# meituan/YOLOv6

Measured on NVIDIA B200. Metric: images/sec YOLOv6-S 640 bs32, higher is better.
Workload: dtype bf16

## Files before the change

### include/yv6.h

```cpp
#ifndef YV6_H_
#define YV6_H_

#include <stdint.h>

#ifdef __cplusplus
extern "C" {
#endif

#define YV6_ABI_VERSION 4

enum {
  YV6_OK = 0,
  YV6_ERR_ARG = -1,
  YV6_ERR_CUDA = -2,
  YV6_ERR_STATE = -3
};

enum { YV6_ACT_NONE = 0, YV6_ACT_RELU = 1, YV6_ACT_SILU = 2, YV6_ACT_SIGMOID = 3 };
enum { YV6_DT_BF16 = 0, YV6_DT_F32 = 1, YV6_DT_U8 = 2 };
#define YV6_PAD_SAME (-1000000)

typedef struct yv6_handle yv6_handle;

int yv6_create(int device, yv6_handle** out);
int yv6_destroy(yv6_handle* h);
const char* yv6_last_error(void);
int yv6_abi_version(void);

typedef struct yv6_conv_desc {
  const void* x;
  int32_t N, H, W, Cin;
  int32_t x_c_total;
  int64_t x_plane_stride;
  const void* w;
  int64_t w_plane_stride;
  const float* bias;
  int32_t Cout, kh, kw, stride, pad;
  int32_t act;
  void* y;
  int32_t y_dtype;
  int64_t y_img_stride, y_h_stride, y_w_stride;
  int64_t y_plane_stride;
  const void* res;
  float alpha;
  int64_t res_img_stride, res_h_stride, res_w_stride, res_plane_stride;
  int32_t nsplit;
  int32_t force_bw, force_bh, force_bi, force_bn, force_stages, force_grid;
  int32_t force_direct;
  int32_t force_halo;
  int32_t pad_w, out_h, out_w;
  int32_t force_groups;
  void* trace;
  int32_t stride_w;
  int32_t force_pair;
  int32_t pair_view;
  int32_t reserved0;
} yv6_conv_desc;

int yv6_conv_fwd(yv6_handle* h, const yv6_conv_desc* d, void* stream);
int yv6_conv_plan(yv6_handle* h, const yv6_conv_desc* d, int32_t* out10);
int yv6_conv_plan_host(int num_sms, int max_smem_optin, int max_clusters, const yv6_conv_desc* d, int32_t* out12);

typedef struct yv6_stem_desc {
  const void* x;
  int32_t x_dtype;
  float in_scale;
  int32_t N, H, W;
  const float* w;
  const float* bias;
  int32_t Cout, act;
  void* y;
  int64_t y_plane_stride;
  int32_t nsplit;
  int32_t fp32_math;
  int32_t force_sync_loads;
} yv6_stem_desc;
int yv6_stem_fwd(yv6_handle* h, const yv6_stem_desc* d, void* stream);

int yv6_sppf_pool(yv6_handle* h, void* buf, int32_t N, int32_t H, int32_t W, int32_t C, int32_t c_total,
                  int32_t nsplit, int64_t plane_stride, void* stream);

int yv6_head_decode(yv6_handle* h, const float* cls, const float* reg, float* out, int32_t B, int32_t nc,
                    int32_t reg_ch, int32_t nl, const int32_t* lvl_h, const int32_t* lvl_w,
                    const float* lvl_stride, void* stream);

int64_t yv6_nms_workspace_bytes(int32_t B, int32_t A, int32_t nc, int32_t multi_label);
int yv6_nms_batched(yv6_handle* h, const float* pred, int32_t B, int32_t A, int32_t nc, float conf_thres,
                    double iou_thres, int32_t agnostic, int32_t multi_label, const uint8_t* class_mask,
                    int32_t max_det, float* out, int32_t* out_count, int32_t* out_src, int32_t* overflow,
                    void* workspace, int64_t workspace_bytes, void* stream);

int yv6_nms_batched_head(yv6_handle* h, const float* cls, const float* reg, int32_t B, int32_t nc, int32_t reg_ch, int32_t nl,
                         const int32_t* lvl_h, const int32_t* lvl_w, const float* lvl_stride, float conf_thres, double iou_thres,
                         int32_t agnostic, int32_t multi_label, const uint8_t* class_mask, int32_t max_det, float* out,
                         int32_t* out_count, int32_t* out_src, int32_t* overflow, void* workspace, int64_t workspace_bytes,
                         void* stream);

int yv6_eval_boxes(yv6_handle* h, const float* det, const int32_t* count, const float* meta, int32_t B, int32_t max_det,
                   float* out, void* stream);


int yv6_targets_pad(yv6_handle* h, const float* targets, int32_t n, int32_t B, int32_t G, float scale_w,
                    float scale_h, double* gt, int32_t* gt_count, void* stream);

int64_t yv6_assign_workspace_bytes(int32_t B, int32_t A, int32_t G);

int yv6_tal_assign(yv6_handle* h, const float* pd_scores, const float* pd_bboxes, const float* anc_points,
                   const double* gt, const uint8_t* mask_gt, int32_t B, int32_t A, int32_t G, int32_t nc,
                   int32_t topk, double alpha, double beta, double eps, int32_t* gt_idx, uint8_t* fg,
                   double* norm, void* workspace, int64_t workspace_bytes, void* stream);

int yv6_atss_assign(yv6_handle* h, const float* anc_bboxes, const int32_t* n_level_bboxes, int32_t nl,
                    const double* gt, const uint8_t* mask_gt, const float* pd_bboxes, int32_t B, int32_t A,
                    int32_t G, int32_t nc, int32_t topk, int32_t* gt_idx, uint8_t* fg, double* norm,
                    void* workspace, int64_t workspace_bytes, void* stream);

int yv6_assign_expand(yv6_handle* h, const double* gt, const int32_t* gt_idx, const uint8_t* fg,
                      const double* norm, int32_t B, int32_t A, int32_t G, int32_t nc, int32_t bg_label,
                      int64_t* labels, double* bboxes, double* scores, uint8_t* fg_out, void* stream);

int yv6_box_decode(yv6_handle* h, const float* pred_distri, const float* anc_points, const float* strides,
                   int32_t B, int32_t A, int32_t reg_ch, int32_t scale_to_pixels, float* boxes, void* stream);

typedef struct yv6_loss_desc {
  const float* pred_scores;
  const float* pred_distri;
  const float* anc_points;
  const float* strides;
  const double* gt;
  const int32_t* gt_idx;
  const uint8_t* fg;
  const double* norm;
  int32_t B, A, G, nc, reg_ch;
  int32_t iou_type;
  double w_cls, w_iou, w_dfl;
  double grad_scale;
  float* grad_scores;
  float* grad_distri;
  double* out;
  void* workspace;
  int64_t workspace_bytes;
  int32_t norm_gt_zero;
} yv6_loss_desc;
int64_t yv6_det_loss_workspace_bytes(int32_t B, int32_t A);
int yv6_det_loss(yv6_handle* h, const yv6_loss_desc* d, void* stream);

int yv6_head_ab_pack(yv6_handle* h, const float* raw_cls, const float* raw_reg, int32_t B, int32_t hw, int32_t na, int32_t nc,
                     const float* anchors_wh, int32_t row_off, int32_t rows_total, float* cls_ab, float* reg_ab, void* stream);
int yv6_head_ab_grad(yv6_handle* h, const float* grad_cls_ab, const float* cls_ab, const float* grad_reg_ab, const float* raw_reg,
                     int32_t B, int32_t hw, int32_t na, int32_t nc, const float* anchors_wh, int32_t row_off, int32_t rows_total,
                     int32_t cls_pad, int32_t reg_pad, void* dl_cls, void* dl_reg, void* stream);
int yv6_ab_boxes(yv6_handle* h, const float* reg_ab, const float* anc_points, const float* strides, int32_t B, int32_t A,
                 float* ltrb, float* boxes_px, void* stream);
int yv6_ab_boxes_bwd(yv6_handle* h, const float* grad_ltrb, int64_t rows, float* grad_reg_ab, void* stream);

int yv6_kl_rows(yv6_handle* h, const float* student, const float* teacher, int64_t rows, int32_t C, float temperature,
                const uint8_t* row_mask, int32_t rows_per_mask, double scale, const double* count_ptr, const double* gate_ptr,
                double* acc, float* grad, void* stream);


typedef struct yv6_wgrad_desc {
  const void* x;  int32_t N, H, W, Cin, x_c_total;
  const void* dy; int32_t Cout, dy_c_total;
  int32_t kh, kw, stride, pad;
  float* dw;
  int32_t force_ksplit;
  int32_t force_taps;
} yv6_wgrad_desc;
int yv6_conv_wgrad(yv6_handle* h, const yv6_wgrad_desc* d, void* stream);

int yv6_bn_stats(yv6_handle* h, const void* x, int64_t pixels, int32_t C, int64_t pitch, double* sum, double* sumsq,
                 void* stream);
int yv6_bn_finalize(yv6_handle* h, const double* sum, const double* sumsq, double count, const float* gamma,
                    const float* beta, float eps, float momentum, float* running_mean, float* running_var,
                    float* mean_out, float* invstd_out, float* scale, float* shift, int32_t C, void* stream);

typedef struct yv6_bn_desc {
  int32_t nb, act, C;
  int64_t pixels;
  const void* x[3];  int64_t x_pitch[3];
  const float* mean[3]; const float* invstd[3]; const float* scale[3]; const float* shift[3];
  void* y; int64_t y_pitch;
  const void* dy; int64_t dy_pitch;
  double* s1; double* s2[3];
  void* dx[3]; int64_t dx_pitch[3]; int32_t accumulate[3];
  const void* res; int64_t res_pitch; float res_alpha;
  void* dres; int64_t dres_pitch; double* dalpha;
  const float* res_alpha_dev;
  double* work; uint32_t* counter; float* coef; int32_t zeroed;
  int32_t dres_assign;
} yv6_bn_desc;
int yv6_bn_apply_fwd(yv6_handle* h, const yv6_bn_desc* d, void* stream);

typedef struct yv6_bn_stats_desc {
  int32_t nb, C;
  int64_t pixels;
  const void* x[3]; int64_t x_pitch[3];
  double* sums;
  uint32_t* counter;
  int32_t zeroed;
  const float* gamma[3]; const float* beta[3];
  float* running_mean[3]; float* running_var[3];
  float* stats[3];
  float eps, momentum;
} yv6_bn_stats_desc;
int yv6_bn_stats_finalize(yv6_handle* h, const yv6_bn_stats_desc* d, void* stream);
int yv6_bn_bwd(yv6_handle* h, const yv6_bn_desc* d, void* stream);

int yv6_head_grad_prep(yv6_handle* h, const float* grad, const float* scores_or_null, int32_t B, int32_t A, int32_t ch,
                       int32_t level_off, int32_t level_hw, int32_t ch_pad, void* out_bf16, void* stream);
int yv6_maxpool5_bwd(yv6_handle* h, const void* x, int64_t x_pitch, const void* dy, int64_t dy_pitch, int32_t N,
                     int32_t H, int32_t W, int32_t C, float* dx_scratch, void* dx, int64_t dx_pitch, int32_t accumulate,
                     void* stream);
int yv6_stem_wgrad(yv6_handle* h, const void* x, int32_t x_dtype, float in_scale, const void* dy, int64_t dy_pitch,
                   int32_t N, int32_t H, int32_t W, int32_t Cout, float* dw, void* stream);

int yv6_stem_wgrad2(yv6_handle* h, const void* x, int32_t x_dtype, float in_scale, const void* dy3, int64_t dy3_pitch,
                    const void* dy1, int64_t dy1_pitch, int32_t N, int32_t H, int32_t W, int32_t Cout, float* dw3, float* dw1,
                    int32_t zeroed, void* stream);

int yv6_stem_im2col(yv6_handle* h, const void* x, int32_t x_dtype, float in_scale, int32_t N, int32_t H, int32_t W,
                    void* patches_bf16, void* patches_lo_bf16, void* stream);

#define YV6_XFORM_CHUNK 4096
enum { YV6_XF_F32 = 0, YV6_XF_F64 = 1, YV6_XF_BF16 = 2 };
typedef struct yv6_xform_seg {
  void* dst; const void* src;
  int32_t n[4], ds[4], ss[4];
  int32_t dst_dtype, src_dtype;
} yv6_xform_seg;
int yv6_xform(yv6_handle* h, const yv6_xform_seg* segs_dev, const int32_t* chunk_seg_dev, const int32_t* chunk_first_dev,
              int32_t n_chunks, int32_t accumulate, void* stream);

int yv6_sgd_ema_step(yv6_handle* h, float* param, const float* grad, float* momentum_buf, float* ema_or_null,
                     const uint8_t* group_per4, int64_t n, const float* hyper_dev, void* stream);

#ifdef __cplusplus
}
#endif
#endif
```

### yolov6_b200/_lib.py

```python
import ctypes as C
import os
import threading

_HERE = os.path.dirname(os.path.abspath(__file__))
LIB_PATH = os.path.join(_HERE, "libyolov6_b200.so")

ACT_NONE, ACT_RELU, ACT_SILU, ACT_SIGMOID = 0, 1, 2, 3
DT_BF16, DT_F32, DT_U8 = 0, 1, 2
PAD_SAME = -1000000
ACT_CODES = {None: ACT_NONE, "none": ACT_NONE, "relu": ACT_RELU, "silu": ACT_SILU, "sigmoid": ACT_SIGMOID}


class ConvDesc(C.Structure):
    _fields_ = [
        ("x", C.c_void_p), ("N", C.c_int32), ("H", C.c_int32), ("W", C.c_int32), ("Cin", C.c_int32),
        ("x_c_total", C.c_int32), ("x_plane_stride", C.c_int64),
        ("w", C.c_void_p), ("w_plane_stride", C.c_int64), ("bias", C.c_void_p),
        ("Cout", C.c_int32), ("kh", C.c_int32), ("kw", C.c_int32), ("stride", C.c_int32), ("pad", C.c_int32),
        ("act", C.c_int32),
        ("y", C.c_void_p), ("y_dtype", C.c_int32),
        ("y_img_stride", C.c_int64), ("y_h_stride", C.c_int64), ("y_w_stride", C.c_int64),
        ("y_plane_stride", C.c_int64),
        ("res", C.c_void_p), ("alpha", C.c_float),
        ("res_img_stride", C.c_int64), ("res_h_stride", C.c_int64), ("res_w_stride", C.c_int64),
        ("res_plane_stride", C.c_int64),
        ("nsplit", C.c_int32),
        ("force_bw", C.c_int32), ("force_bh", C.c_int32), ("force_bi", C.c_int32), ("force_bn", C.c_int32),
        ("force_stages", C.c_int32), ("force_grid", C.c_int32), ("force_direct", C.c_int32), ("force_halo", C.c_int32),
        ("pad_w", C.c_int32), ("out_h", C.c_int32), ("out_w", C.c_int32), ("force_groups", C.c_int32),
        ("trace", C.c_void_p), ("stride_w", C.c_int32), ("force_pair", C.c_int32), ("pair_view", C.c_int32), ("reserved0", C.c_int32),
    ]


class StemDesc(C.Structure):
    _fields_ = [
        ("x", C.c_void_p), ("x_dtype", C.c_int32), ("in_scale", C.c_float),
        ("N", C.c_int32), ("H", C.c_int32), ("W", C.c_int32),
        ("w", C.c_void_p), ("bias", C.c_void_p),
        ("Cout", C.c_int32), ("act", C.c_int32),
        ("y", C.c_void_p), ("y_plane_stride", C.c_int64), ("nsplit", C.c_int32), ("fp32_math", C.c_int32),
        ("force_sync_loads", C.c_int32),
    ]


class LossDesc(C.Structure):
    _fields_ = [
        ("pred_scores", C.c_void_p), ("pred_distri", C.c_void_p), ("anc_points", C.c_void_p), ("strides", C.c_void_p),
        ("gt", C.c_void_p), ("gt_idx", C.c_void_p), ("fg", C.c_void_p), ("norm", C.c_void_p),
        ("B", C.c_int32), ("A", C.c_int32), ("G", C.c_int32), ("nc", C.c_int32), ("reg_ch", C.c_int32),
        ("iou_type", C.c_int32),
        ("w_cls", C.c_double), ("w_iou", C.c_double), ("w_dfl", C.c_double), ("grad_scale", C.c_double),
        ("grad_scores", C.c_void_p), ("grad_distri", C.c_void_p), ("out", C.c_void_p),
        ("workspace", C.c_void_p), ("workspace_bytes", C.c_int64), ("norm_gt_zero", C.c_int32),
    ]


class WgradDesc(C.Structure):
    _fields_ = [
        ("x", C.c_void_p), ("N", C.c_int32), ("H", C.c_int32), ("W", C.c_int32), ("Cin", C.c_int32), ("x_c_total", C.c_int32),
        ("dy", C.c_void_p), ("Cout", C.c_int32), ("dy_c_total", C.c_int32),
        ("kh", C.c_int32), ("kw", C.c_int32), ("stride", C.c_int32), ("pad", C.c_int32),
        ("dw", C.c_void_p), ("force_ksplit", C.c_int32), ("force_taps", C.c_int32),
    ]


class BnDesc(C.Structure):
    _fields_ = [
        ("nb", C.c_int32), ("act", C.c_int32), ("C", C.c_int32), ("pixels", C.c_int64),
        ("x", C.c_void_p * 3), ("x_pitch", C.c_int64 * 3),
        ("mean", C.c_void_p * 3), ("invstd", C.c_void_p * 3), ("scale", C.c_void_p * 3), ("shift", C.c_void_p * 3),
        ("y", C.c_void_p), ("y_pitch", C.c_int64),
        ("dy", C.c_void_p), ("dy_pitch", C.c_int64),
        ("s1", C.c_void_p), ("s2", C.c_void_p * 3),
        ("dx", C.c_void_p * 3), ("dx_pitch", C.c_int64 * 3), ("accumulate", C.c_int32 * 3),
        ("res", C.c_void_p), ("res_pitch", C.c_int64), ("res_alpha", C.c_float),
        ("dres", C.c_void_p), ("dres_pitch", C.c_int64), ("dalpha", C.c_void_p),
        ("res_alpha_dev", C.c_void_p),
        ("work", C.c_void_p), ("counter", C.c_void_p), ("coef", C.c_void_p), ("zeroed", C.c_int32), ("dres_assign", C.c_int32),
    ]


class BnStatsDesc(C.Structure):
    _fields_ = [
        ("nb", C.c_int32), ("C", C.c_int32), ("pixels", C.c_int64),
        ("x", C.c_void_p * 3), ("x_pitch", C.c_int64 * 3),
        ("sums", C.c_void_p), ("counter", C.c_void_p), ("zeroed", C.c_int32),
        ("gamma", C.c_void_p * 3), ("beta", C.c_void_p * 3),
        ("running_mean", C.c_void_p * 3), ("running_var", C.c_void_p * 3),
        ("stats", C.c_void_p * 3),
        ("eps", C.c_float), ("momentum", C.c_float),
    ]


class XformSeg(C.Structure):
    _fields_ = [
        ("dst", C.c_void_p), ("src", C.c_void_p),
        ("n", C.c_int32 * 4), ("ds", C.c_int32 * 4), ("ss", C.c_int32 * 4),
        ("dst_dtype", C.c_int32), ("src_dtype", C.c_int32),
    ]


XF_F32, XF_F64, XF_BF16 = 0, 1, 2
XFORM_CHUNK = 4096


_lib = None
_lock = threading.Lock()
_handles = {}

_SIGNATURES = {
    "yv6_create": (C.c_int, [C.c_int, C.POINTER(C.c_void_p)]),
    "yv6_destroy": (C.c_int, [C.c_void_p]),
    "yv6_last_error": (C.c_char_p, []),
    "yv6_abi_version": (C.c_int, []),
    "yv6_conv_fwd": (C.c_int, [C.c_void_p, C.POINTER(ConvDesc), C.c_void_p]),
    "yv6_conv_plan": (C.c_int, [C.c_void_p, C.POINTER(ConvDesc), C.POINTER(C.c_int32)]),
    "yv6_conv_plan_host": (C.c_int, [C.c_int, C.c_int, C.c_int, C.POINTER(ConvDesc), C.POINTER(C.c_int32)]),
    "yv6_stem_fwd": (C.c_int, [C.c_void_p, C.POINTER(StemDesc), C.c_void_p]),
    "yv6_sppf_pool": (C.c_int, [C.c_void_p, C.c_void_p, C.c_int32, C.c_int32, C.c_int32, C.c_int32, C.c_int32,
                                C.c_int32, C.c_int64, C.c_void_p]),
    "yv6_head_decode": (C.c_int, [C.c_void_p, C.c_void_p, C.c_void_p, C.c_void_p, C.c_int32, C.c_int32, C.c_int32,
                                  C.c_int32, C.POINTER(C.c_int32), C.POINTER(C.c_int32), C.POINTER(C.c_float),
                                  C.c_void_p]),
    "yv6_targets_pad": (C.c_int, [C.c_void_p, C.c_void_p, C.c_int32, C.c_int32, C.c_int32, C.c_float, C.c_float,
                                  C.c_void_p, C.c_void_p, C.c_void_p]),
    "yv6_assign_workspace_bytes": (C.c_int64, [C.c_int32, C.c_int32, C.c_int32]),
    "yv6_tal_assign": (C.c_int, [C.c_void_p, C.c_void_p, C.c_void_p, C.c_void_p, C.c_void_p, C.c_void_p, C.c_int32,
                                 C.c_int32, C.c_int32, C.c_int32, C.c_int32, C.c_double, C.c_double, C.c_double,
                                 C.c_void_p, C.c_void_p, C.c_void_p, C.c_void_p, C.c_int64, C.c_void_p]),
    "yv6_atss_assign": (C.c_int, [C.c_void_p, C.c_void_p, C.POINTER(C.c_int32), C.c_int32, C.c_void_p, C.c_void_p,
                                  C.c_void_p, C.c_int32, C.c_int32, C.c_int32, C.c_int32, C.c_int32, C.c_void_p,
                                  C.c_void_p, C.c_void_p, C.c_void_p, C.c_int64, C.c_void_p]),
    "yv6_assign_expand": (C.c_int, [C.c_void_p, C.c_void_p, C.c_void_p, C.c_void_p, C.c_void_p, C.c_int32, C.c_int32,
                                    C.c_int32, C.c_int32, C.c_int32, C.c_void_p, C.c_void_p, C.c_void_p, C.c_void_p,
                                    C.c_void_p]),
    "yv6_head_ab_pack": (C.c_int, [C.c_void_p, C.c_void_p, C.c_void_p, C.c_int32, C.c_int32, C.c_int32, C.c_int32, C.POINTER(C.c_float),
                                   C.c_int32, C.c_int32, C.c_void_p, C.c_void_p, C.c_void_p]),
    "yv6_head_ab_grad": (C.c_int, [C.c_void_p, C.c_void_p, C.c_void_p, C.c_void_p, C.c_void_p, C.c_int32, C.c_int32, C.c_int32, C.c_int32,
                                   C.POINTER(C.c_float), C.c_int32, C.c_int32, C.c_int32, C.c_int32, C.c_void_p, C.c_void_p, C.c_void_p]),
    "yv6_ab_boxes": (C.c_int, [C.c_void_p, C.c_void_p, C.c_void_p, C.c_void_p, C.c_int32, C.c_int32, C.c_void_p, C.c_void_p, C.c_void_p]),
    "yv6_ab_boxes_bwd": (C.c_int, [C.c_void_p, C.c_void_p, C.c_int64, C.c_void_p, C.c_void_p]),
    "yv6_kl_rows": (C.c_int, [C.c_void_p, C.c_void_p, C.c_void_p, C.c_int64, C.c_int32, C.c_float, C.c_void_p, C.c_int32, C.c_double,
                              C.c_void_p, C.c_void_p, C.c_void_p, C.c_void_p, C.c_void_p]),
    "yv6_box_decode": (C.c_int, [C.c_void_p, C.c_void_p, C.c_void_p, C.c_void_p, C.c_int32, C.c_int32, C.c_int32,
                                 C.c_int32, C.c_void_p, C.c_void_p]),
    "yv6_det_loss_workspace_bytes": (C.c_int64, [C.c_int32, C.c_int32]),
    "yv6_det_loss": (C.c_int, [C.c_void_p, C.POINTER(LossDesc), C.c_void_p]),
    "yv6_conv_wgrad": (C.c_int, [C.c_void_p, C.POINTER(WgradDesc), C.c_void_p]),
    "yv6_bn_stats": (C.c_int, [C.c_void_p, C.c_void_p, C.c_int64, C.c_int32, C.c_int64, C.c_void_p, C.c_void_p, C.c_void_p]),
    "yv6_bn_finalize": (C.c_int, [C.c_void_p, C.c_void_p, C.c_void_p, C.c_double, C.c_void_p, C.c_void_p, C.c_float, C.c_float,
                                  C.c_void_p, C.c_void_p, C.c_void_p, C.c_void_p, C.c_void_p, C.c_void_p, C.c_int32, C.c_void_p]),
    "yv6_bn_apply_fwd": (C.c_int, [C.c_void_p, C.POINTER(BnDesc), C.c_void_p]),
    "yv6_bn_bwd": (C.c_int, [C.c_void_p, C.POINTER(BnDesc), C.c_void_p]),
    "yv6_head_grad_prep": (C.c_int, [C.c_void_p, C.c_void_p, C.c_void_p, C.c_int32, C.c_int32, C.c_int32, C.c_int32, C.c_int32,
                                     C.c_int32, C.c_void_p, C.c_void_p]),
    "yv6_maxpool5_bwd": (C.c_int, [C.c_void_p, C.c_void_p, C.c_int64, C.c_void_p, C.c_int64, C.c_int32, C.c_int32, C.c_int32,
                                   C.c_int32, C.c_void_p, C.c_void_p, C.c_int64, C.c_int32, C.c_void_p]),
    "yv6_stem_wgrad": (C.c_int, [C.c_void_p, C.c_void_p, C.c_int32, C.c_float, C.c_void_p, C.c_int64, C.c_int32, C.c_int32,
                                 C.c_int32, C.c_int32, C.c_void_p, C.c_void_p]),
    "yv6_nms_batched_head": (C.c_int, [C.c_void_p, C.c_void_p, C.c_void_p, C.c_int32, C.c_int32, C.c_int32, C.c_int32,
                                       C.POINTER(C.c_int32), C.POINTER(C.c_int32), C.POINTER(C.c_float), C.c_float, C.c_double,
                                       C.c_int32, C.c_int32, C.c_void_p, C.c_int32, C.c_void_p, C.c_void_p, C.c_void_p,
                                       C.c_void_p, C.c_void_p, C.c_int64, C.c_void_p]),
    "yv6_eval_boxes": (C.c_int, [C.c_void_p, C.c_void_p, C.c_void_p, C.c_void_p, C.c_int32, C.c_int32, C.c_void_p, C.c_void_p]),
    "yv6_bn_stats_finalize": (C.c_int, [C.c_void_p, C.POINTER(BnStatsDesc), C.c_void_p]),
    "yv6_stem_wgrad2": (C.c_int, [C.c_void_p, C.c_void_p, C.c_int32, C.c_float, C.c_void_p, C.c_int64, C.c_void_p, C.c_int64,
                                  C.c_int32, C.c_int32, C.c_int32, C.c_int32, C.c_void_p, C.c_void_p, C.c_int32, C.c_void_p]),
    "yv6_stem_im2col": (C.c_int, [C.c_void_p, C.c_void_p, C.c_int32, C.c_float, C.c_int32, C.c_int32, C.c_int32, C.c_void_p, C.c_void_p, C.c_void_p]),
    "yv6_xform": (C.c_int, [C.c_void_p, C.c_void_p, C.c_void_p, C.c_void_p, C.c_int32, C.c_int32, C.c_void_p]),
    "yv6_sgd_ema_step": (C.c_int, [C.c_void_p, C.c_void_p, C.c_void_p, C.c_void_p, C.c_void_p, C.c_void_p, C.c_int64,
                                   C.c_void_p, C.c_void_p]),
    "yv6_nms_workspace_bytes": (C.c_int64, [C.c_int32, C.c_int32, C.c_int32, C.c_int32]),
    "yv6_nms_batched": (C.c_int, [C.c_void_p, C.c_void_p, C.c_int32, C.c_int32, C.c_int32, C.c_float, C.c_double,
                                  C.c_int32, C.c_int32, C.c_void_p, C.c_int32, C.c_void_p, C.c_void_p, C.c_void_p,
                                  C.c_void_p, C.c_void_p, C.c_int64, C.c_void_p]),
}


def exported_symbols():
    return sorted(_SIGNATURES)


def lib():
    global _lib
    if _lib is not None:
        return _lib
    with _lock:
        if _lib is None:
            if not os.path.exists(LIB_PATH):
                raise RuntimeError(
                    f"{LIB_PATH} is missing: build it with `python -c 'import __graft_entry__ as g; g.build()'` "
                    "(yolov6_b200 has no CPU/PyTorch fallback for its CUDA path)")
            l = C.CDLL(LIB_PATH)
            for name, (res, args) in _SIGNATURES.items():
                try:
                    fn = getattr(l, name)
                except AttributeError as e:
                    raise RuntimeError(f"{LIB_PATH} does not export {name}; rebuild the library") from e
                fn.restype = res
                fn.argtypes = args
            _lib = l
    return _lib


def check(rc):
    if rc != 0:
        raise RuntimeError(f"yolov6_b200 kernel call failed ({rc}): {lib().yv6_last_error().decode()}")


def handle(device_index=0):
    h = _handles.get(device_index)
    if h is None:
        p = C.c_void_p()
        check(lib().yv6_create(int(device_index), C.byref(p)))
        h = _handles[device_index] = p
    return h


def stream_ptr(stream=None):
    import torch
    s = stream if stream is not None else torch.cuda.current_stream()
    return C.c_void_p(s.cuda_stream)
```

### yolov6_b200/csrc/yv6_aux.cu

```cuda
#include "yv6_common.cuh"
#include "yv6_handle.h"

namespace yv6 {

constexpr int kStemMaxCout = 64;
struct StemParams {
  const float* w;
  const float* b;
  const void* x;
  __nv_bfloat16* y;
  int64_t y_plane_stride;
  int32_t N, H, W, Ho, Wo;
  int32_t x_u8, act, planes;
  float in_scale;
};

template <int COUT>
__global__ void __launch_bounds__(256) stem_kernel(const StemParams p) {
  __shared__ __align__(16) float sw[27 * COUT];
  __shared__ __align__(16) __nv_bfloat16 tile[256 * COUT];
  for (int i = threadIdx.x; i < 27 * COUT; i += 256) sw[i] = p.w[i];
  __syncthreads();
  const int64_t total = (int64_t)p.N * p.Ho * p.Wo;
  const int64_t pix0 = (int64_t)blockIdx.x * 256;
  const int64_t pix = pix0 + threadIdx.x;
  float acc[COUT];
#pragma unroll
  for (int c = 0; c < COUT; ++c) acc[c] = p.b ? p.b[c] : 0.f;
  if (pix < total) {
    const int wo = (int)(pix % p.Wo);
    const int ho = (int)((pix / p.Wo) % p.Ho);
    const int n = (int)(pix / ((int64_t)p.Wo * p.Ho));
#pragma unroll
    for (int r = 0; r < 3; ++r) {
      const int hi = 2 * ho - 1 + r;
#pragma unroll
      for (int s = 0; s < 3; ++s) {
        const int wi = 2 * wo - 1 + s;
        const bool ok = (hi >= 0) && (hi < p.H) && (wi >= 0) && (wi < p.W);
#pragma unroll
        for (int c = 0; c < 3; ++c) {
          float v = 0.f;
          if (ok) {
            const int64_t idx = (((int64_t)n * 3 + c) * p.H + hi) * p.W + wi;
            v = p.x_u8 ? (float)__ldg(reinterpret_cast<const uint8_t*>(p.x) + idx) * p.in_scale
                       : __ldg(reinterpret_cast<const float*>(p.x) + idx);
          }
          const float4* wk = reinterpret_cast<const float4*>(&sw[((r * 3 + s) * 3 + c) * COUT]);
#pragma unroll
          for (int c4 = 0; c4 < COUT / 4; ++c4) {
            const float4 w4 = wk[c4];
            acc[4 * c4 + 0] = fmaf(v, w4.x, acc[4 * c4 + 0]);
            acc[4 * c4 + 1] = fmaf(v, w4.y, acc[4 * c4 + 1]);
            acc[4 * c4 + 2] = fmaf(v, w4.z, acc[4 * c4 + 2]);
            acc[4 * c4 + 3] = fmaf(v, w4.w, acc[4 * c4 + 3]);
          }
        }
      }
    }
#pragma unroll
    for (int c = 0; c < COUT; ++c) acc[c] = act_apply(acc[c], p.act);
  }
  const int nvec = 256 * COUT / 8;
  const int64_t left = total - pix0;
  const int64_t valid_elems = (left < 256 ? left : (int64_t)256) * COUT;
  for (int pl = 0; pl < p.planes; ++pl) {
    if (pl) __syncthreads();
#pragma unroll
    for (int c = 0; c < COUT; c += 2) {
      __nv_bfloat162 v = __floats2bfloat162_rn(acc[c], acc[c + 1]);
      *reinterpret_cast<__nv_bfloat162*>(&tile[threadIdx.x * COUT + c]) = v;
      if (pl + 1 < p.planes) {
        acc[c] -= __low2float(v);
        acc[c + 1] -= __high2float(v);
      }
    }
    __syncthreads();
    uint4* dst = reinterpret_cast<uint4*>(p.y + pl * p.y_plane_stride + pix0 * COUT);
    const uint4* src = reinterpret_cast<const uint4*>(tile);
    for (int i = threadIdx.x; i < nvec; i += 256)
      if ((int64_t)i * 8 < valid_elems) dst[i] = src[i];
  }
}

template <int COUT>
__global__ void __launch_bounds__(256, 2) stem_mma_kernel(const StemParams p) {
  constexpr int TH = 8, TW = 32, PH = 2 * TH + 1, PW = 2 * TW + 1, NT = COUT / 8;
  constexpr int PWP = 68;
  static_assert(PW + 1 <= PWP, "patch pitch");
  constexpr int PITCH = COUT * 2 + 16;
  __shared__ __align__(16) __nv_bfloat16 patch[3 * PH * PWP];
  __shared__ __align__(16) uint8_t stage[8 * 32 * PITCH];
  const int tiles_w = (p.Wo + TW - 1) / TW, tiles_h = (p.Ho + TH - 1) / TH;
  const int num_tiles = tiles_w * tiles_h * p.N;
  const int warp = threadIdx.x >> 5, lane = threadIdx.x & 31, g = lane >> 2, t = lane & 3;

  uint32_t bfrag[NT][2][2];
#pragma unroll
  for (int nt = 0; nt < NT; ++nt)
#pragma unroll
    for (int ks = 0; ks < 2; ++ks)
#pragma unroll
      for (int h2 = 0; h2 < 2; ++h2) {
        const int k = ks * 16 + h2 * 8 + 2 * t, nn = nt * 8 + g;
        const float w0 = (k < 27) ? __ldg(p.w + k * COUT + nn) : 0.f;
        const float w1 = (k + 1 < 27) ? __ldg(p.w + (k + 1) * COUT + nn) : 0.f;
        __nv_bfloat162 v = __floats2bfloat162_rn(w0, w1);
        bfrag[nt][ks][h2] = *reinterpret_cast<uint32_t*>(&v);
      }
  float bias[NT][2];
#pragma unroll
  for (int nt = 0; nt < NT; ++nt) {
    bias[nt][0] = p.b ? __ldg(p.b + nt * 8 + 2 * t) : 0.f;
    bias[nt][1] = p.b ? __ldg(p.b + nt * 8 + 2 * t + 1) : 0.f;
  }
  int koff[2][2][2];
#pragma unroll
  for (int ks = 0; ks < 2; ++ks)
#pragma unroll
    for (int h2 = 0; h2 < 2; ++h2)
#pragma unroll
      for (int e = 0; e < 2; ++e) {
        const int k = ks * 16 + h2 * 8 + 2 * t + e;
        const int tap = k / 3, c = k - 3 * tap, r = tap / 3, sx = tap - 3 * r;
        koff[ks][h2][e] = (k < 27) ? (c * PH + r) * PWP + sx + 1 : -1;
      }
  const bool vec_ok = (p.W % 4 == 0);
  const unsigned short* P = reinterpret_cast<const unsigned short*>(patch);
  uint8_t* wstage = stage + warp * 32 * PITCH;

  constexpr int NITEM = (3 * PH * 17 + 255) / 256;
  float4 pre[NITEM];
  auto fetch = [&](int tile) {
    const int tw = tile % tiles_w, th = (tile / tiles_w) % tiles_h, n = tile / (tiles_w * tiles_h);
    const int hi0 = 2 * th * TH - 1, wi0 = 2 * tw * TW - 1;
#pragma unroll
    for (int it = 0; it < NITEM; ++it) {
      const int item = threadIdx.x + it * 256;
      float4 v = make_float4(0.f, 0.f, 0.f, 0.f);
      if (item < 3 * PH * 17) {
        const int rc = item / 17, q = item - rc * 17;
        const int row = rc % PH, c = rc / PH;
        const int hi = hi0 + row;
        if (hi >= 0 && hi < p.H) {
          const int64_t rbase = (((int64_t)n * 3 + c) * p.H + hi) * p.W;
          if (q == 0) {
            if (wi0 >= 0)
              v.x = p.x_u8 ? (float)__ldg(reinterpret_cast<const uint8_t*>(p.x) + rbase + wi0) * p.in_scale
                           : __ldg(reinterpret_cast<const float*>(p.x) + rbase + wi0);
          } else {
            const int wi = wi0 + 1 + 4 * (q - 1);
            if (vec_ok && wi + 3 < p.W) {
              if (p.x_u8) {
                const uchar4 u = __ldg(reinterpret_cast<const uchar4*>(reinterpret_cast<const uint8_t*>(p.x) + rbase + wi));
                v = make_float4(u.x * p.in_scale, u.y * p.in_scale, u.z * p.in_scale, u.w * p.in_scale);
              } else {
                v = __ldg(reinterpret_cast<const float4*>(reinterpret_cast<const float*>(p.x) + rbase + wi));
              }
            } else {
              float e[4] = {0.f, 0.f, 0.f, 0.f};
#pragma unroll
              for (int j = 0; j < 4; ++j)
                if (wi + j < p.W)
                  e[j] = p.x_u8 ? (float)__ldg(reinterpret_cast<const uint8_t*>(p.x) + rbase + wi + j) * p.in_scale
                                : __ldg(reinterpret_cast<const float*>(p.x) + rbase + wi + j);
              v = make_float4(e[0], e[1], e[2], e[3]);
            }
          }
        }
      }
      pre[it] = v;
    }
  };
  if ((int)blockIdx.x < num_tiles) fetch(blockIdx.x);

  for (int tile = blockIdx.x; tile < num_tiles; tile += gridDim.x) {
    const int tw = tile % tiles_w, th = (tile / tiles_w) % tiles_h, n = tile / (tiles_w * tiles_h);
    const int px0 = tw * TW, py0 = th * TH;
    __syncthreads();
#pragma unroll
    for (int it = 0; it < NITEM; ++it) {
      const int item = threadIdx.x + it * 256;
      if (item < 3 * PH * 17) {
        const int rc = item / 17, q = item - rc * 17;
        __nv_bfloat16* dst = patch + rc * PWP;
        if (q == 0) {
          dst[1] = __float2bfloat16_rn(pre[it].x);
        } else {
          __nv_bfloat162* d2 = reinterpret_cast<__nv_bfloat162*>(dst + 2 + 4 * (q - 1));
          d2[0] = __floats2bfloat162_rn(pre[it].x, pre[it].y);
          d2[1] = __floats2bfloat162_rn(pre[it].z, pre[it].w);
        }
      }
    }
    __syncthreads();
    if (tile + (int)gridDim.x < num_tiles) fetch(tile + gridDim.x);
    float acc[2][NT][4];
#pragma unroll
    for (int mt = 0; mt < 2; ++mt)
#pragma unroll
      for (int nt = 0; nt < NT; ++nt)
#pragma unroll
        for (int j = 0; j < 4; ++j) acc[mt][nt][j] = 0.f;
#pragma unroll
    for (int mt = 0; mt < 2; ++mt) {
      const int base0 = (2 * warp) * PWP + 2 * (mt * 16 + g), base1 = base0 + 16;
#pragma unroll
      for (int ks = 0; ks < 2; ++ks) {
        uint32_t a[4];
#pragma unroll
        for (int h2 = 0; h2 < 2; ++h2) {
          const int o0 = koff[ks][h2][0], o1 = koff[ks][h2][1];
          const uint32_t lo0 = o0 >= 0 ? P[base0 + o0] : 0u, hi0v = o1 >= 0 ? P[base0 + o1] : 0u;
          const uint32_t lo1 = o0 >= 0 ? P[base1 + o0] : 0u, hi1v = o1 >= 0 ? P[base1 + o1] : 0u;
          a[2 * h2 + 0] = lo0 | (hi0v << 16);
          a[2 * h2 + 1] = lo1 | (hi1v << 16);
        }
#pragma unroll
        for (int nt = 0; nt < NT; ++nt) {
          asm volatile(
              "mma.sync.aligned.m16n8k16.row.col.f32.bf16.bf16.f32 {%0,%1,%2,%3}, {%4,%5,%6,%7}, {%8,%9}, {%0,%1,%2,%3};"
              : "+f"(acc[mt][nt][0]), "+f"(acc[mt][nt][1]), "+f"(acc[mt][nt][2]), "+f"(acc[mt][nt][3])
              : "r"(a[0]), "r"(a[1]), "r"(a[2]), "r"(a[3]), "r"(bfrag[nt][ks][0]), "r"(bfrag[nt][ks][1]));
        }
      }
    }
#pragma unroll
    for (int mt = 0; mt < 2; ++mt)
#pragma unroll
      for (int nt = 0; nt < NT; ++nt) {
        const float v0 = act_apply(acc[mt][nt][0] + bias[nt][0], p.act), v1 = act_apply(acc[mt][nt][1] + bias[nt][1], p.act);
        const float v2 = act_apply(acc[mt][nt][2] + bias[nt][0], p.act), v3 = act_apply(acc[mt][nt][3] + bias[nt][1], p.act);
        *reinterpret_cast<__nv_bfloat162*>(wstage + (mt * 16 + g) * PITCH + (nt * 8 + 2 * t) * 2) = __floats2bfloat162_rn(v0, v1);
        *reinterpret_cast<__nv_bfloat162*>(wstage + (mt * 16 + g + 8) * PITCH + (nt * 8 + 2 * t) * 2) = __floats2bfloat162_rn(v2, v3);
      }
    __syncwarp();
    const int py = py0 + warp;
    if (py < p.Ho) {
      const int valid = min(TW, p.Wo - px0);
      __nv_bfloat16* dst = p.y + (((int64_t)n * p.Ho + py) * p.Wo + px0) * COUT;
      constexpr int CPP = COUT / 8;
      for (int i = lane; i < valid * CPP; i += 32) {
        const int px = i / CPP, part = i - px * CPP;
        reinterpret_cast<uint4*>(dst)[i] = *reinterpret_cast<const uint4*>(wstage + px * PITCH + part * 16);
      }
    }
    __syncwarp();
  }
}

__device__ __forceinline__ void cp_async16(void* dst, const void* src, int src_bytes) {
  asm volatile("cp.async.cg.shared.global [%0], [%1], 16, %2;" ::"r"(smem_u32(dst)), "l"(src), "r"(src_bytes) : "memory");
}
__device__ __forceinline__ void cp_async4(void* dst, const void* src, int src_bytes) {
  asm volatile("cp.async.ca.shared.global [%0], [%1], 4, %2;" ::"r"(smem_u32(dst)), "l"(src), "r"(src_bytes) : "memory");
}
__device__ __forceinline__ void cp_async_commit() { asm volatile("cp.async.commit_group;" ::: "memory"); }
template <int N>
__device__ __forceinline__ void cp_async_wait() { asm volatile("cp.async.wait_group %0;" ::"n"(N) : "memory"); }

template <int COUT>
__global__ void __launch_bounds__(256, 2) stem_mma_async_kernel(const StemParams p) {
  constexpr int TH = 8, TW = 32, PH = 2 * TH + 1, NT = COUT / 8;
  constexpr int PWP = 72;
  constexpr int PATCH = 3 * PH * PWP;
  constexpr int STAGES = 3;
  constexpr int PITCH = COUT * 2 + 16;
  extern __shared__ __align__(16) uint8_t stem_smem[];
  float* ring = reinterpret_cast<float*>(stem_smem);
  uint8_t* stage = stem_smem + (size_t)STAGES * PATCH * sizeof(float);
  const int tiles_w = (p.Wo + TW - 1) / TW, tiles_h = (p.Ho + TH - 1) / TH;
  const int num_tiles = tiles_w * tiles_h * p.N;
  const int warp = threadIdx.x >> 5, lane = threadIdx.x & 31, g = lane >> 2, t = lane & 3;

  uint32_t bfrag[NT][2][2];
#pragma unroll
  for (int nt = 0; nt < NT; ++nt)
#pragma unroll
    for (int ks = 0; ks < 2; ++ks)
#pragma unroll
      for (int h2 = 0; h2 < 2; ++h2) {
        const int k = ks * 16 + h2 * 8 + 2 * t, nn = nt * 8 + g;
        const float w0 = (k < 27) ? __ldg(p.w + k * COUT + nn) : 0.f;
        const float w1 = (k + 1 < 27) ? __ldg(p.w + (k + 1) * COUT + nn) : 0.f;
        __nv_bfloat162 v = __floats2bfloat162_rn(w0, w1);
        bfrag[nt][ks][h2] = *reinterpret_cast<uint32_t*>(&v);
      }
  float bias[NT][2];
#pragma unroll
  for (int nt = 0; nt < NT; ++nt) {
    bias[nt][0] = p.b ? __ldg(p.b + nt * 8 + 2 * t) : 0.f;
    bias[nt][1] = p.b ? __ldg(p.b + nt * 8 + 2 * t + 1) : 0.f;
  }
  int koff[2][2][2];
#pragma unroll
  for (int ks = 0; ks < 2; ++ks)
#pragma unroll
    for (int h2 = 0; h2 < 2; ++h2)
#pragma unroll
      for (int e = 0; e < 2; ++e) {
        const int k = ks * 16 + h2 * 8 + 2 * t + e;
        const int tap = k / 3, c = k - 3 * tap, r = tap / 3, sx = tap - 3 * r;
        koff[ks][h2][e] = (k < 27) ? (c * PH + r) * PWP + sx + 3 : -1;
      }
  uint8_t* wstage = stage + warp * 32 * PITCH;
  const float* X = reinterpret_cast<const float*>(p.x);

  auto issue = [&](int tile, int slot) {
    if (tile < num_tiles) {
      const int tw = tile % tiles_w, th = (tile / tiles_w) % tiles_h, n = tile / (tiles_w * tiles_h);
      const int hi0 = 2 * th * TH - 1, wc0 = 64 * tw;
      float* dst0 = ring + (size_t)slot * PATCH;
      for (int item = threadIdx.x; item < 3 * PH * 17; item += 256) {
        const int rc = item / 17, q = item - rc * 17;
        const int row = rc % PH, c = rc / PH;
        const int hi = hi0 + row;
        const bool row_ok = (hi >= 0 && hi < p.H);
        const float* src_row = X + (((int64_t)n * 3 + c) * p.H + (row_ok ? hi : 0)) * p.W;
        float* d = dst0 + rc * PWP;
        if (q == 0) {
          const int col = wc0 - 1;
          const bool ok = row_ok && col >= 0;
          cp_async4(d + 3, src_row + (ok ? col : 0), ok ? 4 : 0);
        } else {
          const int col = wc0 + 4 * (q - 1);
          const int nb = row_ok ? max(0, min(16, (p.W - col) * 4)) : 0;
          cp_async16(d + 4 + 4 * (q - 1), src_row + (nb > 0 ? col : 0), nb);
        }
      }
    }
    cp_async_commit();
  };
  issue(blockIdx.x, 0);
  issue(blockIdx.x + gridDim.x, 1);
  int slot = 0;
  for (int tile = blockIdx.x; tile < num_tiles; tile += gridDim.x) {
    const int tw = tile % tiles_w, th = (tile / tiles_w) % tiles_h, n = tile / (tiles_w * tiles_h);
    const int px0 = tw * TW, py0 = th * TH;
    cp_async_wait<1>();
    __syncthreads();
    issue(tile + 2 * gridDim.x, (slot + 2) % STAGES);
    const float* P = ring + (size_t)slot * PATCH;
    float acc[2][NT][4];
#pragma unroll
    for (int mt = 0; mt < 2; ++mt)
#pragma unroll
      for (int nt = 0; nt < NT; ++nt)
#pragma unroll
        for (int j = 0; j < 4; ++j) acc[mt][nt][j] = 0.f;
#pragma unroll
    for (int mt = 0; mt < 2; ++mt) {
      const int base0 = (2 * warp) * PWP + 2 * (mt * 16 + g), base1 = base0 + 16;
#pragma unroll
      for (int ks = 0; ks < 2; ++ks) {
        uint32_t a[4];
#pragma unroll
        for (int h2 = 0; h2 < 2; ++h2) {
          const int o0 = koff[ks][h2][0], o1 = koff[ks][h2][1];
          const float l0 = o0 >= 0 ? P[base0 + o0] : 0.f, h0 = o1 >= 0 ? P[base0 + o1] : 0.f;
          const float l1 = o0 >= 0 ? P[base1 + o0] : 0.f, h1 = o1 >= 0 ? P[base1 + o1] : 0.f;
          __nv_bfloat162 q0 = __floats2bfloat162_rn(l0, h0), q1 = __floats2bfloat162_rn(l1, h1);
          a[2 * h2 + 0] = *reinterpret_cast<uint32_t*>(&q0);
          a[2 * h2 + 1] = *reinterpret_cast<uint32_t*>(&q1);
        }
#pragma unroll
        for (int nt = 0; nt < NT; ++nt) {
          asm volatile(
              "mma.sync.aligned.m16n8k16.row.col.f32.bf16.bf16.f32 {%0,%1,%2,%3}, {%4,%5,%6,%7}, {%8,%9}, {%0,%1,%2,%3};"
              : "+f"(acc[mt][nt][0]), "+f"(acc[mt][nt][1]), "+f"(acc[mt][nt][2]), "+f"(acc[mt][nt][3])
              : "r"(a[0]), "r"(a[1]), "r"(a[2]), "r"(a[3]), "r"(bfrag[nt][ks][0]), "r"(bfrag[nt][ks][1]));
        }
      }
    }
#pragma unroll
    for (int mt = 0; mt < 2; ++mt)
#pragma unroll
      for (int nt = 0; nt < NT; ++nt) {
        const float v0 = act_apply(acc[mt][nt][0] + bias[nt][0], p.act), v1 = act_apply(acc[mt][nt][1] + bias[nt][1], p.act);
        const float v2 = act_apply(acc[mt][nt][2] + bias[nt][0], p.act), v3 = act_apply(acc[mt][nt][3] + bias[nt][1], p.act);
        *reinterpret_cast<__nv_bfloat162*>(wstage + (mt * 16 + g) * PITCH + (nt * 8 + 2 * t) * 2) = __floats2bfloat162_rn(v0, v1);
        *reinterpret_cast<__nv_bfloat162*>(wstage + (mt * 16 + g + 8) * PITCH + (nt * 8 + 2 * t) * 2) = __floats2bfloat162_rn(v2, v3);
      }
    __syncwarp();
    const int py = py0 + warp;
    if (py < p.Ho) {
      const int valid = min(TW, p.Wo - px0);
      __nv_bfloat16* dst = p.y + (((int64_t)n * p.Ho + py) * p.Wo + px0) * COUT;
      constexpr int CPP = COUT / 8;
      for (int i = lane; i < valid * CPP; i += 32) {
        const int px = i / CPP, part = i - px * CPP;
        reinterpret_cast<uint4*>(dst)[i] = *reinterpret_cast<const uint4*>(wstage + px * PITCH + part * 16);
      }
    }
    __syncwarp();
    slot = (slot + 1) % STAGES;
  }
  cp_async_wait<0>();
}

struct PoolParams {
  __nv_bfloat16* buf;
  int64_t plane_stride;
  int32_t N, H, W, C, c_total, planes;
};

__device__ __forceinline__ void load8(const __nv_bfloat16* p, float (&v)[8]) {
  const uint4 q = __ldg(reinterpret_cast<const uint4*>(p));
  const uint32_t w[4] = {q.x, q.y, q.z, q.w};
#pragma unroll
  for (int j = 0; j < 4; ++j) {
    const __nv_bfloat162 b2 = *reinterpret_cast<const __nv_bfloat162*>(&w[j]);
    v[2 * j] = __low2float(b2);
    v[2 * j + 1] = __high2float(b2);
  }
}

__global__ void __launch_bounds__(256) sppf_pool_kernel(const PoolParams p) {
  extern __shared__ float sp[];
  const int cgs = p.C / 8;
  const int n = blockIdx.x / cgs, cg = blockIdx.x % cgs;
  const int HW = p.H * p.W;
  float* sx = sp;
  float* r5 = sp + (size_t)HW * 8;
  float* r9 = r5 + (size_t)HW * 8;
  float* r13 = r9 + (size_t)HW * 8;
  for (int i = threadIdx.x; i < HW; i += blockDim.x) {
    const int64_t off = ((int64_t)n * HW + i) * p.c_total + cg * 8;
    float v[8];
    load8(p.buf + off, v);
    for (int pl = 1; pl < p.planes; ++pl) {
      float t[8];
      load8(p.buf + pl * p.plane_stride + off, t);
#pragma unroll
      for (int j = 0; j < 8; ++j) v[j] += t[j];
    }
#pragma unroll
    for (int j = 0; j < 8; ++j) sx[i * 8 + j] = v[j];
  }
  __syncthreads();
  for (int i = threadIdx.x; i < HW; i += blockDim.x) {
    const int h = i / p.W, w = i % p.W;
    float m5[8], m9[8], m13[8];
#pragma unroll
    for (int j = 0; j < 8; ++j) m5[j] = m9[j] = m13[j] = -INFINITY;
    for (int dx = -6; dx <= 6; ++dx) {
      const int ww = w + dx;
      if (ww < 0 || ww >= p.W) continue;
      const float* v = &sx[(h * p.W + ww) * 8];
      const int ad = abs(dx);
#pragma unroll
      for (int j = 0; j < 8; ++j) {
        m13[j] = fmaxf(m13[j], v[j]);
        if (ad <= 4) m9[j] = fmaxf(m9[j], v[j]);
        if (ad <= 2) m5[j] = fmaxf(m5[j], v[j]);
      }
    }
#pragma unroll
    for (int j = 0; j < 8; ++j) { r5[i * 8 + j] = m5[j]; r9[i * 8 + j] = m9[j]; r13[i * 8 + j] = m13[j]; }
  }
  __syncthreads();
  for (int i = threadIdx.x; i < HW; i += blockDim.x) {
    const int h = i / p.W, w = i % p.W;
    float m[3][8];
#pragma unroll
    for (int j = 0; j < 8; ++j) m[0][j] = m[1][j] = m[2][j] = -INFINITY;
    for (int dy = -6; dy <= 6; ++dy) {
      const int hh = h + dy;
      if (hh < 0 || hh >= p.H) continue;
      const int o = (hh * p.W + w) * 8;
      const int ad = abs(dy);
#pragma unroll
      for (int j = 0; j < 8; ++j) {
        m[2][j] = fmaxf(m[2][j], r13[o + j]);
        if (ad <= 4) m[1][j] = fmaxf(m[1][j], r9[o + j]);
        if (ad <= 2) m[0][j] = fmaxf(m[0][j], r5[o + j]);
      }
    }
    const int64_t o = ((int64_t)n * HW + i) * p.c_total + cg * 8;
#pragma unroll
    for (int k = 0; k < 3; ++k) {
      for (int pl = 0; pl < p.planes; ++pl) {
        uint32_t wds[4];
#pragma unroll
        for (int j = 0; j < 4; ++j) {
          __nv_bfloat162 b2 = __floats2bfloat162_rn(m[k][2 * j], m[k][2 * j + 1]);
          wds[j] = *reinterpret_cast<uint32_t*>(&b2);
          m[k][2 * j] -= __low2float(b2);
          m[k][2 * j + 1] -= __high2float(b2);
        }
        *reinterpret_cast<uint4*>(p.buf + pl * p.plane_stride + o + (int64_t)(k + 1) * p.C) =
            make_uint4(wds[0], wds[1], wds[2], wds[3]);
      }
    }
  }
}

__device__ __forceinline__ uint4 hmax8(uint4 a, uint4 b) {
  uint4 r;
  *reinterpret_cast<__nv_bfloat162*>(&r.x) = __hmax2(*reinterpret_cast<__nv_bfloat162*>(&a.x), *reinterpret_cast<__nv_bfloat162*>(&b.x));
  *reinterpret_cast<__nv_bfloat162*>(&r.y) = __hmax2(*reinterpret_cast<__nv_bfloat162*>(&a.y), *reinterpret_cast<__nv_bfloat162*>(&b.y));
  *reinterpret_cast<__nv_bfloat162*>(&r.z) = __hmax2(*reinterpret_cast<__nv_bfloat162*>(&a.z), *reinterpret_cast<__nv_bfloat162*>(&b.z));
  *reinterpret_cast<__nv_bfloat162*>(&r.w) = __hmax2(*reinterpret_cast<__nv_bfloat162*>(&a.w), *reinterpret_cast<__nv_bfloat162*>(&b.w));
  return r;
}

__global__ void __launch_bounds__(256) sppf_pool_bf16_kernel(const PoolParams p) {
  extern __shared__ uint4 sq[];
  const int cgs = p.C / 16;
  const int n = blockIdx.x / cgs, cg = blockIdx.x % cgs;
  const int HW = p.H * p.W, U = HW * 2;
  uint4* sx = sq;
  uint4* r5 = sq + U;
  uint4* r9 = r5 + U;
  uint4* r13 = r9 + U;
  const __nv_bfloat16* src = p.buf + (int64_t)n * HW * p.c_total + cg * 16;
  for (int u = threadIdx.x; u < U; u += blockDim.x)
    sx[u] = __ldg(reinterpret_cast<const uint4*>(src + (int64_t)(u >> 1) * p.c_total + (u & 1) * 8));
  __syncthreads();
  for (int u = threadIdx.x; u < U; u += blockDim.x) {
    const int i = u >> 1, half = u & 1;
    const int h = i / p.W, w = i - h * p.W;
    uint4 m5 = sx[u], m9, m13;
#pragma unroll
    for (int dx = 1; dx <= 2; ++dx) {
      if (w - dx >= 0) m5 = hmax8(m5, sx[u - 2 * dx]);
      if (w + dx < p.W) m5 = hmax8(m5, sx[u + 2 * dx]);
    }
    m9 = m5;
#pragma unroll
    for (int dx = 3; dx <= 4; ++dx) {
      if (w - dx >= 0) m9 = hmax8(m9, sx[u - 2 * dx]);
      if (w + dx < p.W) m9 = hmax8(m9, sx[u + 2 * dx]);
    }
    m13 = m9;
#pragma unroll
    for (int dx = 5; dx <= 6; ++dx) {
      if (w - dx >= 0) m13 = hmax8(m13, sx[u - 2 * dx]);
      if (w + dx < p.W) m13 = hmax8(m13, sx[u + 2 * dx]);
    }
    (void)half;
    r5[u] = m5;
    r9[u] = m9;
    r13[u] = m13;
  }
  __syncthreads();
  __nv_bfloat16* dst = p.buf + (int64_t)n * HW * p.c_total + cg * 16;
  const int rs = 2 * p.W;
  for (int u = threadIdx.x; u < U; u += blockDim.x) {
    const int i = u >> 1;
    const int h = i / p.W;
    uint4 m5 = r5[u], m9 = r9[u], m13 = r13[u];
#pragma unroll
    for (int dy = 1; dy <= 6; ++dy) {
      if (h - dy >= 0) {
        if (dy <= 2) m5 = hmax8(m5, r5[u - dy * rs]);
        if (dy <= 4) m9 = hmax8(m9, r9[u - dy * rs]);
        m13 = hmax8(m13, r13[u - dy * rs]);
      }
      if (h + dy < p.H) {
        if (dy <= 2) m5 = hmax8(m5, r5[u + dy * rs]);
        if (dy <= 4) m9 = hmax8(m9, r9[u + dy * rs]);
        m13 = hmax8(m13, r13[u + dy * rs]);
      }
    }
    __nv_bfloat16* o = dst + (int64_t)i * p.c_total + (u & 1) * 8;
    *reinterpret_cast<uint4*>(o + (int64_t)p.C) = m5;
    *reinterpret_cast<uint4*>(o + (int64_t)2 * p.C) = m9;
    *reinterpret_cast<uint4*>(o + (int64_t)3 * p.C) = m13;
  }
}

constexpr int kMaxLevels = 6;
struct DecodeParams {
  const float* cls;
  const float* reg;
  float* out;
  int32_t B, A, nc, R, reg_max, nl;
  int32_t lvl_off[kMaxLevels + 1];
  int32_t lvl_w[kMaxLevels];
  float lvl_stride[kMaxLevels];
};

__global__ void __launch_bounds__(256) head_decode_kernel(const __grid_constant__ DecodeParams p) {
  const int lane = threadIdx.x & 31;
  const int64_t row = (int64_t)blockIdx.x * (blockDim.x >> 5) + (threadIdx.x >> 5);
  if (row >= (int64_t)p.B * p.A) return;
  const int a = (int)(row % p.A);
  const float* cls = p.cls + row * p.nc;
  float* out = p.out + row * (5 + p.nc);
  for (int c = lane; c < p.nc; c += 32) out[5 + c] = __ldg(cls + c);
  float dist = 0.f;
  if (lane < 4) {
    const float* reg = p.reg + row * p.R;
    if (p.R == 4) {
      dist = __ldg(reg + lane);
    } else {
      const int nb = p.reg_max + 1;
      const float* l = reg + lane * nb;
      float mx = -INFINITY;
      for (int i = 0; i < nb; ++i) mx = fmaxf(mx, __ldg(l + i));
      float den = 0.f;
      for (int i = 0; i < nb; ++i) den += expf(__ldg(l + i) - mx);
      float e = 0.f;
      for (int i = 0; i < nb; ++i) e = __fadd_rn(e, __fmul_rn(expf(__ldg(l + i) - mx) / den, (float)i));
      dist = e;
    }
  }
  const float dl = __shfl_sync(0xffffffffu, dist, 0), dt = __shfl_sync(0xffffffffu, dist, 1);
  const float dr = __shfl_sync(0xffffffffu, dist, 2), db = __shfl_sync(0xffffffffu, dist, 3);
  if (lane == 0) {
    int lvl = 0;
    while (lvl + 1 < p.nl && a >= p.lvl_off[lvl + 1]) ++lvl;
    const int local = a - p.lvl_off[lvl];
    const float ax = (float)(local % p.lvl_w[lvl]) + 0.5f;
    const float ay = (float)(local / p.lvl_w[lvl]) + 0.5f;
    const float s = p.lvl_stride[lvl];
    const float x1 = __fsub_rn(ax, dl), y1 = __fsub_rn(ay, dt);
    const float x2 = __fadd_rn(ax, dr), y2 = __fadd_rn(ay, db);
    out[0] = __fmul_rn(__fdiv_rn(__fadd_rn(x1, x2), 2.f), s);
    out[1] = __fmul_rn(__fdiv_rn(__fadd_rn(y1, y2), 2.f), s);
    out[2] = __fmul_rn(__fsub_rn(x2, x1), s);
    out[3] = __fmul_rn(__fsub_rn(y2, y1), s);
    out[4] = 1.0f;
  }
}

}

using namespace yv6;

extern "C" int yv6_stem_fwd(yv6_handle* h, const yv6_stem_desc* d, void* stream) {
  yv6_device_guard _dev(h);
  YV6_REQUIRE(h && d && d->x && d->w && d->y, "stem: null argument");
  YV6_REQUIRE(d->Cout > 0 && d->Cout <= kStemMaxCout && d->Cout % 16 == 0, "stem: Cout=%d must be 16/32/48/64", d->Cout);
  YV6_REQUIRE(d->nsplit == 1 || d->nsplit == 3, "stem: nsplit must be 1 or 3");
  YV6_REQUIRE(d->x_dtype == YV6_DT_F32 || d->x_dtype == YV6_DT_U8, "stem: image must be fp32 or uint8");
  StemParams p;
  p.w = d->w;
  p.b = d->bias;
  p.x = d->x;
  p.y = reinterpret_cast<__nv_bfloat16*>(d->y);
  p.y_plane_stride = d->y_plane_stride;
  p.N = d->N;
  p.H = d->H;
  p.W = d->W;
  p.Ho = (d->H + 2 - 3) / 2 + 1;
  p.Wo = (d->W + 2 - 3) / 2 + 1;
  p.x_u8 = (d->x_dtype == YV6_DT_U8);
  p.in_scale = d->in_scale;
  p.act = d->act;
  p.planes = d->nsplit;
  const int64_t total = (int64_t)p.N * p.Ho * p.Wo;
  const unsigned grid = (unsigned)((total + 255) / 256);
  cudaStream_t s = (cudaStream_t)stream;
  if (d->nsplit == 1 && !d->fp32_math) {
    const unsigned ntile = (unsigned)(((p.Wo + 31) / 32) * ((p.Ho + 7) / 8) * p.N);
    const unsigned tiles = std::min<unsigned>(ntile, (unsigned)h->num_sms * 2);
    if (!p.x_u8 && p.W % 4 == 0 && (reinterpret_cast<uintptr_t>(p.x) & 15) == 0 && (d->Cout == 16 || d->Cout == 32 || d->Cout == 48 || d->Cout == 64) &&
        d->force_sync_loads == 0) {
      const size_t smem = (size_t)3 * 3 * 17 * 72 * 4 + (size_t)8 * 32 * (d->Cout * 2 + 16);
      if (!(h->configured & YV6_CFG_STEM)) {
        YV6_CHECK_CUDA(cudaFuncSetAttribute(stem_mma_async_kernel<16>, cudaFuncAttributeMaxDynamicSharedMemorySize, 96 * 1024));
        YV6_CHECK_CUDA(cudaFuncSetAttribute(stem_mma_async_kernel<32>, cudaFuncAttributeMaxDynamicSharedMemorySize, 96 * 1024));
        YV6_CHECK_CUDA(cudaFuncSetAttribute(stem_mma_async_kernel<48>, cudaFuncAttributeMaxDynamicSharedMemorySize, 96 * 1024));
        YV6_CHECK_CUDA(cudaFuncSetAttribute(stem_mma_async_kernel<64>, cudaFuncAttributeMaxDynamicSharedMemorySize, 96 * 1024));
        h->configured |= YV6_CFG_STEM;
      }
      switch (d->Cout) {
        case 16: stem_mma_async_kernel<16><<<tiles, 256, smem, s>>>(p); break;
        case 32: stem_mma_async_kernel<32><<<tiles, 256, smem, s>>>(p); break;
        case 48: stem_mma_async_kernel<48><<<tiles, 256, smem, s>>>(p); break;
        default: stem_mma_async_kernel<64><<<tiles, 256, smem, s>>>(p); break;
      }
      YV6_CHECK_CUDA(cudaGetLastError());
      return YV6_OK;
    }
    switch (d->Cout) {
      case 16: stem_mma_kernel<16><<<tiles, 256, 0, s>>>(p); break;
      case 32: stem_mma_kernel<32><<<tiles, 256, 0, s>>>(p); break;
      case 48: stem_mma_kernel<48><<<tiles, 256, 0, s>>>(p); break;
      default: stem_mma_kernel<64><<<tiles, 256, 0, s>>>(p); break;
    }
    YV6_CHECK_CUDA(cudaGetLastError());
    return YV6_OK;
  }
  switch (d->Cout) {
    case 16: stem_kernel<16><<<grid, 256, 0, s>>>(p); break;
    case 32: stem_kernel<32><<<grid, 256, 0, s>>>(p); break;
    case 48: stem_kernel<48><<<grid, 256, 0, s>>>(p); break;
    default: stem_kernel<64><<<grid, 256, 0, s>>>(p); break;
  }
  YV6_CHECK_CUDA(cudaGetLastError());
  return YV6_OK;
}

extern "C" int yv6_sppf_pool(yv6_handle* h, void* buf, int32_t N, int32_t H, int32_t W, int32_t C, int32_t c_total,
                             int32_t nsplit, int64_t plane_stride, void* stream) {
  yv6_device_guard _dev(h);
  YV6_REQUIRE(h && buf, "sppf_pool: null argument");
  YV6_REQUIRE(C % 8 == 0 && c_total >= 4 * C && c_total % 8 == 0, "sppf_pool: bad channels C=%d c_total=%d", C, c_total);
  const size_t smem = (size_t)4 * H * W * 8 * sizeof(float);
  YV6_REQUIRE(smem <= (size_t)h->max_smem_optin, "sppf_pool: %dx%d plane does not fit in shared memory", H, W);
  PoolParams p{reinterpret_cast<__nv_bfloat16*>(buf), plane_stride, N, H, W, C, c_total, nsplit == 3 ? 3 : 1};
  if (!(h->configured & YV6_CFG_POOL)) {
    YV6_CHECK_CUDA(cudaFuncSetAttribute(sppf_pool_kernel, cudaFuncAttributeMaxDynamicSharedMemorySize, (int)h->max_smem_optin));
    h->configured |= YV6_CFG_POOL;
  }
  const size_t smem16 = (size_t)4 * H * W * 32;
  if (nsplit != 3 && C % 16 == 0 && smem16 <= (size_t)h->max_smem_optin) {
    if (!(h->configured & YV6_CFG_POOL16)) {
      YV6_CHECK_CUDA(cudaFuncSetAttribute(sppf_pool_bf16_kernel, cudaFuncAttributeMaxDynamicSharedMemorySize, (int)h->max_smem_optin));
      h->configured |= YV6_CFG_POOL16;
    }
    sppf_pool_bf16_kernel<<<(unsigned)(N * (C / 16)), 256, smem16, (cudaStream_t)stream>>>(p);
    YV6_CHECK_CUDA(cudaGetLastError());
    return YV6_OK;
  }
  sppf_pool_kernel<<<(unsigned)(N * (C / 8)), 256, smem, (cudaStream_t)stream>>>(p);
  YV6_CHECK_CUDA(cudaGetLastError());
  return YV6_OK;
}

extern "C" int yv6_head_decode(yv6_handle* h, const float* cls, const float* reg, float* out, int32_t B, int32_t nc,
                               int32_t reg_ch, int32_t nl, const int32_t* lvl_h, const int32_t* lvl_w,
                               const float* lvl_stride, void* stream) {
  yv6_device_guard _dev(h);
  YV6_REQUIRE(h && cls && reg && out && lvl_h && lvl_w && lvl_stride, "head_decode: null argument");
  YV6_REQUIRE(nl >= 1 && nl <= kMaxLevels, "head_decode: nl=%d out of range", nl);
  YV6_REQUIRE(reg_ch == 4 || reg_ch % 4 == 0, "head_decode: reg_ch=%d", reg_ch);
  DecodeParams p;
  p.cls = cls;
  p.reg = reg;
  p.out = out;
  p.B = B;
  p.nc = nc;
  p.R = reg_ch;
  p.reg_max = reg_ch / 4 - 1;
  p.nl = nl;
  int off = 0;
  for (int l = 0; l < nl; ++l) {
    p.lvl_off[l] = off;
    p.lvl_w[l] = lvl_w[l];
    p.lvl_stride[l] = lvl_stride[l];
    off += lvl_h[l] * lvl_w[l];
  }
  p.lvl_off[nl] = off;
  p.A = off;
  const int64_t rows = (int64_t)B * p.A;
  head_decode_kernel<<<(unsigned)((rows + 7) / 8), 256, 0, (cudaStream_t)stream>>>(p);
  YV6_CHECK_CUDA(cudaGetLastError());
  return YV6_OK;
}
```

### yolov6_b200/csrc/yv6_common.cuh

```cuda
#pragma once
#include <cuda.h>
#include <cuda_bf16.h>
#include <cuda_runtime.h>
#include <stdint.h>
#include <stdio.h>
#include <string.h>

#include "../../include/yv6.h"

void yv6_set_error(const char* fmt, ...);

#define YV6_CHECK_CUDA(expr)                                                          \
  do {                                                                                \
    cudaError_t _e = (expr);                                                          \
    if (_e != cudaSuccess) {                                                          \
      yv6_set_error("%s:%d CUDA error %d (%s) in `%s`", __FILE__, __LINE__, (int)_e,  \
                    cudaGetErrorString(_e), #expr);                                   \
      (void)cudaGetLastError();  \
      return YV6_ERR_CUDA;                                                            \
    }                                                                                 \
  } while (0)

#define YV6_REQUIRE(cond, ...)                                                        \
  do {                                                                                \
    if (!(cond)) {                                                                    \
      yv6_set_error(__VA_ARGS__);                                                     \
      return YV6_ERR_ARG;                                                             \
    }                                                                                 \
  } while (0)

namespace yv6 {

__device__ __forceinline__ uint32_t smem_u32(const void* p) {
  return static_cast<uint32_t>(__cvta_generic_to_shared(p));
}

__device__ __forceinline__ uint32_t lane_id() { return threadIdx.x & 31; }

__device__ __forceinline__ bool elect_one() {
  uint32_t pred;
  asm volatile(
      "{\n"
      ".reg .pred p;\n"
      "elect.sync _|p, 0xffffffff;\n"
      "selp.b32 %0, 1, 0, p;\n"
      "}\n"
      : "=r"(pred));
  return pred != 0;
}

__device__ __forceinline__ void mbar_init(uint64_t* bar, uint32_t count) {
  asm volatile("mbarrier.init.shared::cta.b64 [%0], %1;" ::"r"(smem_u32(bar)), "r"(count));
}
__device__ __forceinline__ void fence_mbar_init() {
  asm volatile("fence.mbarrier_init.release.cluster;" ::: "memory");
}
__device__ __forceinline__ void fence_proxy_async_smem() {
  asm volatile("fence.proxy.async.shared::cta;" ::: "memory");
}
__device__ __forceinline__ void mbar_expect_tx(uint64_t* bar, uint32_t bytes) {
  asm volatile("mbarrier.arrive.expect_tx.shared::cta.b64 _, [%0], %1;" ::"r"(smem_u32(bar)),
               "r"(bytes)
               : "memory");
}
__device__ __forceinline__ void mbar_arrive(uint64_t* bar) {
  asm volatile("mbarrier.arrive.shared::cta.b64 _, [%0];" ::"r"(smem_u32(bar)) : "memory");
}
__device__ __forceinline__ bool mbar_try_wait(uint64_t* bar, uint32_t parity) {
  uint32_t ok;
  asm volatile(
      "{\n"
      ".reg .pred p;\n"
      "mbarrier.try_wait.parity.shared::cta.b64 p, [%1], %2;\n"
      "selp.b32 %0, 1, 0, p;\n"
      "}\n"
      : "=r"(ok)
      : "r"(smem_u32(bar)), "r"(parity)
      : "memory");
  return ok != 0;
}
static __device__ __noinline__ void mbar_wait_slow(uint64_t* bar, uint32_t parity) {
  uint64_t t0 = 0;
  uint32_t spins = 0;
  while (!mbar_try_wait(bar, parity)) {
    if ((++spins & 0x3fff) == 0) {
      uint64_t now;
      asm volatile("mov.u64 %0, %%globaltimer;" : "=l"(now));
      if (t0 == 0) t0 = now;
      else if (now - t0 > 4000000000ull) {
        if ((threadIdx.x & 31) == 0) printf("yv6: mbarrier wait timeout block %d warp %d\n", blockIdx.x, threadIdx.x >> 5);
        __trap();
      }
    }
  }
}
__device__ __forceinline__ void mbar_wait(uint64_t* bar, uint32_t parity) {
  if (!mbar_try_wait(bar, parity)) mbar_wait_slow(bar, parity);
}

__device__ __forceinline__ void tma_prefetch_desc(const CUtensorMap* m) {
  asm volatile("prefetch.tensormap [%0];" ::"l"(reinterpret_cast<uint64_t>(m)) : "memory");
}
__device__ __forceinline__ void tma_load_2d(void* dst, const CUtensorMap* m, uint64_t* bar, int c0,
                                            int c1) {
  asm volatile(
      "cp.async.bulk.tensor.2d.shared::cluster.global.tile.mbarrier::complete_tx::bytes"
      " [%0], [%1, {%3, %4}], [%2];" ::"r"(smem_u32(dst)),
      "l"(reinterpret_cast<uint64_t>(m)), "r"(smem_u32(bar)), "r"(c0), "r"(c1)
      : "memory");
}
__device__ __forceinline__ void tma_load_5d(void* dst, const CUtensorMap* m, uint64_t* bar, int c0,
                                            int c1, int c2, int c3, int c4) {
  asm volatile(
      "cp.async.bulk.tensor.5d.shared::cluster.global.tile.mbarrier::complete_tx::bytes"
      " [%0], [%1, {%3, %4, %5, %6, %7}], [%2];" ::"r"(smem_u32(dst)),
      "l"(reinterpret_cast<uint64_t>(m)), "r"(smem_u32(bar)), "r"(c0), "r"(c1), "r"(c2), "r"(c3),
      "r"(c4)
      : "memory");
}

__device__ __forceinline__ void tc_fence_before() {
  asm volatile("tcgen05.fence::before_thread_sync;" ::: "memory");
}
__device__ __forceinline__ void tc_fence_after() {
  asm volatile("tcgen05.fence::after_thread_sync;" ::: "memory");
}
__device__ __forceinline__ void tmem_alloc(uint32_t* dst_smem, uint32_t ncols) {
  asm volatile("tcgen05.alloc.cta_group::1.sync.aligned.shared::cta.b32 [%0], %1;" ::"r"(
                   smem_u32(dst_smem)),
               "r"(ncols)
               : "memory");
  asm volatile("tcgen05.relinquish_alloc_permit.cta_group::1.sync.aligned;" ::: "memory");
}
__device__ __forceinline__ void tmem_dealloc(uint32_t taddr, uint32_t ncols) {
  asm volatile("tcgen05.dealloc.cta_group::1.sync.aligned.b32 %0, %1;" ::"r"(taddr), "r"(ncols)
               : "memory");
}
__device__ __forceinline__ void umma_bf16(uint32_t tmem_d, uint64_t adesc, uint64_t bdesc,
                                          uint32_t idesc, uint32_t accumulate) {
  asm volatile(
      "{\n"
      ".reg .pred p;\n"
      "setp.ne.b32 p, %4, 0;\n"
      "tcgen05.mma.cta_group::1.kind::f16 [%0], %1, %2, %3, p;\n"
      "}\n" ::"r"(tmem_d),
      "l"(adesc), "l"(bdesc), "r"(idesc), "r"(accumulate)
      : "memory");
}
__device__ __forceinline__ void umma_commit(uint64_t* bar) {
  asm volatile("tcgen05.commit.cta_group::1.mbarrier::arrive::one.shared::cluster.b64 [%0];" ::"r"(
                   smem_u32(bar))
               : "memory");
}
__device__ __forceinline__ uint32_t cluster_ctarank() {
  uint32_t r;
  asm volatile("mov.u32 %0, %%cluster_ctarank;" : "=r"(r));
  return r;
}
__device__ __forceinline__ void cluster_sync_all() {
  asm volatile("barrier.cluster.arrive.release.aligned;" ::: "memory");
  asm volatile("barrier.cluster.wait.acquire.aligned;" ::: "memory");
}
constexpr uint32_t kPeerBitMask = 0xFEFFFFFFu;
__device__ __forceinline__ void tmem_alloc_pair(uint32_t* dst_smem, uint32_t ncols) {
  asm volatile("tcgen05.alloc.cta_group::2.sync.aligned.shared::cta.b32 [%0], %1;" ::"r"(smem_u32(dst_smem)), "r"(ncols)
               : "memory");
  asm volatile("tcgen05.relinquish_alloc_permit.cta_group::2.sync.aligned;" ::: "memory");
}
__device__ __forceinline__ void tmem_dealloc_pair(uint32_t taddr, uint32_t ncols) {
  asm volatile("tcgen05.dealloc.cta_group::2.sync.aligned.b32 %0, %1;" ::"r"(taddr), "r"(ncols) : "memory");
}
__device__ __forceinline__ void umma_bf16_pair(uint32_t tmem_d, uint64_t adesc, uint64_t bdesc, uint32_t idesc,
                                               uint32_t accumulate) {
  asm volatile(
      "{\n"
      ".reg .pred p;\n"
      "setp.ne.b32 p, %4, 0;\n"
      "tcgen05.mma.cta_group::2.kind::f16 [%0], %1, %2, %3, p;\n"
      "}\n" ::"r"(tmem_d),
      "l"(adesc), "l"(bdesc), "r"(idesc), "r"(accumulate)
      : "memory");
}
__device__ __forceinline__ void umma_commit_pair(uint64_t* bar) {
  asm volatile("tcgen05.commit.cta_group::2.mbarrier::arrive::one.shared::cluster.multicast::cluster.b64 [%0], %1;" ::"r"(
                   smem_u32(bar)),
               "h"((uint16_t)3)
               : "memory");
}
__device__ __forceinline__ void tma_load_5d_pair(void* dst, const CUtensorMap* m, uint64_t* bar, int c0, int c1, int c2,
                                                 int c3, int c4) {
  asm volatile(
      "cp.async.bulk.tensor.5d.cta_group::2.shared::cluster.global.mbarrier::complete_tx::bytes"
      " [%0], [%1, {%3, %4, %5, %6, %7}], [%2];" ::"r"(smem_u32(dst)),
      "l"(reinterpret_cast<uint64_t>(m)), "r"(smem_u32(bar) & kPeerBitMask), "r"(c0), "r"(c1), "r"(c2), "r"(c3), "r"(c4)
      : "memory");
}
__device__ __forceinline__ void tma_load_3d_pair(void* dst, const CUtensorMap* m, uint64_t* bar, int c0, int c1, int c2) {
  asm volatile(
      "cp.async.bulk.tensor.3d.cta_group::2.shared::cluster.global.mbarrier::complete_tx::bytes"
      " [%0], [%1, {%3, %4, %5}], [%2];" ::"r"(smem_u32(dst)),
      "l"(reinterpret_cast<uint64_t>(m)), "r"(smem_u32(bar) & kPeerBitMask), "r"(c0), "r"(c1), "r"(c2)
      : "memory");
}
__device__ __forceinline__ void mbar_arrive_leader(uint64_t* bar) {
  asm volatile("mbarrier.arrive.release.cluster.shared::cluster.b64 _, [%0];" ::"r"(smem_u32(bar) & kPeerBitMask) : "memory");
}

__device__ __forceinline__ void tmem_ld16(uint32_t taddr, uint32_t (&r)[16]) {
  asm volatile(
      "tcgen05.ld.sync.aligned.32x32b.x16.b32 "
      "{%0, %1, %2, %3, %4, %5, %6, %7, %8, %9, %10, %11, %12, %13, %14, %15}, [%16];"
      : "=r"(r[0]), "=r"(r[1]), "=r"(r[2]), "=r"(r[3]), "=r"(r[4]), "=r"(r[5]), "=r"(r[6]),
        "=r"(r[7]), "=r"(r[8]), "=r"(r[9]), "=r"(r[10]), "=r"(r[11]), "=r"(r[12]), "=r"(r[13]),
        "=r"(r[14]), "=r"(r[15])
      : "r"(taddr)
      : "memory");
}
__device__ __forceinline__ void tmem_ld32(uint32_t taddr, uint32_t (&r)[32]) {
  asm volatile(
      "tcgen05.ld.sync.aligned.32x32b.x32.b32 "
      "{%0, %1, %2, %3, %4, %5, %6, %7, %8, %9, %10, %11, %12, %13, %14, %15, "
      "%16, %17, %18, %19, %20, %21, %22, %23, %24, %25, %26, %27, %28, %29, %30, %31}, [%32];"
      : "=r"(r[0]), "=r"(r[1]), "=r"(r[2]), "=r"(r[3]), "=r"(r[4]), "=r"(r[5]), "=r"(r[6]), "=r"(r[7]),
        "=r"(r[8]), "=r"(r[9]), "=r"(r[10]), "=r"(r[11]), "=r"(r[12]), "=r"(r[13]), "=r"(r[14]), "=r"(r[15]),
        "=r"(r[16]), "=r"(r[17]), "=r"(r[18]), "=r"(r[19]), "=r"(r[20]), "=r"(r[21]), "=r"(r[22]), "=r"(r[23]),
        "=r"(r[24]), "=r"(r[25]), "=r"(r[26]), "=r"(r[27]), "=r"(r[28]), "=r"(r[29]), "=r"(r[30]), "=r"(r[31])
      : "r"(taddr)
      : "memory");
}
__device__ __forceinline__ void tmem_ld_wait() {
  asm volatile("tcgen05.wait::ld.sync.aligned;" ::: "memory");
}

__device__ __forceinline__ uint64_t umma_smem_desc(uint32_t saddr, uint32_t sbo_bytes,
                                                   uint32_t layout_type) {
  uint64_t d = 0;
  d |= (uint64_t)((saddr >> 4) & 0x3fff);
  d |= (uint64_t)1 << 16;
  d |= (uint64_t)((sbo_bytes >> 4) & 0x3fff) << 32;
  d |= (uint64_t)1 << 46;
  d |= (uint64_t)(layout_type & 7) << 61;
  return d;
}

__host__ __device__ inline uint32_t umma_idesc_bf16(uint32_t M, uint32_t N) {
  uint32_t d = 0;
  d |= 1u << 4;
  d |= 1u << 7;
  d |= 1u << 10;
  d |= (N >> 3) << 17;
  d |= (M >> 4) << 24;
  return d;
}

__device__ __forceinline__ float act_apply(float v, int act) {
  switch (act) {
    case YV6_ACT_RELU: return fmaxf(v, 0.f);
    case YV6_ACT_SILU: return v / (1.f + expf(-v));
    case YV6_ACT_SIGMOID: return 1.f / (1.f + expf(-v));
    default: return v;
  }
}

}
```

### yolov6_b200/csrc/yv6_conv_igemm.cu

```cuda
#include <algorithm>
#include <cstdarg>

#include "yv6_common.cuh"
#include "yv6_handle.h"

namespace yv6 {

constexpr int kMaxGroups = 4;
constexpr int kMaxStages = 12;
constexpr int kTileRows = 128;

struct ConvKParams {
  int32_t BW, BH, BI, rows;
  int32_t tiles_w, tiles_h, tiles_i, tiles_n, num_tiles;
  int32_t N, Ho, Wo, Cout, BN;
  int32_t taps, kw, stride, stride_w, pad, pad_w, Cin;
  int32_t cin_blocks, kb_elems, kb_bytes, ksteps;
  int32_t sbo_bytes, layout_type;
  int32_t npairs;
  int32_t stages, a_stage_bytes, b_stage_bytes;
  int32_t tmem_cols, groups;
  int32_t act, y_dtype, out_planes, res_planes;
  void* y;
  int64_t y_img_stride, y_h_stride, y_w_stride, y_plane_stride;
  const __nv_bfloat16* res;
  float alpha;
  int64_t res_img_stride, res_h_stride, res_w_stride, res_plane_stride;
  const float* bias;
  int32_t tma_store;
  int32_t c_chunk;
  int32_t halo, a_stages, b_stages, b_resident;
  int32_t skip_cb;
  int32_t a_region_bytes, b_region_bytes;
  int32_t cpair, m_tiles, b_rows;
  int32_t bias_smem;
  int32_t res_aligned;
  int32_t fast_act;
  unsigned long long* trace;
};
#define YV6_TRACE(slot) do { if (p.trace != nullptr && blockIdx.x == 0) p.trace[slot] = (unsigned long long)clock64(); } while (0)

constexpr int kHaloW = 10, kHaloH = 18;
constexpr int kHaloBytes = kHaloW * kHaloH * 128;
constexpr int kHaloStageBytes = 24 * 1024;
template <bool S2>
struct HaloGeom {
  static constexpr int W = S2 ? 9 : kHaloW, H = S2 ? 33 : kHaloH, KW = S2 ? 2 : 3, TAPS = S2 ? 6 : 9, SH = S2 ? 2 : 1;
  static constexpr int kBytes = W * H * 128;
  static constexpr int kStageBytes = ((kBytes + 1023) / 1024) * 1024;
};
constexpr int kMaxAStages = 6, kMaxBStages = 40;

__device__ __forceinline__ void tma_load_3d(void* dst, const CUtensorMap* m, uint64_t* bar, int c0,
                                            int c1, int c2) {
  asm volatile(
      "cp.async.bulk.tensor.3d.shared::cluster.global.tile.mbarrier::complete_tx::bytes"
      " [%0], [%1, {%3, %4, %5}], [%2];" ::"r"(smem_u32(dst)),
      "l"(reinterpret_cast<uint64_t>(m)), "r"(smem_u32(bar)), "r"(c0), "r"(c1), "r"(c2)
      : "memory");
}

__device__ __forceinline__ void tma_store_5d(const CUtensorMap* m, const void* src, int c0, int c1, int c2,
                                             int c3, int c4) {
  asm volatile(
      "cp.async.bulk.tensor.5d.global.shared::cta.tile.bulk_group [%0, {%2, %3, %4, %5, %6}], [%1];" ::"l"(
          reinterpret_cast<uint64_t>(m)),
      "r"(smem_u32(src)), "r"(c0), "r"(c1), "r"(c2), "r"(c3), "r"(c4)
      : "memory");
}
__device__ __forceinline__ void tma_store_commit() { asm volatile("cp.async.bulk.commit_group;" ::: "memory"); }
template <int N>
__device__ __forceinline__ void tma_store_wait_read() {
  asm volatile("cp.async.bulk.wait_group.read %0;" ::"n"(N) : "memory");
}
__device__ __forceinline__ void epi_bar_sync(int group) {
  asm volatile("bar.sync %0, 128;" ::"r"(group + 1) : "memory");
}

struct TileCoord {
  int w0, h0, i0, n0;
};
__device__ __forceinline__ TileCoord decode_tile(const ConvKParams& p, int tile) {
  TileCoord t;
  int nt = tile % p.tiles_n;
  int m = tile / p.tiles_n;
  int tw = m % p.tiles_w;
  m /= p.tiles_w;
  int th = m % p.tiles_h;
  int ti = m / p.tiles_h;
  t.w0 = tw * p.BW;
  t.h0 = th * p.BH;
  t.i0 = ti * p.BI;
  t.n0 = nt * p.BN;
  return t;
}

__device__ __forceinline__ TileCoord decode_unit(const ConvKParams& p, int unit, int rank) {
  TileCoord t;
  const int nt = unit % p.tiles_n;
  int m = (unit / p.tiles_n) * 2 + rank;
  t.n0 = nt * p.BN;
  if (m >= p.m_tiles) {
    t.w0 = 0;
    t.h0 = 0;
    t.i0 = p.N;
    return t;
  }
  const int tw = m % p.tiles_w;
  m /= p.tiles_w;
  const int th = m % p.tiles_h;
  const int ti = m / p.tiles_h;
  t.w0 = tw * p.BW;
  t.h0 = th * p.BH;
  t.i0 = ti * p.BI;
  return t;
}

__constant__ int kPairA[6] = {0, 1, 2, 0, 1, 0};
__constant__ int kPairB[6] = {2, 1, 0, 1, 0, 0};

__device__ __forceinline__ uint32_t pack_bf16x2(float a, float b) {
  __nv_bfloat162 v = __floats2bfloat162_rn(a, b);
  return *reinterpret_cast<uint32_t*>(&v);
}

__device__ __forceinline__ void store_chunk(const ConvKParams& p, int64_t off, int n, int ncol,
                                            const float (&v)[16]) {
  if (p.y_dtype == YV6_DT_F32) {
    float* y = reinterpret_cast<float*>(p.y) + off + n;
    if (ncol == 16 && ((reinterpret_cast<uintptr_t>(y) & 15) == 0)) {
      float4* y4 = reinterpret_cast<float4*>(y);
#pragma unroll
      for (int j = 0; j < 4; ++j) y4[j] = make_float4(v[4 * j], v[4 * j + 1], v[4 * j + 2], v[4 * j + 3]);
    } else {
      for (int j = 0; j < ncol; ++j) y[j] = v[j];
    }
    return;
  }
  float rem[16];
#pragma unroll
  for (int j = 0; j < 16; ++j) rem[j] = v[j];
  for (int pl = 0; pl < p.out_planes; ++pl) {
    __nv_bfloat16* y = reinterpret_cast<__nv_bfloat16*>(p.y) + pl * p.y_plane_stride + off + n;
    if (ncol == 16 && ((reinterpret_cast<uintptr_t>(y) & 15) == 0)) {
      uint4 q0, q1;
      q0.x = pack_bf16x2(rem[0], rem[1]);
      q0.y = pack_bf16x2(rem[2], rem[3]);
      q0.z = pack_bf16x2(rem[4], rem[5]);
      q0.w = pack_bf16x2(rem[6], rem[7]);
      q1.x = pack_bf16x2(rem[8], rem[9]);
      q1.y = pack_bf16x2(rem[10], rem[11]);
      q1.z = pack_bf16x2(rem[12], rem[13]);
      q1.w = pack_bf16x2(rem[14], rem[15]);
      reinterpret_cast<uint4*>(y)[0] = q0;
      reinterpret_cast<uint4*>(y)[1] = q1;
    } else {
      for (int j = 0; j < ncol; ++j) y[j] = __float2bfloat16_rn(rem[j]);
    }
    if (pl + 1 < p.out_planes) {
#pragma unroll
      for (int j = 0; j < 16; ++j) rem[j] -= __bfloat162float(__float2bfloat16_rn(rem[j]));
    }
  }
}

constexpr int kCBufBytes = kTileRows * 128;
constexpr int kCBufCount = 4;

constexpr int kBiasSmemFloats = 1024;

__device__ __forceinline__ float ex2_ftz(float x) {
  float y;
  asm("ex2.approx.ftz.f32 %0, %1;" : "=f"(y) : "f"(x));
  return y;
}
__device__ __forceinline__ float rcp_ftz(float x) {
  float y;
  asm("rcp.approx.ftz.f32 %0, %1;" : "=f"(y) : "f"(x));
  return y;
}
__device__ __forceinline__ float tanh_fast(float x) {
  float y;
  asm("tanh.approx.f32 %0, %1;" : "=f"(y) : "f"(x));
  return y;
}

__device__ __forceinline__ void epilogue_math(const ConvKParams& p, const float* sbias, const uint32_t (&r)[16], int n, int ncol,
                                              bool valid, int64_t roff, float (&v)[16]) {
  if (p.bias != nullptr) {
#pragma unroll
    for (int j = 0; j < 4; ++j) {
      const float4 b = sbias ? *reinterpret_cast<const float4*>(sbias + n + 4 * j)
                             : __ldg(reinterpret_cast<const float4*>(p.bias + n) + j);
      v[4 * j + 0] = __uint_as_float(r[4 * j + 0]) + b.x;
      v[4 * j + 1] = __uint_as_float(r[4 * j + 1]) + b.y;
      v[4 * j + 2] = __uint_as_float(r[4 * j + 2]) + b.z;
      v[4 * j + 3] = __uint_as_float(r[4 * j + 3]) + b.w;
    }
  } else {
#pragma unroll
    for (int j = 0; j < 16; ++j) v[j] = __uint_as_float(r[j]);
  }
  if (p.act == YV6_ACT_RELU) {
#pragma unroll
    for (int j = 0; j < 16; ++j) v[j] = fmaxf(v[j], 0.f);
  } else if (p.act == YV6_ACT_SILU) {
    if (p.fast_act) {
#pragma unroll
      for (int j = 0; j < 16; ++j) {
        const float h = 0.5f * v[j];
        v[j] = fmaf(h, tanh_fast(h), h);
      }
    } else {
#pragma unroll
      for (int j = 0; j < 16; ++j) v[j] = v[j] * rcp_ftz(1.f + ex2_ftz(-1.4426950408889634f * v[j]));
    }
  } else if (p.act == YV6_ACT_SIGMOID) {
#pragma unroll
    for (int j = 0; j < 16; ++j) v[j] = rcp_ftz(1.f + ex2_ftz(-1.4426950408889634f * v[j]));
  }
  if (p.res != nullptr && valid && ncol > 0) {
    for (int pl = 0; pl < p.res_planes; ++pl) {
      const __nv_bfloat16* rp = p.res + pl * p.res_plane_stride + roff + n;
      if (ncol == 16 && ((reinterpret_cast<uintptr_t>(rp) & 15) == 0)) {
        const uint4 q0 = __ldg(reinterpret_cast<const uint4*>(rp));
        const uint4 q1 = __ldg(reinterpret_cast<const uint4*>(rp) + 1);
        const uint32_t w[8] = {q0.x, q0.y, q0.z, q0.w, q1.x, q1.y, q1.z, q1.w};
#pragma unroll
        for (int j = 0; j < 8; ++j) {
          const __nv_bfloat162 b2 = *reinterpret_cast<const __nv_bfloat162*>(&w[j]);
          v[2 * j] += p.alpha * __low2float(b2);
          v[2 * j + 1] += p.alpha * __high2float(b2);
        }
      } else {
#pragma unroll
        for (int j = 0; j < 16; ++j)
          if (j < ncol) v[j] += p.alpha * __bfloat162float(rp[j]);
      }
    }
  }
}

template <bool F32>
__device__ __forceinline__ void epi_cols32(const ConvKParams& p, const float* sbias, uint32_t taddr, int n,
                                           const __nv_bfloat16* res_row, uint32_t base, uint32_t rxor, int unit0) {
  uint32_t r[32];
  tmem_ld32(taddr, r);
  uint4 rq[4];
  if (res_row != nullptr) {
#pragma unroll
    for (int j = 0; j < 4; ++j) rq[j] = __ldg(reinterpret_cast<const uint4*>(res_row + n) + j);
  }
  tmem_ld_wait();
  float v[32];
  if (p.bias != nullptr) {
#pragma unroll
    for (int j = 0; j < 8; ++j) {
      const float4 b = sbias ? *reinterpret_cast<const float4*>(sbias + n + 4 * j)
                             : __ldg(reinterpret_cast<const float4*>(p.bias + n) + j);
      v[4 * j + 0] = __uint_as_float(r[4 * j + 0]) + b.x;
      v[4 * j + 1] = __uint_as_float(r[4 * j + 1]) + b.y;
      v[4 * j + 2] = __uint_as_float(r[4 * j + 2]) + b.z;
      v[4 * j + 3] = __uint_as_float(r[4 * j + 3]) + b.w;
    }
  } else {
#pragma unroll
    for (int j = 0; j < 32; ++j) v[j] = __uint_as_float(r[j]);
  }
  if (p.act == YV6_ACT_RELU) {
#pragma unroll
    for (int j = 0; j < 32; ++j) v[j] = fmaxf(v[j], 0.f);
  } else if (p.act == YV6_ACT_SILU) {
    if (p.fast_act) {
#pragma unroll
      for (int j = 0; j < 32; ++j) {
        const float h = 0.5f * v[j];
        v[j] = fmaf(h, tanh_fast(h), h);
      }
    } else {
#pragma unroll
      for (int j = 0; j < 32; ++j) v[j] = v[j] * rcp_ftz(1.f + ex2_ftz(-1.4426950408889634f * v[j]));
    }
  } else if (p.act == YV6_ACT_SIGMOID) {
#pragma unroll
    for (int j = 0; j < 32; ++j) v[j] = rcp_ftz(1.f + ex2_ftz(-1.4426950408889634f * v[j]));
  }
  if (res_row != nullptr) {
#pragma unroll
    for (int j = 0; j < 4; ++j) {
      const uint32_t w[4] = {rq[j].x, rq[j].y, rq[j].z, rq[j].w};
#pragma unroll
      for (int k = 0; k < 4; ++k) {
        const __nv_bfloat162 b2 = *reinterpret_cast<const __nv_bfloat162*>(&w[k]);
        v[8 * j + 2 * k] = fmaf(p.alpha, __low2float(b2), v[8 * j + 2 * k]);
        v[8 * j + 2 * k + 1] = fmaf(p.alpha, __high2float(b2), v[8 * j + 2 * k + 1]);
      }
    }
  }
  if (F32) {
#pragma unroll
    for (int j = 0; j < 8; ++j) {
      const uint32_t a = base + ((((uint32_t)(unit0 + j)) ^ rxor) << 4);
      asm volatile("st.shared.v4.f32 [%0], {%1, %2, %3, %4};" ::"r"(a), "f"(v[4 * j]), "f"(v[4 * j + 1]), "f"(v[4 * j + 2]),
                   "f"(v[4 * j + 3])
                   : "memory");
    }
  } else {
#pragma unroll
    for (int j = 0; j < 4; ++j) {
      const uint32_t a = base + ((((uint32_t)(unit0 + j)) ^ rxor) << 4);
      asm volatile("st.shared.v4.b32 [%0], {%1, %2, %3, %4};" ::"r"(a), "r"(pack_bf16x2(v[8 * j + 0], v[8 * j + 1])),
                   "r"(pack_bf16x2(v[8 * j + 2], v[8 * j + 3])), "r"(pack_bf16x2(v[8 * j + 4], v[8 * j + 5])),
                   "r"(pack_bf16x2(v[8 * j + 6], v[8 * j + 7]))
                   : "memory");
    }
  }
}

template <int G, int MODE, bool CP>
__global__ void __launch_bounds__(64 + 128 * G, 1)
conv_igemm_kernel(const __grid_constant__ CUtensorMap tmA, const __grid_constant__ CUtensorMap tmB,
                  const __grid_constant__ CUtensorMap tmC, const ConvKParams p) {
  extern __shared__ uint8_t smem_raw[];
  const uint32_t raw_addr = smem_u32(smem_raw);
  uint8_t* smem = smem_raw + ((1024u - (raw_addr & 1023u)) & 1023u);
  uint8_t* sA = smem;
  uint8_t* sB = smem + (size_t)p.a_region_bytes;
  uint8_t* sC = sB + (size_t)p.b_region_bytes;
  float* sBiasBuf = reinterpret_cast<float*>(sC + kCBufCount * kCBufBytes);
  uint64_t* bars = reinterpret_cast<uint64_t*>(sC + kCBufCount * kCBufBytes + kBiasSmemFloats * sizeof(float));
  uint64_t* full = bars;
  uint64_t* empty = bars + kMaxStages;
  uint64_t* tfull = bars + 2 * kMaxStages;
  uint64_t* tempty = tfull + kMaxGroups;
  uint32_t* tmem_ptr = reinterpret_cast<uint32_t*>(tempty + kMaxGroups);
  uint64_t* a_full = tempty + kMaxGroups + 2;
  uint64_t* a_empty = a_full + kMaxAStages;
  uint64_t* b_full = a_empty + kMaxAStages;
  uint64_t* b_empty = b_full + kMaxBStages;

  const int warp = threadIdx.x >> 5;
  const int lane = threadIdx.x & 31;
  constexpr bool HALO = (MODE != 0);
  constexpr bool BRES = (MODE == 2 || MODE == 4);
  using HG = HaloGeom<(MODE >= 3)>;
  const int rank = CP ? (int)cluster_ctarank() : 0;
  const int unit0 = CP ? (int)(blockIdx.x >> 1) : (int)blockIdx.x;
  const int ustep = CP ? (int)(gridDim.x >> 1) : (int)gridDim.x;
  const bool leader = (rank == 0);
  if (threadIdx.x == 0) YV6_TRACE(0);

  if (warp == 0) {
    if (lane == 0) {
      tma_prefetch_desc(&tmA);
      tma_prefetch_desc(&tmB);
      if (p.tma_store) tma_prefetch_desc(&tmC);
    }
    constexpr int kBarSlots = 2 * kMaxStages + 2 * kMaxGroups + 2 + 2 * kMaxAStages + 2 * kMaxBStages;
    constexpr int kTemptyFirst = 2 * kMaxStages + kMaxGroups, kTmemSlot = 2 * kMaxStages + 2 * kMaxGroups;
    for (int i = lane; i < kBarSlots; i += 32) {
      if (i == kTmemSlot || i == kTmemSlot + 1) continue;
      const bool is_tempty = (i >= kTemptyFirst && i < kTemptyFirst + kMaxGroups);
      mbar_init(&bars[i], is_tempty ? (CP ? 8u : 128u) : 1u);
    }
    fence_mbar_init();
  }
  if (warp == 1) {
    if (CP) tmem_alloc_pair(tmem_ptr, (uint32_t)p.tmem_cols);
    else tmem_alloc(tmem_ptr, (uint32_t)p.tmem_cols);
  }
  tc_fence_before();
  if (CP) cluster_sync_all();
  else __syncthreads();
  tc_fence_after();
  const uint32_t tmem_base = *tmem_ptr;
  if (threadIdx.x == 0) YV6_TRACE(1);

  const int kblocks = p.npairs * p.taps * p.cin_blocks;

  if (warp == 0) {
    if constexpr (HALO) {
      int sa = 0, sb = 0;
      uint32_t pha = 0, phb = 0;
      bool first = true;
      const uint32_t a_tx = (uint32_t)HG::kBytes * (CP ? 2u : 1u), b_tx = (uint32_t)(p.b_rows * 128) * (CP ? 2u : 1u);
      const int nrow0 = rank * p.b_rows;
      for (int tile = unit0; tile < p.num_tiles; tile += ustep) {
        const TileCoord t = CP ? decode_unit(p, tile, rank) : decode_tile(p, tile);
        int slot = 0;
        for (int pi = 0; pi < p.npairs; ++pi) {
          const int pa = kPairA[6 - p.npairs + pi], pb = kPairB[6 - p.npairs + pi];
          for (int cb = 0; cb < p.cin_blocks; ++cb) {
            mbar_wait(&a_empty[sa], pha ^ 1);
            if (pi == 0 && cb == 0 && lane == 0) {
              if (tile == unit0 + 4 * ustep) YV6_TRACE(12);
              if (tile == unit0 + 8 * ustep) YV6_TRACE(13);
            }
            if (elect_one()) {
              if (leader) mbar_expect_tx(&a_full[sa], a_tx);
              if (CP) tma_load_5d_pair(sA + (size_t)sa * HG::kStageBytes, &tmA, &a_full[sa], cb * 64, t.w0 - 1, t.h0 * HG::SH - 1, t.i0, pa);
              else tma_load_5d(sA + (size_t)sa * HG::kStageBytes, &tmA, &a_full[sa], cb * 64, t.w0 - 1, t.h0 * HG::SH - 1, t.i0, pa);
            }
            __syncwarp();
            if (++sa == p.a_stages) { sa = 0; pha ^= 1; }
            for (int tap = 0; tap < HG::TAPS; ++tap) {
              if (HG::SH == 2 && (tap % HG::KW) == 0 && cb < p.skip_cb) continue;
              if constexpr (BRES) {
                if (first && elect_one()) {
                  if (leader) mbar_expect_tx(&b_full[slot], b_tx);
                  if (CP) tma_load_3d_pair(sB + (size_t)slot * p.b_stage_bytes, &tmB, &b_full[slot], tap * p.Cin + cb * 64, t.n0 + nrow0, pb);
                  else tma_load_3d(sB + (size_t)slot * p.b_stage_bytes, &tmB, &b_full[slot], tap * p.Cin + cb * 64, t.n0, pb);
                }
                __syncwarp();
              } else {
                mbar_wait(&b_empty[sb], phb ^ 1);
                if (elect_one()) {
                  if (leader) mbar_expect_tx(&b_full[sb], b_tx);
                  if (CP) tma_load_3d_pair(sB + (size_t)sb * p.b_stage_bytes, &tmB, &b_full[sb], tap * p.Cin + cb * 64, t.n0 + nrow0, pb);
                  else tma_load_3d(sB + (size_t)sb * p.b_stage_bytes, &tmB, &b_full[sb], tap * p.Cin + cb * 64, t.n0, pb);
                }
                __syncwarp();
                if (++sb == p.b_stages) { sb = 0; phb ^= 1; }
              }
              ++slot;
            }
          }
        }
        first = false;
      }
    } else {
    int stage = 0;
    uint32_t phase = 0;
    const uint32_t tx = (uint32_t)(p.rows * p.kb_bytes + p.b_rows * p.kb_bytes) * (CP ? 2u : 1u);
    const int nrow0 = rank * p.b_rows;
    for (int tile = unit0; tile < p.num_tiles; tile += ustep) {
      const TileCoord t = CP ? decode_unit(p, tile, rank) : decode_tile(p, tile);
      for (int pi = 0; pi < p.npairs; ++pi) {
        const int pa = kPairA[6 - p.npairs + pi], pb = kPairB[6 - p.npairs + pi];
        for (int tap = 0; tap < p.taps; ++tap) {
          const int r = tap / p.kw, s = tap - r * p.kw;
          const int cx = t.w0 * p.stride_w + s - p.pad_w;
          const int cy = t.h0 * p.stride + r - p.pad;
          for (int cb = 0; cb < p.cin_blocks; ++cb) {
            mbar_wait(&empty[stage], phase ^ 1);
            if (elect_one()) {
              if (leader) mbar_expect_tx(&full[stage], tx);
              if (CP) {
                tma_load_5d_pair(sA + (size_t)stage * p.a_stage_bytes, &tmA, &full[stage], cb * p.kb_elems, cx, cy, t.i0, pa);
                tma_load_3d_pair(sB + (size_t)stage * p.b_stage_bytes, &tmB, &full[stage], tap * p.Cin + cb * p.kb_elems,
                                 t.n0 + nrow0, pb);
              } else {
                tma_load_5d(sA + (size_t)stage * p.a_stage_bytes, &tmA, &full[stage], cb * p.kb_elems, cx, cy,
                            t.i0, pa);
                tma_load_3d(sB + (size_t)stage * p.b_stage_bytes, &tmB, &full[stage],
                            tap * p.Cin + cb * p.kb_elems, t.n0, pb);
              }
              if (tile == unit0 && pi == 0 && tap == 0 && cb == 0) YV6_TRACE(2);
            }
            __syncwarp();
            if (++stage == p.stages) {
              stage = 0;
              phase ^= 1;
            }
          }
        }
      }
    }
    }
  } else if (warp == 1 && leader) {
    const uint32_t idesc = umma_idesc_bf16(CP ? 256u : 128u, (uint32_t)p.BN);
    const uint64_t desc_const = umma_smem_desc(0, (uint32_t)p.sbo_bytes, (uint32_t)p.layout_type);
    const uint32_t a_base = (smem_u32(sA) & 0x3ffffu) >> 4, b_base = (smem_u32(sB) & 0x3ffffu) >> 4;
    auto mma = [&](uint32_t d, uint64_t ad, uint64_t bd, uint32_t accumulate) {
      if (CP) umma_bf16_pair(d, ad, bd, idesc, accumulate);
      else umma_bf16(d, ad, bd, idesc, accumulate);
    };
    auto commit = [&](uint64_t* bar) {
      if (CP) umma_commit_pair(bar);
      else umma_commit(bar);
    };
    const uint32_t a_step = (uint32_t)p.a_stage_bytes >> 4, b_step = (uint32_t)p.b_stage_bytes >> 4;
    int stage = 0;
    uint32_t phase = 0;
    int acc = 0;
    uint32_t acc_phase = 0;
    const int num_tiles = p.num_tiles, BN = p.BN, ksteps = p.ksteps, nstages = p.stages;
    const int a_stages = p.a_stages, b_stages = p.b_stages;
    constexpr bool b_resident = BRES;
    const int pcs = p.npairs * p.cin_blocks;
    if constexpr (HALO) {
      const uint64_t desc_a = umma_smem_desc(0, (uint32_t)(HG::W * 128 * HG::SH), 2u);
      const uint64_t desc_b = umma_smem_desc(0, 1024u, 2u);
      const uint32_t halo_step = (uint32_t)HG::kStageBytes >> 4;
      const int skip_cb = p.skip_cb, cin_blocks = p.cin_blocks;
      int sa = 0, sb = 0;
      uint32_t pha = 0, phb = 0;
      bool first = true;
      for (int tile = unit0; tile < num_tiles; tile += ustep) {
        mbar_wait(&tempty[acc], acc_phase ^ 1);
        tc_fence_after();
        const uint32_t d_tmem = tmem_base + (uint32_t)(acc * BN);
        int slot = 0;
        uint32_t started = 0;
        for (int pc = 0; pc < pcs; ++pc) {
          mbar_wait(&a_full[sa], pha);
          tc_fence_after();
          const uint32_t a0 = a_base + (uint32_t)sa * halo_step;
          const bool skip_s0 = (HG::SH == 2) && (pc % cin_blocks) < skip_cb;
#pragma unroll
          for (int tap = 0; tap < HG::TAPS; ++tap) {
            if (HG::SH == 2 && (tap % HG::KW) == 0 && skip_s0) continue;
            const int bs = b_resident ? slot : sb;
            if (!b_resident || first) {
              mbar_wait(&b_full[bs], b_resident ? 0u : phb);
              tc_fence_after();
            }
            const uint64_t ad = desc_a | (uint64_t)(a0 + (uint32_t)((tap / HG::KW) * HG::W + (tap % HG::KW)) * 8u);
            const uint64_t bd = desc_b | (uint64_t)(b_base + (uint32_t)bs * b_step);
            if (elect_one()) {
              mma(d_tmem, ad, bd, started);
              mma(d_tmem, ad + 2, bd + 2, 1u);
              mma(d_tmem, ad + 4, bd + 4, 1u);
              mma(d_tmem, ad + 6, bd + 6, 1u);
              if (!b_resident) commit(&b_empty[sb]);
            }
            __syncwarp();
            started = 1u;
            if (!b_resident && ++sb == b_stages) { sb = 0; phb ^= 1; }
            ++slot;
          }
          if (elect_one()) commit(&a_empty[sa]);
          __syncwarp();
          if (++sa == a_stages) { sa = 0; pha ^= 1; }
        }
        if (elect_one()) commit(&tfull[acc]);
        __syncwarp();
        if (lane == 0) {
          if (tile == unit0) YV6_TRACE(4);
          if (tile == unit0 + 4 * ustep) YV6_TRACE(14);
          if (tile == unit0 + 8 * ustep) YV6_TRACE(15);
        }
        first = false;
        if (++acc == G) { acc = 0; acc_phase ^= 1; }
      }
    } else
    for (int tile = unit0; tile < num_tiles; tile += ustep) {
      mbar_wait(&tempty[acc], acc_phase ^ 1);
      tc_fence_after();
      const uint32_t d_tmem = tmem_base + (uint32_t)(acc * BN);
      for (int kb = 0; kb < kblocks; ++kb) {
        mbar_wait(&full[stage], phase);
        tc_fence_after();
        if (kb == 0 && tile == unit0 && lane == 0) YV6_TRACE(3);
        const uint64_t ad = desc_const | (uint64_t)(a_base + (uint32_t)stage * a_step);
        const uint64_t bd = desc_const | (uint64_t)(b_base + (uint32_t)stage * b_step);
        if (elect_one()) {
          mma(d_tmem, ad, bd, (uint32_t)(kb != 0));
          if (ksteps > 1) mma(d_tmem, ad + 2, bd + 2, 1u);
          if (ksteps > 2) {
            mma(d_tmem, ad + 4, bd + 4, 1u);
            mma(d_tmem, ad + 6, bd + 6, 1u);
          }
          commit(&empty[stage]);
        }
        __syncwarp();
        if (++stage == nstages) {
          stage = 0;
          phase ^= 1;
        }
      }
      if (elect_one()) commit(&tfull[acc]);
      __syncwarp();
      if (tile == unit0 && lane == 0) YV6_TRACE(4);
      if (++acc == G) { acc = 0; acc_phase ^= 1; }
    }
  } else if (warp >= 2) {
    const int group = (warp - 2) >> 2;
    const int q = warp & 3;
    const int row = q * 32 + lane;
    const int bw = row % p.BW;
    const int tq = row / p.BW;
    const int bh = tq % p.BH;
    const int bi = tq / p.BH;
    constexpr int NBUF = kCBufCount / G;
    uint8_t* gC = sC + group * NBUF * kCBufBytes;
    const bool f32 = (p.y_dtype == YV6_DT_F32);
    const float* sbias = nullptr;
    if (p.bias_smem) {
      for (int i = (int)threadIdx.x - 64; i < p.tiles_n * p.BN; i += 128 * G) sBiasBuf[i] = __ldg(p.bias + i);
      asm volatile("bar.sync 7, %0;" ::"r"(128 * G) : "memory");
      sbias = sBiasBuf;
    }
    uint32_t acc_phase = 0;
    int cbuf = 0;
    for (int tile = unit0 + group * ustep; tile < p.num_tiles; tile += G * ustep) {
      const TileCoord t = CP ? decode_unit(p, tile, rank) : decode_tile(p, tile);
      const int img = t.i0 + bi, ho = t.h0 + bh, wo = t.w0 + bw;
      const bool valid = (row < p.rows) && (img < p.N) && (ho < p.Ho) && (wo < p.Wo);
      const int64_t off = (int64_t)img * p.y_img_stride + (int64_t)ho * p.y_h_stride +
                          (int64_t)wo * p.y_w_stride;
      const int64_t roff = (int64_t)img * p.res_img_stride + (int64_t)ho * p.res_h_stride +
                           (int64_t)wo * p.res_w_stride;
      const __nv_bfloat16* res_row = (p.res != nullptr && valid) ? p.res + roff : nullptr;
      const bool fast_tile = (p.out_planes == 1) && (p.res == nullptr || (p.res_planes == 1 && p.res_aligned));
      mbar_wait(&tfull[group], acc_phase);
      tc_fence_after();
      if (tile == unit0 && q == 0 && lane == 0) YV6_TRACE(5);
      const uint32_t taddr = tmem_base + ((uint32_t)(q * 32) << 16) + (uint32_t)(group * p.BN);
      if (p.tma_store == 2) {
        const int wrow0 = q * 32;
        const int sw0 = t.w0 + wrow0 % p.BW, sh0 = t.h0 + wrow0 / p.BW;
        const uint32_t lrow = (uint32_t)lane * 128u, lxor = (uint32_t)(lane & 7);
        for (int c0 = 0; c0 < p.BN; c0 += p.c_chunk) {
          const int nsub = min(p.c_chunk, p.BN - c0) >> 4;
          for (int pl = 0; pl < p.out_planes; ++pl) {
            uint8_t* buf = gC + cbuf * kCBufBytes + q * 4096;
            if (lane == 0) tma_store_wait_read<NBUF - 1>();
            __syncwarp();
            const uint32_t base = smem_u32(buf) + lrow;
            if (fast_tile && nsub * 16 == p.c_chunk) {
              if (f32) {
                epi_cols32<true>(p, sbias, taddr + (uint32_t)c0, t.n0 + c0, res_row, base, lxor, 0);
              } else {
                epi_cols32<false>(p, sbias, taddr + (uint32_t)c0, t.n0 + c0, res_row, base, lxor, 0);
                epi_cols32<false>(p, sbias, taddr + (uint32_t)(c0 + 32), t.n0 + c0 + 32, res_row, base, lxor, 4);
              }
            } else {
            uint32_t r[2][16];
            tmem_ld16(taddr + (uint32_t)c0, r[0]);
#pragma unroll 1
            for (int sb = 0; sb < 4; ++sb) {
              if (sb < nsub) {
                tmem_ld_wait();
                if (sb + 1 < nsub) tmem_ld16(taddr + (uint32_t)(c0 + 16 * (sb + 1)), r[(sb + 1) & 1]);
                const int n = t.n0 + c0 + 16 * sb;
                float v[16];
                epilogue_math(p, sbias, r[sb & 1], n, min(16, p.Cout - n), valid, roff, v);
                for (int k = 0; k < pl; ++k) {
#pragma unroll
                  for (int j = 0; j < 16; ++j) v[j] -= __bfloat162float(__float2bfloat16_rn(v[j]));
                }
                if (f32) {
#pragma unroll
                  for (int j = 0; j < 4; ++j) {
                    const uint32_t a = base + ((((uint32_t)(4 * sb + j)) ^ lxor) << 4);
                    asm volatile("st.shared.v4.f32 [%0], {%1, %2, %3, %4};" ::"r"(a), "f"(v[4 * j]), "f"(v[4 * j + 1]),
                                 "f"(v[4 * j + 2]), "f"(v[4 * j + 3])
                                 : "memory");
                  }
                } else {
#pragma unroll
                  for (int j = 0; j < 2; ++j) {
                    const uint32_t a = base + ((((uint32_t)(2 * sb + j)) ^ lxor) << 4);
                    asm volatile("st.shared.v4.b32 [%0], {%1, %2, %3, %4};" ::"r"(a),
                                 "r"(pack_bf16x2(v[8 * j + 0], v[8 * j + 1])), "r"(pack_bf16x2(v[8 * j + 2], v[8 * j + 3])),
                                 "r"(pack_bf16x2(v[8 * j + 4], v[8 * j + 5])), "r"(pack_bf16x2(v[8 * j + 6], v[8 * j + 7]))
                                 : "memory");
                  }
                }
              }
            }
            }
            fence_proxy_async_smem();
            __syncwarp();
            if (lane == 0) {
              tma_store_5d(&tmC, buf, t.n0 + c0, sw0, sh0, t.i0, pl);
              tma_store_commit();
            }
            if (++cbuf == NBUF) cbuf = 0;
          }
        }
      } else if (p.tma_store == 1) {
        const bool issuer = (((warp - 2) & 3) == 0 && lane == 0);
        const uint32_t row_smem = (uint32_t)row * 128u, row_xor = (uint32_t)(row & 7);
        for (int c0 = 0; c0 < p.BN; c0 += p.c_chunk) {
          const int nsub = min(p.c_chunk, p.BN - c0) >> 4;
          for (int pl = 0; pl < p.out_planes; ++pl) {
            uint8_t* buf = gC + cbuf * kCBufBytes;
            if (issuer) tma_store_wait_read<NBUF - 1>();
            epi_bar_sync(group);
            const uint32_t base = smem_u32(buf) + row_smem;
            if (fast_tile && nsub * 16 == p.c_chunk) {
              if (f32) {
                epi_cols32<true>(p, sbias, taddr + (uint32_t)c0, t.n0 + c0, res_row, base, row_xor, 0);
              } else {
                epi_cols32<false>(p, sbias, taddr + (uint32_t)c0, t.n0 + c0, res_row, base, row_xor, 0);
                epi_cols32<false>(p, sbias, taddr + (uint32_t)(c0 + 32), t.n0 + c0 + 32, res_row, base, row_xor, 4);
              }
            } else {
            uint32_t r[2][16];
            tmem_ld16(taddr + (uint32_t)c0, r[0]);
#pragma unroll 1
            for (int sb = 0; sb < 4; ++sb) {
              if (sb < nsub) {
                tmem_ld_wait();
                if (sb + 1 < nsub) tmem_ld16(taddr + (uint32_t)(c0 + 16 * (sb + 1)), r[(sb + 1) & 1]);
                const int n = t.n0 + c0 + 16 * sb;
                float v[16];
                epilogue_math(p, sbias, r[sb & 1], n, min(16, p.Cout - n), valid, roff, v);
                for (int k = 0; k < pl; ++k) {
#pragma unroll
                  for (int j = 0; j < 16; ++j) v[j] -= __bfloat162float(__float2bfloat16_rn(v[j]));
                }
                if (row < p.rows) {
                  if (f32) {
#pragma unroll
                    for (int j = 0; j < 4; ++j) {
                      const uint32_t a = base + ((((uint32_t)(4 * sb + j)) ^ row_xor) << 4);
                      asm volatile("st.shared.v4.f32 [%0], {%1, %2, %3, %4};" ::"r"(a), "f"(v[4 * j]), "f"(v[4 * j + 1]),
                                   "f"(v[4 * j + 2]), "f"(v[4 * j + 3])
                                   : "memory");
                    }
                  } else {
#pragma unroll
                    for (int j = 0; j < 2; ++j) {
                      const uint32_t a = base + ((((uint32_t)(2 * sb + j)) ^ row_xor) << 4);
                      asm volatile("st.shared.v4.b32 [%0], {%1, %2, %3, %4};" ::"r"(a),
                                   "r"(pack_bf16x2(v[8 * j + 0], v[8 * j + 1])), "r"(pack_bf16x2(v[8 * j + 2], v[8 * j + 3])),
                                   "r"(pack_bf16x2(v[8 * j + 4], v[8 * j + 5])), "r"(pack_bf16x2(v[8 * j + 6], v[8 * j + 7]))
                                   : "memory");
                    }
                  }
                }
              }
            }
            }
            fence_proxy_async_smem();
            epi_bar_sync(group);
            if (issuer) {
              tma_store_5d(&tmC, buf, t.n0 + c0, t.w0, t.h0, t.i0, pl);
              tma_store_commit();
            }
            if (++cbuf == NBUF) cbuf = 0;
          }
        }
      } else {
        for (int c0 = 0; c0 < p.BN; c0 += 16) {
          uint32_t r[16];
          tmem_ld16(taddr + (uint32_t)c0, r);
          tmem_ld_wait();
          const int n = t.n0 + c0;
          const int ncol = min(16, p.Cout - n);
          float v[16];
          epilogue_math(p, sbias, r, n, ncol, valid, roff, v);
          if (valid && ncol > 0) store_chunk(p, off, n, ncol, v);
        }
      }
      tc_fence_before();
      if (CP) {
        __syncwarp();
        if (lane == 0) mbar_arrive_leader(&tempty[group]);
      } else {
        mbar_arrive(&tempty[group]);
      }
      if (q == 0 && lane == 0) {
        if (tile == unit0) YV6_TRACE(6);
        if (tile == unit0 + 4 * ustep) YV6_TRACE(9);
        if (tile == unit0 + 8 * ustep) YV6_TRACE(10);
      }
      acc_phase ^= 1;
    }
    if (p.tma_store && lane == 0) asm volatile("cp.async.bulk.wait_group.read 0;" ::: "memory");
    if (group == 0 && q == 0 && lane == 0) YV6_TRACE(7);
  }

  tc_fence_before();
  if (CP) cluster_sync_all();
  else __syncthreads();
  if (warp == 1) {
    tc_fence_after();
    if (CP) tmem_dealloc_pair(tmem_base, (uint32_t)p.tmem_cols);
    else tmem_dealloc(tmem_base, (uint32_t)p.tmem_cols);
    if (lane == 0) YV6_TRACE(8);
  }
}

struct ConvPlan {
  ConvKParams k;
  int grid;
  size_t smem_bytes;
  CUtensorMapSwizzle swz;
};

static inline int ceil_div(int a, int b) { return (a + b - 1) / b; }

static int plan_conv(const yv6_handle* h, const yv6_conv_desc* d, ConvPlan* plan) {
  YV6_REQUIRE(d != nullptr, "conv: null descriptor");
  YV6_REQUIRE(d->x && d->w && d->y, "conv: null tensor pointer");
  YV6_REQUIRE(d->N > 0 && d->H > 0 && d->W > 0, "conv: bad input shape %dx%dx%d", d->N, d->H, d->W);
  YV6_REQUIRE(d->Cin > 0 && d->Cin % 16 == 0, "conv: Cin=%d must be a positive multiple of 16", d->Cin);
  YV6_REQUIRE(d->x_c_total >= d->Cin && d->x_c_total % 8 == 0, "conv: bad x_c_total=%d", d->x_c_total);
  YV6_REQUIRE(d->Cout > 0, "conv: Cout=%d", d->Cout);
  YV6_REQUIRE(d->kh >= 1 && d->kh <= 3 && d->kw >= 1 && d->kw <= 3, "conv: kernel %dx%d unsupported", d->kh, d->kw);
  YV6_REQUIRE(d->stride == 1 || d->stride == 2, "conv: stride %d unsupported", d->stride);
  YV6_REQUIRE(d->stride_w >= 0 && d->stride_w <= 2, "conv: stride_w %d unsupported", d->stride_w);
  const int stride_w = d->stride_w > 0 ? d->stride_w : d->stride;
  YV6_REQUIRE(d->nsplit == 1 || d->nsplit == 3, "conv: nsplit must be 1 or 3");
  YV6_REQUIRE((reinterpret_cast<uintptr_t>(d->x) & 15) == 0 && (reinterpret_cast<uintptr_t>(d->w) & 15) == 0,
              "conv: x / w must be 16-byte aligned");
  YV6_REQUIRE(d->y_dtype == YV6_DT_BF16 || d->y_dtype == YV6_DT_F32, "conv: bad y_dtype");

  ConvKParams& k = plan->k;
  memset(&k, 0, sizeof(k));
  k.N = d->N;
  const int pad_w = (d->pad_w == YV6_PAD_SAME) ? d->pad : d->pad_w;
  k.Ho = d->out_h > 0 ? d->out_h : (d->H + 2 * d->pad - d->kh) / d->stride + 1;
  k.Wo = d->out_w > 0 ? d->out_w : (d->W + 2 * pad_w - d->kw) / stride_w + 1;
  YV6_REQUIRE(k.Ho > 0 && k.Wo > 0, "conv: empty output");
  k.Cout = d->Cout;
  k.Cin = d->Cin;
  k.taps = d->kh * d->kw;
  k.kw = d->kw;
  k.stride = d->stride;
  k.stride_w = stride_w;
  k.pad = d->pad;
  k.pad_w = pad_w;

  k.kb_elems = (d->Cin % 64 == 0) ? 64 : (d->Cin % 32 == 0) ? 32 : 16;
  k.kb_bytes = k.kb_elems * 2;
  k.ksteps = k.kb_elems / 16;
  k.cin_blocks = d->Cin / k.kb_elems;
  k.sbo_bytes = 8 * k.kb_bytes;
  k.layout_type = (k.kb_bytes == 128) ? 2 : (k.kb_bytes == 64) ? 4 : 6;
  plan->swz = (k.kb_bytes == 128) ? CU_TENSOR_MAP_SWIZZLE_128B
              : (k.kb_bytes == 64) ? CU_TENSOR_MAP_SWIZZLE_64B
                                   : CU_TENSOR_MAP_SWIZZLE_32B;
  k.npairs = (d->nsplit == 3) ? 6 : 1;

  const int esz = (d->y_dtype == YV6_DT_F32) ? 4 : 2;
  k.c_chunk = 128 / esz;
  k.tma_store = (d->force_direct != 1) && ((d->y_w_stride * esz) % 16 == 0) && ((d->y_h_stride * esz) % 16 == 0) &&
                ((d->y_img_stride * esz) % 16 == 0) && ((d->y_plane_stride * esz) % 16 == 0) &&
                ((reinterpret_cast<uintptr_t>(d->y) & 15) == 0);
  const int bn_align = k.c_chunk;
  if (d->force_bw > 0) {
    k.BW = d->force_bw;
    k.BH = std::max(1, d->force_bh);
    k.BI = std::max(1, d->force_bi);
    YV6_REQUIRE(k.BW * k.BH * k.BI <= kTileRows && k.BW * stride_w <= 256 && k.BH * d->stride <= 256,
                "conv: forced tile %dx%dx%d invalid", k.BW, k.BH, k.BI);
  } else {
    long best_tiles = -1, best_box_tiles = -1;
    int bestw = 1, besth = 1, besti = 1, boxw = 0, boxh = 0;
    const int maxbw = std::min(std::min(k.Wo, kTileRows), 256 / stride_w);
    for (int bw = 1; bw <= maxbw; ++bw) {
      const int maxbh = std::min(std::min(k.Ho, kTileRows / bw), 256 / d->stride);
      for (int bh = 1; bh <= maxbh; ++bh) {
        int bi = 1;
        if (bw >= k.Wo && bh >= k.Ho) bi = std::max(1, std::min(d->N, kTileRows / (bw * bh)));
        long tiles = (long)ceil_div(k.Wo, bw) * ceil_div(k.Ho, bh) * ceil_div(d->N, bi);
        if (best_tiles < 0 || tiles < best_tiles || (tiles == best_tiles && bw > bestw)) {
          best_tiles = tiles;
          bestw = bw;
          besth = bh;
          besti = bi;
        }
      }
    }
    for (int bw = 1; bw <= std::min(kTileRows, 256 / stride_w); bw <<= 1) {
      const int bh = kTileRows / bw;
      if (bh * d->stride > 256) continue;
      long tiles = (long)ceil_div(k.Wo, bw) * ceil_div(k.Ho, bh) * d->N;
      if (best_box_tiles < 0 || tiles < best_box_tiles || (tiles == best_box_tiles && bw > boxw)) {
        best_box_tiles = tiles;
        boxw = bw;
        boxh = bh;
      }
    }
    if (best_box_tiles > 0 && best_box_tiles * 100 <= best_tiles * 108 && d->force_bi == 0) {
      bestw = boxw;
      besth = boxh;
      besti = 1;
    }
    k.BW = bestw;
    k.BH = besth;
    k.BI = besti;
  }
  k.halo = 0;
  if (d->kh == 3 && d->kw == 3 && d->stride == 1 && stride_w == 1 && d->pad == 1 && pad_w == 1 && d->out_h == 0 && d->out_w == 0 &&
      d->Cin % 64 == 0 && d->force_bw == 0 && d->force_halo >= 0) {
    const long generic = (long)ceil_div(k.Wo, k.BW) * ceil_div(k.Ho, k.BH) * ceil_div(d->N, k.BI);
    const long halo_tiles = (long)ceil_div(k.Wo, 8) * ceil_div(k.Ho, 16) * d->N;
    if (d->force_halo > 0 || halo_tiles * 4 <= generic * 5) {
      k.halo = 1;
      k.BW = 8;
      k.BH = 16;
      k.BI = 1;
    }
  }
  k.skip_cb = 0;
  if (d->kh == 3 && d->kw == 2 && d->stride == 2 && stride_w == 1 && d->pad == 1 && pad_w == 1 && d->out_w == d->W && d->out_h == 0 &&
      d->Cin % 64 == 0 && d->force_bw == 0 && d->force_halo >= 0 && d->H % 2 == 0) {
    const long generic = (long)ceil_div(k.Wo, k.BW) * ceil_div(k.Ho, k.BH) * ceil_div(d->N, k.BI);
    const long halo_tiles = (long)ceil_div(k.Wo, 8) * ceil_div(k.Ho, 16) * d->N;
    if (d->force_halo > 0 || (halo_tiles * 4 <= generic * 5 && d->Cin <= 256)) {
      k.halo = 2;
      k.BW = 8;
      k.BH = 16;
      k.BI = 1;
      if (d->pair_view && (d->Cin / 2) % 64 == 0) k.skip_cb = d->Cin / 128;
    }
  }
  const long m_tiles = (long)ceil_div(k.Wo, k.BW) * ceil_div(k.Ho, k.BH) * ceil_div(d->N, k.BI);
  if (d->force_bn > 0) {
    YV6_REQUIRE(d->force_bn % 16 == 0 && d->force_bn <= 256, "conv: force_bn must be a multiple of 16 <= 256");
    k.BN = d->force_bn;
  } else {
    double best_cost = -1;
    int best_bn = 0;
    const int nt_min = ceil_div(d->Cout, 256);
    for (int nt = nt_min; nt <= nt_min * 4; ++nt) {
      int bn = ceil_div(ceil_div(d->Cout, nt), 16) * 16;
      if (nt > 1) bn = ceil_div(bn, bn_align) * bn_align;
      if (bn > 256 || (nt > 1 && bn < 64)) continue;
      const long tiles = m_tiles * ceil_div(d->Cout, bn);
      const double waves = (double)ceil_div((int)std::min<long>(tiles, 1l << 30), h->num_sms);
      const double cost = waves * (bn + 48.0);
      if (best_cost < 0 || cost < best_cost - 1e-9) {
        best_cost = cost;
        best_bn = bn;
      }
    }
    k.BN = best_bn;
  }
  YV6_REQUIRE(k.BN >= 16, "conv: could not choose BN for Cout=%d", d->Cout);
  k.tiles_n = ceil_div(d->Cout, k.BN);
  if (k.tiles_n > 1 && k.tma_store && (k.BN % bn_align) != 0) k.tma_store = 0;
  k.rows = k.BW * k.BH * k.BI;
  if (k.tma_store && k.rows == kTileRows && k.BI == 1 && (32 % k.BW == 0 || k.BW % 32 == 0) && d->force_direct != 2)
    k.tma_store = 2;
  k.tiles_w = ceil_div(k.Wo, k.BW);
  k.tiles_h = ceil_div(k.Ho, k.BH);
  k.tiles_i = ceil_div(d->N, k.BI);
  YV6_REQUIRE(m_tiles * k.tiles_n < (1l << 30), "conv: too many tiles");
  k.m_tiles = (int)m_tiles;
  const bool pair_auto = (d->kh == 3 && d->kw == 3 && d->stride == 1 && stride_w == 1 && d->Cin >= 128 && d->Cout <= d->Cin) ||
                         (k.halo == 2 && d->Cout >= 128);
  k.cpair = (m_tiles >= 2 && h->max_clusters > 0 && (d->force_pair > 0 || (d->force_pair == 0 && pair_auto))) ? 1 : 0;
  k.b_rows = k.cpair ? k.BN / 2 : k.BN;
  k.num_tiles = k.cpair ? (int)(((m_tiles + 1) / 2) * k.tiles_n) : (int)(m_tiles * k.tiles_n);

  k.a_stage_bytes = kTileRows * k.kb_bytes;
  k.b_stage_bytes = ((k.b_rows * k.kb_bytes + 1023) / 1024) * 1024;
  const int budget = h->max_smem_optin - 1024 - 1024 - kCBufCount * kCBufBytes - kBiasSmemFloats * (int)sizeof(float);
  if (k.halo) {
    const int halo_stage = (k.halo == 2) ? HaloGeom<true>::kStageBytes : HaloGeom<false>::kStageBytes;
    const int min_a = (k.halo == 2) ? 2 : 3;
    const int b_tiles = (k.halo == 2) ? k.npairs * (k.cin_blocks * 6 - 3 * k.skip_cb) : k.npairs * k.cin_blocks * 9;
    k.b_resident = (k.tiles_n == 1 && b_tiles <= kMaxBStages && d->force_stages == 0 &&
                    (long)b_tiles * k.b_stage_bytes + min_a * halo_stage <= budget) ? 1 : 0;
    if (k.b_resident) {
      k.b_stages = b_tiles;
      k.a_stages = std::min(kMaxAStages, (budget - b_tiles * k.b_stage_bytes) / halo_stage);
    } else {
      k.a_stages = (k.halo == 1 && budget - 3 * halo_stage >= 3 * k.b_stage_bytes) ? 3 : 2;
      k.b_stages = std::min(kMaxBStages, (budget - k.a_stages * halo_stage) / k.b_stage_bytes);
      if (d->force_stages > 0) k.b_stages = std::min(k.b_stages, std::max(2, d->force_stages));
    }
    YV6_REQUIRE(k.a_stages >= 2 && k.b_stages >= 2, "conv(halo): not enough shared memory");
    k.stages = k.b_stages;
    k.a_region_bytes = k.a_stages * halo_stage;
    k.b_region_bytes = k.b_stages * k.b_stage_bytes;
  } else {
    const int stage_bytes = k.a_stage_bytes + k.b_stage_bytes;
    int stages = std::min(kMaxStages, budget / stage_bytes);
    if (d->force_stages > 0) stages = std::min(stages, d->force_stages);
    YV6_REQUIRE(stages >= 2, "conv: not enough shared memory for a 2-stage pipeline");
    k.stages = stages;
    k.a_region_bytes = stages * k.a_stage_bytes;
    k.b_region_bytes = stages * k.b_stage_bytes;
  }
  k.trace = reinterpret_cast<unsigned long long*>(d->trace);
  plan->smem_bytes = (size_t)k.a_region_bytes + k.b_region_bytes + kCBufCount * kCBufBytes + kBiasSmemFloats * sizeof(float) + 1024 + 1024;

  const int kblocks_per_tile = k.npairs * k.taps * k.cin_blocks;
  k.groups = (4 * k.BN <= 512 && kblocks_per_tile <= 8 && d->force_groups != 2) ? 4 : 2;
  if (d->force_groups == 4 && 4 * k.BN <= 512) k.groups = 4;
  int cols = 32;
  while (cols < k.groups * k.BN) cols *= 2;
  k.tmem_cols = cols;

  k.act = d->act;
  k.y_dtype = d->y_dtype;
  k.bias_smem = (d->bias != nullptr && k.tiles_n * k.BN <= kBiasSmemFloats) ? 1 : 0;
  k.fast_act = (d->y_dtype == YV6_DT_BF16 && d->nsplit != 3) ? 1 : 0;
  k.res_aligned = (d->res != nullptr && (reinterpret_cast<uintptr_t>(d->res) & 15) == 0 && d->res_img_stride % 8 == 0 &&
                   d->res_h_stride % 8 == 0 && d->res_w_stride % 8 == 0) ? 1 : 0;
  k.out_planes = (d->nsplit == 3 && d->y_dtype == YV6_DT_BF16) ? 3 : 1;
  k.res_planes = (d->nsplit == 3) ? 3 : 1;
  k.y = d->y;
  k.y_img_stride = d->y_img_stride;
  k.y_h_stride = d->y_h_stride;
  k.y_w_stride = d->y_w_stride;
  k.y_plane_stride = d->y_plane_stride;
  k.res = reinterpret_cast<const __nv_bfloat16*>(d->res);
  k.alpha = d->alpha;
  k.res_img_stride = d->res_img_stride;
  k.res_h_stride = d->res_h_stride;
  k.res_w_stride = d->res_w_stride;
  k.res_plane_stride = d->res_plane_stride;
  k.bias = d->bias;

  if (k.cpair) {
    int clusters = std::min(k.num_tiles, h->max_clusters);
    if (d->force_grid > 0) clusters = std::min(k.num_tiles, std::max(1, d->force_grid / 2));
    plan->grid = 2 * clusters;
  } else {
    plan->grid = std::min(k.num_tiles, h->num_sms);
    if (d->force_grid > 0) plan->grid = std::min(k.num_tiles, d->force_grid);
  }
  return YV6_OK;
}

}

using namespace yv6;

using ConvKernelFn = void (*)(const CUtensorMap, const CUtensorMap, const CUtensorMap, const ConvKParams);
static const ConvKernelFn kConvKernels[2][2][5] = {
    {{conv_igemm_kernel<2, 0, false>, conv_igemm_kernel<2, 1, false>, conv_igemm_kernel<2, 2, false>, conv_igemm_kernel<2, 3, false>,
      conv_igemm_kernel<2, 4, false>},
     {conv_igemm_kernel<4, 0, false>, conv_igemm_kernel<4, 1, false>, conv_igemm_kernel<4, 2, false>, conv_igemm_kernel<4, 3, false>,
      conv_igemm_kernel<4, 4, false>}},
    {{conv_igemm_kernel<2, 0, true>, conv_igemm_kernel<2, 1, true>, conv_igemm_kernel<2, 2, true>, conv_igemm_kernel<2, 3, true>,
      conv_igemm_kernel<2, 4, true>},
     {conv_igemm_kernel<4, 0, true>, conv_igemm_kernel<4, 1, true>, conv_igemm_kernel<4, 2, true>, conv_igemm_kernel<4, 3, true>,
      conv_igemm_kernel<4, 4, true>}}};

static int conv_configure(yv6_handle* h) {
  if (h->configured & YV6_CFG_CONV) return YV6_OK;
  for (int c = 0; c < 2; ++c)
    for (int g = 0; g < 2; ++g)
      for (int m = 0; m < 5; ++m)
        YV6_CHECK_CUDA(cudaFuncSetAttribute(kConvKernels[c][g][m], cudaFuncAttributeMaxDynamicSharedMemorySize, (int)h->max_smem_optin));
  cudaLaunchConfig_t cfg;
  memset(&cfg, 0, sizeof(cfg));
  cfg.gridDim = dim3((unsigned)(2 * h->num_sms));
  cfg.blockDim = dim3(64 + 128 * 2);
  cfg.dynamicSmemBytes = 200 * 1024;
  cudaLaunchAttribute attr[1];
  attr[0].id = cudaLaunchAttributeClusterDimension;
  attr[0].val.clusterDim.x = 2;
  attr[0].val.clusterDim.y = 1;
  attr[0].val.clusterDim.z = 1;
  cfg.attrs = attr;
  cfg.numAttrs = 1;
  int n = 0;
  const cudaError_t e = cudaOccupancyMaxActiveClusters(&n, kConvKernels[1][0][1], &cfg);
  if (e != cudaSuccess) {
    (void)cudaGetLastError();
    n = 0;
  }
  h->max_clusters = std::min(n, h->num_sms / 2);
  h->configured |= YV6_CFG_CONV;
  return YV6_OK;
}

extern "C" int yv6_conv_plan(yv6_handle* h, const yv6_conv_desc* d, int32_t* out8) {
  yv6_device_guard _dev(h);
  YV6_REQUIRE(h != nullptr && out8 != nullptr, "conv_plan: null argument");
  { const int rc0 = conv_configure(h); if (rc0 != YV6_OK) return rc0; }
  ConvPlan plan;
  int rc = plan_conv(h, d, &plan);
  if (rc != YV6_OK) return rc;
  out8[0] = plan.k.BW;
  out8[1] = plan.k.BH;
  out8[2] = plan.k.BI;
  out8[3] = plan.k.BN;
  out8[4] = plan.k.kb_elems;
  out8[5] = plan.k.stages;
  out8[6] = plan.grid;
  out8[7] = plan.k.num_tiles;
  out8[8] = plan.k.halo;
  out8[9] = (plan.k.halo ? plan.k.a_stages * 100 + plan.k.b_resident : 0) + 10 * plan.k.cpair;
  return YV6_OK;
}

extern "C" int yv6_conv_plan_host(int num_sms, int max_smem_optin, int max_clusters, const yv6_conv_desc* d, int32_t* out12) {
  YV6_REQUIRE(out12 != nullptr, "conv_plan_host: null argument");
  YV6_REQUIRE(num_sms > 0 && max_smem_optin > 0 && max_clusters >= 0, "conv_plan_host: bad device properties");
  yv6_handle fake;
  memset(&fake, 0, sizeof(fake));
  fake.device = -1;
  fake.num_sms = num_sms;
  fake.max_smem_optin = max_smem_optin;
  fake.max_clusters = max_clusters;
  ConvPlan plan;
  int rc = plan_conv(&fake, d, &plan);
  if (rc != YV6_OK) return rc;
  YV6_REQUIRE(plan.smem_bytes <= (size_t)max_smem_optin, "conv_plan_host: plan needs %zu bytes of shared memory, device offers %d",
              plan.smem_bytes, max_smem_optin);
  YV6_REQUIRE(plan.k.tmem_cols <= 512, "conv_plan_host: plan needs %d TMEM columns", plan.k.tmem_cols);
  out12[0] = plan.k.BW;
  out12[1] = plan.k.BH;
  out12[2] = plan.k.BI;
  out12[3] = plan.k.BN;
  out12[4] = plan.k.kb_elems;
  out12[5] = plan.k.stages;
  out12[6] = plan.grid;
  out12[7] = plan.k.num_tiles;
  out12[8] = plan.k.halo;
  out12[9] = (plan.k.halo ? plan.k.a_stages * 100 + plan.k.b_resident : 0) + 10 * plan.k.cpair;
  out12[10] = (int32_t)plan.smem_bytes;
  out12[11] = plan.k.tmem_cols;
  return YV6_OK;
}

extern "C" int yv6_conv_fwd(yv6_handle* h, const yv6_conv_desc* d, void* stream) {
  yv6_device_guard _dev(h);
  YV6_REQUIRE(h != nullptr, "conv_fwd: null handle");
  { const int rc0 = conv_configure(h); if (rc0 != YV6_OK) return rc0; }
  ConvPlan plan;
  int rc = plan_conv(h, d, &plan);
  if (rc != YV6_OK) return rc;
  const ConvKParams& k = plan.k;
  YV6_REQUIRE(h->encode_tiled != nullptr, "conv_fwd: cuTensorMapEncodeTiled unavailable (no CUDA driver?)");

  CUtensorMap tmA, tmB, tmC;
  {
    const uint64_t planes = (d->nsplit == 3) ? 3 : 1;
    cuuint64_t dims[5] = {(cuuint64_t)d->Cin, (cuuint64_t)d->W, (cuuint64_t)d->H, (cuuint64_t)d->N, planes};
    const uint64_t pix = (uint64_t)d->x_c_total * 2;
    uint64_t plane_stride = (d->nsplit == 3) ? (uint64_t)d->x_plane_stride * 2
                                             : (uint64_t)d->N * d->H * d->W * pix;
    YV6_REQUIRE(plane_stride % 16 == 0, "conv: x_plane_stride must be a multiple of 8 elements");
    cuuint64_t strides[4] = {pix, pix * d->W, pix * d->W * d->H, plane_stride};
    cuuint32_t box[5] = {(cuuint32_t)k.kb_elems, (cuuint32_t)(k.BW * k.stride_w), (cuuint32_t)(k.BH * d->stride),
                         (cuuint32_t)k.BI, 1};
    cuuint32_t estr[5] = {1, (cuuint32_t)k.stride_w, (cuuint32_t)d->stride, 1, 1};
    if (k.halo) {
      box[1] = (k.halo == 2) ? HaloGeom<true>::W : HaloGeom<false>::W;
      box[2] = (k.halo == 2) ? HaloGeom<true>::H : HaloGeom<false>::H;
      estr[1] = estr[2] = 1;
    }
    CUresult cr = h->encode_tiled(&tmA, CU_TENSOR_MAP_DATA_TYPE_BFLOAT16, 5, const_cast<void*>(d->x), dims,
                                  strides, box, estr, CU_TENSOR_MAP_INTERLEAVE_NONE, plan.swz,
                                  CU_TENSOR_MAP_L2_PROMOTION_L2_256B, CU_TENSOR_MAP_FLOAT_OOB_FILL_NONE);
    if (cr != CUDA_SUCCESS) {
      yv6_set_error("conv: cuTensorMapEncodeTiled(A) failed with %d (C=%d W=%d H=%d N=%d box=%u,%u,%u,%u)", (int)cr,
                    d->Cin, d->W, d->H, d->N, box[0], box[1], box[2], box[3]);
      return YV6_ERR_CUDA;
    }
  }
  {
    const uint64_t planes = (d->nsplit == 3) ? 3 : 1;
    const uint64_t ktot = (uint64_t)k.taps * d->Cin;
    cuuint64_t dims[3] = {ktot, (cuuint64_t)d->Cout, planes};
    uint64_t plane_stride = (d->nsplit == 3) ? (uint64_t)d->w_plane_stride * 2 : ktot * 2 * d->Cout;
    YV6_REQUIRE(plane_stride % 16 == 0, "conv: w_plane_stride must be a multiple of 8 elements");
    cuuint64_t strides[2] = {ktot * 2, plane_stride};
    cuuint32_t box[3] = {(cuuint32_t)k.kb_elems, (cuuint32_t)k.b_rows, 1};
    cuuint32_t estr[3] = {1, 1, 1};
    CUresult cr = h->encode_tiled(&tmB, CU_TENSOR_MAP_DATA_TYPE_BFLOAT16, 3, const_cast<void*>(d->w), dims,
                                  strides, box, estr, CU_TENSOR_MAP_INTERLEAVE_NONE, plan.swz,
                                  CU_TENSOR_MAP_L2_PROMOTION_L2_256B, CU_TENSOR_MAP_FLOAT_OOB_FILL_NONE);
    if (cr != CUDA_SUCCESS) {
      yv6_set_error("conv: cuTensorMapEncodeTiled(B) failed with %d", (int)cr);
      return YV6_ERR_CUDA;
    }
  }

  if (k.tma_store) {
    const uint64_t esz = (d->y_dtype == YV6_DT_F32) ? 4 : 2;
    const uint64_t planes = (uint64_t)k.out_planes;
    cuuint64_t dims[5] = {(cuuint64_t)d->Cout, (cuuint64_t)k.Wo, (cuuint64_t)k.Ho, (cuuint64_t)d->N, planes};
    uint64_t plane_stride = (planes > 1) ? (uint64_t)d->y_plane_stride * esz : (uint64_t)d->y_img_stride * esz * d->N;
    if (plane_stride == 0) plane_stride = 16;
    cuuint64_t strides[4] = {(uint64_t)d->y_w_stride * esz, (uint64_t)d->y_h_stride * esz,
                             (uint64_t)d->y_img_stride * esz, plane_stride};
    cuuint32_t box[5] = {(cuuint32_t)k.c_chunk, (cuuint32_t)k.BW, (cuuint32_t)k.BH, (cuuint32_t)k.BI, 1};
    if (k.tma_store == 2) {
      box[1] = (cuuint32_t)std::min(k.BW, 32);
      box[2] = (cuuint32_t)std::max(1, 32 / k.BW);
    }
    cuuint32_t estr[5] = {1, 1, 1, 1, 1};
    CUresult cr = h->encode_tiled(&tmC, esz == 4 ? CU_TENSOR_MAP_DATA_TYPE_FLOAT32 : CU_TENSOR_MAP_DATA_TYPE_BFLOAT16,
                                  5, d->y, dims, strides, box, estr, CU_TENSOR_MAP_INTERLEAVE_NONE,
                                  CU_TENSOR_MAP_SWIZZLE_128B, CU_TENSOR_MAP_L2_PROMOTION_NONE,
                                  CU_TENSOR_MAP_FLOAT_OOB_FILL_NONE);
    if (cr != CUDA_SUCCESS) {
      yv6_set_error("conv: cuTensorMapEncodeTiled(C) failed with %d (Cout=%d Wo=%d Ho=%d N=%d strides=%llu,%llu,%llu)",
                    (int)cr, d->Cout, k.Wo, k.Ho, d->N, (unsigned long long)strides[0],
                    (unsigned long long)strides[1], (unsigned long long)strides[2]);
      return YV6_ERR_CUDA;
    }
  } else {
    tmC = tmA;
  }

  const int mode = k.halo ? (k.halo == 2 ? 3 : 1) + (k.b_resident ? 1 : 0) : 0;
  ConvKernelFn fn = kConvKernels[k.cpair][k.groups == 4 ? 1 : 0][mode];
  cudaLaunchConfig_t cfg;
  memset(&cfg, 0, sizeof(cfg));
  cfg.gridDim = dim3((unsigned)plan.grid);
  cfg.blockDim = dim3((unsigned)(64 + 128 * k.groups));
  cfg.dynamicSmemBytes = plan.smem_bytes;
  cfg.stream = (cudaStream_t)stream;
  cudaLaunchAttribute attr[1];
  if (k.cpair) {
    attr[0].id = cudaLaunchAttributeClusterDimension;
    attr[0].val.clusterDim.x = 2;
    attr[0].val.clusterDim.y = 1;
    attr[0].val.clusterDim.z = 1;
    cfg.attrs = attr;
    cfg.numAttrs = 1;
  }
  YV6_CHECK_CUDA(cudaLaunchKernelEx(&cfg, fn, tmA, tmB, tmC, k));
  YV6_CHECK_CUDA(cudaGetLastError());
  return YV6_OK;
}
```

### yolov6_b200/engine.py

```python
import ctypes as C
import os

import numpy as np
import torch

from . import _lib, ops
from ._lib import ACT_CODES, DT_BF16, DT_F32, DT_U8, ConvDesc, StemDesc
from .fold import fold_op


def _split3(t):
    t = t.float()
    p0 = t.to(torch.bfloat16)
    r1 = t - p0.float()
    p1 = r1.to(torch.bfloat16)
    p2 = (r1 - p1.float()).to(torch.bfloat16)
    return torch.stack([p0, p1, p2])


class InferEngine:
    def __init__(self, graph, state_dict, device, precision="bf16"):
        if device.type != "cuda":
            raise RuntimeError("yolov6_b200 runs its networks on sm_100a CUDA kernels only (no CPU fallback); "
                               f"got device {device}")
        assert precision in ("bf16", "fp32")
        self.g = graph
        self.device = device
        self.precision = precision
        self.nsplit = 3 if precision == "fp32" else 1
        self.handle = _lib.handle(device.index or 0)
        self.lib = _lib.lib()
        self.fuse_siblings = True
        self.n_lanes = int(os.environ.get("YV6_LANES", "4"))
        self.force_pair = -1 if os.environ.get("YV6_PAIR", "1") == "0" else 0
        self._side = None
        self.weights = {}
        self._plans = {}
        self.max_plans = 4
        self._pinned = set()
        self._pack(state_dict)

    def _siblings(self):
        pairs = {}
        ops = self.g.ops
        for i, a in enumerate(ops):
            if a.kind != "conv" or not a.name.startswith("detect.cls_convs."):
                continue
            for j in range(i + 1, min(i + 3, len(ops))):
                b = ops[j]
                if (b.kind == "conv" and b.name == a.name.replace("cls_convs", "reg_convs") and b.src == a.src and
                        (b.k, b.s, b.act, b.cout, b.cin) == (a.k, a.s, a.act, a.cout, a.cin) and a.res is None and b.res is None and
                        a.dst.c_off == 0 and b.dst.c_off == 0 and a.cout % 64 == 0):
                    pairs[i] = j
        return pairs

    def _pack(self, sd):
        sd = {k: v.detach().cpu() for k, v in sd.items()}
        dev = self.device
        self.sibling = self._siblings() if self.fuse_siblings else {}
        self.sibling_second = {j: i for i, j in self.sibling.items()}
        for i, op in enumerate(self.g.ops):
            if op.kind == "pool" or (op.kind == "pred" and op.head[0] not in ("cls", "reg")):
                continue
            w, b = fold_op(sd, op)
            ent = {}
            if op.kind == "stem":
                ent["w_dev"] = w.float().permute(1, 2, 3, 0).contiguous().to(dev)
                ent["b_dev"] = b.float().contiguous().to(dev)
            else:
                ws = w if isinstance(w, list) else [w]
                packed = []
                for wi in ws:
                    wi = wi.float().to(dev)
                    packed.append(_split3(wi).contiguous() if self.nsplit == 3 else wi.to(torch.bfloat16).contiguous())
                ent["w"] = packed
                if op.kind == "conv" and op.k == 3 and op.s == 2 and (op.cin <= 32 or op.cin in (64, 128)):
                    wf = ops.pair_view_weights(ws[0].float()).to(dev)
                    ent["w_pair"] = _split3(wf).contiguous() if self.nsplit == 3 else wf.to(torch.bfloat16).contiguous()
                bias = torch.zeros((op.cout + 255) // 256 * 256, dtype=torch.float32, device=dev)
                bias[:op.cout] = b.float().to(dev)
                ent["bias"] = bias
            ent["alpha"] = float(sd[op.alpha]) if (op.alpha and op.res is not None) else 1.0
            self.weights[i] = ent
        for i, j in self.sibling.items():
            (wa, ba), (wb, bb) = fold_op(sd, self.g.ops[i]), fold_op(sd, self.g.ops[j])
            wf = torch.cat([wa, wb], 0).float().to(dev)
            c2 = wf.shape[0]
            bias = torch.zeros((c2 + 255) // 256 * 256, dtype=torch.float32, device=dev)
            bias[:c2] = torch.cat([ba, bb]).float().to(dev)
            self.weights[i]["w_fused"] = _split3(wf).contiguous() if self.nsplit == 3 else wf.to(torch.bfloat16).contiguous()
            self.weights[i]["bias_fused"] = bias

    def _plan(self, N, H, W, in_dtype):
        key = (N, H, W, in_dtype)
        if key in self._plans:
            plan = self._plans.pop(key)
            self._plans[key] = plan
            return plan
        while len(self._plans) >= self.max_plans:
            victim = next((k for k in self._plans if k not in self._pinned), None)
            if victim is None:
                break
            del self._plans[victim]
        g, dev, P = self.g, self.device, self.nsplit
        maxs = max(g.strides)
        if H % maxs or W % maxs:
            raise RuntimeError(f"input {H}x{W} must be a multiple of the largest stride {maxs}")
        plan = {"bufs": [], "calls": [], "conv_info": [], "deps": [], "pred_descs": [], "head_set": 0}
        for b in g.bufs:
            h, w = H >> b.level, W >> b.level
            shape = (P, N, h, w, b.c_total) if P == 3 else (N, h, w, b.c_total)
            plan["bufs"].append(torch.zeros(shape, dtype=torch.bfloat16, device=dev))
        sizes = [(H // s, W // s) for s in g.strides]
        offs = np.concatenate([[0], np.cumsum([h * w for h, w in sizes])]).astype(int)
        A = int(offs[-1])
        nc, R = g.num_classes, 4 * (g.reg_max + 1)
        plan["cls"] = torch.empty(N, A, nc, dtype=torch.float32, device=dev)
        plan["reg"] = torch.empty(N, A, R, dtype=torch.float32, device=dev)
        plan["pred"] = torch.empty(N, A, 5 + nc, dtype=torch.float32, device=dev)
        plan["sizes"], plan["A"] = sizes, A
        plan["lvl_h"] = (C.c_int32 * len(sizes))(*[h for h, _ in sizes])
        plan["lvl_w"] = (C.c_int32 * len(sizes))(*[w for _, w in sizes])
        plan["lvl_s"] = (C.c_float * len(sizes))(*[float(s) for s in g.strides])
        plan["image"] = None

        redirect = {}
        plan["fused_bufs"] = []
        for i, j in self.sibling.items():
            a, b2 = g.ops[i], g.ops[j]
            lvl = g.bufs[a.dst.buf].level
            h, w = H >> lvl, W >> lvl
            shape = (P, N, h, w, 2 * a.cout) if P == 3 else (N, h, w, 2 * a.cout)
            fb = torch.zeros(shape, dtype=torch.bfloat16, device=dev)
            plan["fused_bufs"].append(fb)
            redirect[a.dst.buf] = (fb, 0, 2 * a.cout)
            redirect[b2.dst.buf] = (fb, a.cout, 2 * a.cout)

        def view(t):
            b = g.bufs[t.buf]
            h, w = H >> b.level, W >> b.level
            if t.buf in redirect:
                fb, coff, pitch = redirect[t.buf]
                return fb, h, w, pitch
            return plan["bufs"][t.buf], h, w, b.c_total

        def coff(t):
            return t.c_off + (redirect[t.buf][1] if t.buf in redirect else 0)

        def span(t):
            return (id(view(t)[0]), coff(t), coff(t) + t.c)

        for i, op in enumerate(g.ops):
            ent = self.weights.get(i)
            if op.kind == "stem":
                buf, h, w, ct = view(op.dst)
                d = StemDesc()
                d.x_dtype = DT_U8 if in_dtype == torch.uint8 else DT_F32
                d.in_scale = 1.0 / 255.0
                d.N, d.H, d.W = N, H, W
                d.w = ent["w_dev"].data_ptr()
                d.bias = ent["b_dev"].data_ptr()
                d.Cout, d.act = op.cout, ACT_CODES[op.act]
                d.y = buf.data_ptr()
                d.y_plane_stride = buf.stride(0) if P == 3 else 0
                d.nsplit = P
                plan["stem"] = d
                plan["calls"].append(("stem", d))
                plan["deps"].append(dict(reads=[], writes=[span(op.dst)]))
            elif op.kind in ("conv", "pred", "convT"):
                if op.kind == "pred" and op.head[0] not in ("cls", "reg"):
                    continue
                if i in self.sibling_second:
                    continue
                sbuf, sh, sw, sct = view(op.src)
                quads = ent["w"] if op.kind == "convT" else [ent["w"][0]]
                fused = i in self.sibling
                for q, wq in enumerate(quads):
                    d = ConvDesc()
                    d.x = sbuf.data_ptr() + coff(op.src) * 2
                    d.N, d.H, d.W, d.Cin, d.x_c_total = N, sh, sw, op.cin, sct
                    d.x_plane_stride = sbuf.stride(0) if P == 3 else 0
                    if fused:
                        wq = ent["w_fused"]
                    d.w = wq.data_ptr()
                    d.w_plane_stride = wq.stride(0) if P == 3 else 0
                    d.bias = (ent["bias_fused"] if fused else ent["bias"]).data_ptr()
                    d.Cout = op.cout * (2 if fused else 1)
                    d.kh = d.kw = 1 if op.kind == "convT" else op.k
                    d.stride = 1 if op.kind == "convT" else op.s
                    d.pad = d.kh // 2
                    d.pad_w = _lib.PAD_SAME
                    d.act = ACT_CODES[op.act]
                    d.nsplit = P
                    d.force_pair = self.force_pair
                    oh, ow = (sh + 2 * d.pad - d.kh) // d.stride + 1, (sw + 2 * d.pad - d.kw) // d.stride + 1
                    plan["conv_info"].append(dict(name=op.name if op.kind != "convT" else f"{op.name}[{q}]", cin=op.cin, cout=int(d.Cout),
                                                  k=d.kh, s=d.stride, ho=oh, wo=ow, h=sh, w=sw,
                                                  flops=2.0 * N * oh * ow * d.Cout * op.cin * d.kh * d.kw,
                                                  y_f32=op.kind == "pred"))
                    if op.kind == "pred":
                        which, lvl = op.head
                        out = plan[which]
                        ch = out.shape[2]
                        lh, lw = sizes[lvl]
                        d.y = out.data_ptr() + int(offs[lvl]) * ch * 4
                        plan["pred_descs"].append((d, which, int(offs[lvl]) * ch * 4))
                        d.y_dtype = DT_F32
                        d.y_img_stride, d.y_h_stride, d.y_w_stride = A * ch, lw * ch, ch
                    else:
                        dbuf, dh, dw, dct = view(op.dst)
                        d.y_dtype = DT_BF16
                        d.y_plane_stride = dbuf.stride(0) if P == 3 else 0
                        if op.kind == "convT":
                            dy, dx = q // 2, q % 2
                            d.y = dbuf.data_ptr() + ((dy * dw + dx) * dct + op.dst.c_off) * 2
                            d.y_img_stride, d.y_h_stride, d.y_w_stride = dh * dw * dct, 2 * dw * dct, 2 * dct
                        else:
                            d.y = dbuf.data_ptr() + (coff(op.dst) if not fused else 0) * 2
                            d.y_img_stride, d.y_h_stride, d.y_w_stride = dh * dw * dct, dw * dct, dct
                    if op.res is not None:
                        rbuf, rh, rw, rct = view(op.res)
                        d.res = rbuf.data_ptr() + coff(op.res) * 2
                        d.res_img_stride, d.res_h_stride, d.res_w_stride = rh * rw * rct, rw * rct, rct
                        d.res_plane_stride = rbuf.stride(0) if P == 3 else 0
                        d.alpha = ent["alpha"]
                    if "w_pair" in ent and op.src.c_off == 0 and sct == op.cin and sw % 2 == 0:
                        keep = (d.W, d.Cin, d.x_c_total, d.w, d.w_plane_stride, d.kw, d.stride_w, d.pad_w, d.out_w)
                        d.W, d.Cin, d.x_c_total = sw // 2, 2 * op.cin, 2 * op.cin
                        d.w = ent["w_pair"].data_ptr()
                        d.w_plane_stride = ent["w_pair"].stride(0) if P == 3 else 0
                        d.kw, d.stride_w, d.pad_w, d.out_w = 2, 1, 1, sw // 2
                        d.pair_view = 1
                        out10 = (C.c_int32 * 10)()
                        _lib.check(self.lib.yv6_conv_plan(self.handle, C.byref(d), out10))
                        if op.cin > 32 and out10[8] != 2:
                            d.W, d.Cin, d.x_c_total, d.w, d.w_plane_stride, d.kw, d.stride_w, d.pad_w, d.out_w = keep
                            d.pair_view = 0
                    if "neck_start" not in plan and op.name.startswith("neck."):
                        plan["neck_start"] = len(plan["calls"])
                    plan["calls"].append(("conv", d))
                    reads = [span(op.src)] + ([span(op.res)] if op.res is not None else [])
                    if op.kind == "pred":
                        writes = [(("head",) + tuple(op.head), 0, 1)]
                    elif fused:
                        writes = [(id(dbuf), 0, 2 * op.cout)]
                    else:
                        writes = [span(op.dst)]
                    plan["deps"].append(dict(reads=reads, writes=writes))
            elif op.kind == "pool":
                buf, h, w, ct = view(op.dst)
                plan["calls"].append(("pool", (buf.data_ptr(), N, h, w, op.cin, ct, P, buf.stride(0) if P == 3 else 0)))
                plan["deps"].append(dict(reads=[(id(buf), 0, op.cin)], writes=[(id(buf), op.cin, 4 * op.cin)]))
        self._schedule(plan)
        self._plans[key] = plan
        return plan

    def _schedule(self, plan):
        K = self.n_lanes
        deps = plan["deps"]
        n = len(deps)
        writers = {}
        lane, waits = [0] * n, [[] for _ in range(n)]
        last_on = [-1] * K
        for i, dp in enumerate(deps):
            prod = set()
            for key, lo, hi in dp["reads"]:
                for wlo, whi, j in writers.get(key, ()):
                    if wlo < hi and lo < whi:
                        prod.add(j)
            chain = [lane[j] for j in prod if last_on[lane[j]] == j]
            if chain:
                s = min(chain)
            elif not prod:
                s = 0
            else:
                s = min(range(K), key=lambda t: last_on[t])
            lane[i] = s
            waits[i] = sorted(j for j in prod if lane[j] != s)
            last_on[s] = i
            for key, lo, hi in dp["writes"]:
                writers.setdefault(key, []).append((lo, hi, i))
        need = set(j for w in waits for j in w)
        tails = [last_on[t] for t in range(1, K) if last_on[t] >= 0]
        need.update(tails)
        plan["lane"], plan["waits"], plan["tails"] = lane, waits, tails
        plan["events"] = {j: torch.cuda.Event() for j in need}
        plan["fork"] = torch.cuda.Event()

    def pin(self, N, H, W, in_dtype=torch.float32):
        self._plan(N, H, W, in_dtype)
        self._pinned.add((N, H, W, in_dtype))

    def launch_count(self, N, H, W, in_dtype=torch.float32):
        return len(self._plan(N, H, W, in_dtype)["calls"]) + 1

    def _select_head_set(self, plan, k):
        if k == plan["head_set"]:
            return
        if k == 1 and "cls_alt" not in plan:
            plan["cls_alt"], plan["reg_alt"] = torch.empty_like(plan["cls"]), torch.empty_like(plan["reg"])
        for d, which, off in plan["pred_descs"]:
            d.y = plan[which + ("_alt" if k == 1 else "")].data_ptr() + off
        plan["head_set"] = k

    def forward(self, x, stream=None, decode=True, head_set=0, hook=None):
        if x.device != self.device:
            raise RuntimeError(f"input on {x.device}, engine on {self.device}")
        if x.dtype not in (torch.float32, torch.uint8):
            x = x.float()
        x = x.contiguous()
        N, Cin, H, W = x.shape
        assert Cin == 3
        plan = self._plan(N, H, W, x.dtype)
        plan["image"] = x
        assert head_set == 0 or not decode, "the alternate head set is for decode=False callers"
        self._select_head_set(plan, head_set)
        main = stream if stream is not None else torch.cuda.current_stream(self.device)
        sp = _lib.stream_ptr(main)
        lib, h, chk = self.lib, self.handle, _lib.check
        plan["stem"].x = x.data_ptr()
        lane, waits, events = plan["lane"], plan["waits"], plan["events"]
        multi = self.n_lanes > 1 and max(lane) > 0
        if multi:
            if self._side is None:
                self._side = [torch.cuda.Stream(device=self.device) for _ in range(self.n_lanes - 1)]
            streams = [main] + self._side
            sps = [_lib.stream_ptr(t) for t in streams]
            plan["fork"].record(main)
            forked = set()
        for i, (kind, d) in enumerate(plan["calls"]):
            if hook is not None and i == hook[0]:
                hook[1]()
            if multi:
                t = lane[i]
                if t and t not in forked:
                    streams[t].wait_event(plan["fork"])
                    forked.add(t)
                for j in waits[i]:
                    streams[t].wait_event(events[j])
                sp = sps[t]
            if kind == "conv":
                chk(lib.yv6_conv_fwd(h, C.byref(d), sp))
            elif kind == "stem":
                chk(lib.yv6_stem_fwd(h, C.byref(d), sp))
            else:
                chk(lib.yv6_sppf_pool(h, C.c_void_p(d[0]), d[1], d[2], d[3], d[4], d[5], d[6], d[7], sp))
            if multi and i in events:
                events[i].record(streams[lane[i]])
        if multi:
            for j in plan["tails"]:
                main.wait_event(events[j])
            sp = sps[0]
        g = self.g
        if not decode:
            if head_set == 1:
                return plan["cls_alt"], plan["reg_alt"], plan["sizes"]
            return plan["cls"], plan["reg"], plan["sizes"]
        chk(lib.yv6_head_decode(h, C.c_void_p(plan["cls"].data_ptr()), C.c_void_p(plan["reg"].data_ptr()),
                                C.c_void_p(plan["pred"].data_ptr()), N, g.num_classes, 4 * (g.reg_max + 1),
                                len(g.strides), plan["lvl_h"], plan["lvl_w"], plan["lvl_s"], sp))
        return plan["pred"]

    def head_outputs(self, N, H, W, in_dtype=torch.float32):
        plan = self._plan(N, H, W, in_dtype)
        return plan["cls"], plan["reg"]

    def feature_maps(self, N, H, W, in_dtype=torch.float32):
        plan = self._plan(N, H, W, in_dtype)
        out = []
        for t in self.g.feat:
            buf = plan["bufs"][t.buf]
            buf = buf[0] if self.nsplit == 3 else buf
            out.append(buf[..., t.c_off:t.c_off + t.c].permute(0, 3, 1, 2))
        return out

    def profile_convs(self, x, steps=5, stream=None):
        x = x.contiguous()
        N, _, H, W = x.shape
        plan = self._plan(N, H, W, x.dtype if x.dtype == torch.uint8 else torch.float32)
        self.forward(x, stream)
        torch.cuda.synchronize()
        sp = _lib.stream_ptr(stream)
        convs = [d for kind, d in plan["calls"] if kind == "conv"]
        flops = sum(ci["flops"] for ci in plan["conv_info"])
        total_ms = 0.0
        for _ in range(steps):
            e0, e1 = torch.cuda.Event(enable_timing=True), torch.cuda.Event(enable_timing=True)
            e0.record()
            for d in convs:
                _lib.check(self.lib.yv6_conv_fwd(self.handle, C.byref(d), sp))
            e1.record()
            torch.cuda.synchronize()
            total_ms += e0.elapsed_time(e1)
        return total_ms / steps, flops, len(convs)

    def conv_bytes_per_launch(self, N, H, W):
        plan = self._plan(N, H, W, torch.float32)
        tot, n = 0.0, 0
        for ci in plan["conv_info"]:
            ysz = 4 if ci["y_f32"] else 2
            tot += N * (ci["h"] * ci["w"] * ci["cin"] * 2 + ci["ho"] * ci["wo"] * ci["cout"] * ysz) + ci["cout"] * ci["k"] ** 2 * ci["cin"] * 2
            n += 1
        return tot / max(n, 1)

    def profile_layers(self, x, iters=10, stream=None):
        x = x.contiguous()
        N, _, H, W = x.shape
        plan = self._plan(N, H, W, x.dtype if x.dtype == torch.uint8 else torch.float32)
        self.forward(x, stream)
        torch.cuda.synchronize()
        sp = _lib.stream_ptr(stream)
        flush = torch.empty(256 << 20, dtype=torch.uint8, device=self.device)
        rows = []
        convs = [d for kind, d in plan["calls"] if kind == "conv"]
        for ci, d in zip(plan["conv_info"], convs):
            name = ci["name"]
            ts = []
            for _ in range(iters):
                flush.zero_()
                e0, e1 = torch.cuda.Event(enable_timing=True), torch.cuda.Event(enable_timing=True)
                e0.record()
                _lib.check(self.lib.yv6_conv_fwd(self.handle, C.byref(d), sp))
                e1.record()
                torch.cuda.synchronize()
                ts.append(e0.elapsed_time(e1))
            ts.sort()
            ms = ts[len(ts) // 2]
            ho, wo = ci["ho"], ci["wo"]
            fl = ci["flops"]
            by = 2.0 * d.N * (ci["h"] * ci["w"] * ci["cin"] + ho * wo * ci["cout"])
            out = (C.c_int32 * 10)()
            _lib.check(self.lib.yv6_conv_plan(self.handle, C.byref(d), out))
            rows.append(dict(name=name, cin=ci["cin"], cout=ci["cout"], k=ci["k"], s=ci["s"], hw=f"{ho}x{wo}", ms=ms,
                             tflops=fl / ms / 1e9, gbs=by / ms / 1e6, plan=list(out)))
        return rows
```

Baseline: 16240.

## Fuse stem conv into the following stride-2 conv's A-operand producer

Adds a new kernel mode in which extra producer warps load image patches with cp.async and compute the 3x3 stem conv with mma.sync. They write the bf16 activations straight into the A-operand shared-memory stages of the next stride-2 conv, which runs on tcgen05. This removes the stem launch and the full-resolution stem activation round-trip through global memory. The costs are extra threads, a second patch buffer in shared memory, fewer A stages, stem halo recomputation across tiles, and a fixed group count of 2. The fused path is on by default when the shapes match.

```diff
diff --git a/include/yv6.h b/include/yv6.h
--- a/include/yv6.h
+++ b/include/yv6.h
@@ -77,6 +77,8 @@
 } yv6_stem_desc;
 int yv6_stem_fwd(yv6_handle* h, const yv6_stem_desc* d, void* stream);
 
+int yv6_stem_conv_fwd(yv6_handle* h, const yv6_stem_desc* s, const yv6_conv_desc* cd, void* stream);
+
 int yv6_sppf_pool(yv6_handle* h, void* buf, int32_t N, int32_t H, int32_t W, int32_t C, int32_t c_total,
                   int32_t nsplit, int64_t plane_stride, void* stream);
 
diff --git a/yolov6_b200/_lib.py b/yolov6_b200/_lib.py
--- a/yolov6_b200/_lib.py
+++ b/yolov6_b200/_lib.py
@@ -117,6 +117,7 @@
     "yv6_conv_plan": (C.c_int, [C.c_void_p, C.POINTER(ConvDesc), C.POINTER(C.c_int32)]),
     "yv6_conv_plan_host": (C.c_int, [C.c_int, C.c_int, C.c_int, C.POINTER(ConvDesc), C.POINTER(C.c_int32)]),
     "yv6_stem_fwd": (C.c_int, [C.c_void_p, C.POINTER(StemDesc), C.c_void_p]),
+    "yv6_stem_conv_fwd": (C.c_int, [C.c_void_p, C.POINTER(StemDesc), C.POINTER(ConvDesc), C.c_void_p]),
     "yv6_sppf_pool": (C.c_int, [C.c_void_p, C.c_void_p, C.c_int32, C.c_int32, C.c_int32, C.c_int32, C.c_int32,
                                 C.c_int32, C.c_int64, C.c_void_p]),
     "yv6_head_decode": (C.c_int, [C.c_void_p, C.c_void_p, C.c_void_p, C.c_void_p, C.c_int32, C.c_int32, C.c_int32,
diff --git a/yolov6_b200/csrc/yv6_aux.cu b/yolov6_b200/csrc/yv6_aux.cu
--- a/yolov6_b200/csrc/yv6_aux.cu
+++ b/yolov6_b200/csrc/yv6_aux.cu
@@ -248,16 +248,6 @@
     __syncwarp();
   }
 }
-
-__device__ __forceinline__ void cp_async16(void* dst, const void* src, int src_bytes) {
-  asm volatile("cp.async.cg.shared.global [%0], [%1], 16, %2;" ::"r"(smem_u32(dst)), "l"(src), "r"(src_bytes) : "memory");
-}
-__device__ __forceinline__ void cp_async4(void* dst, const void* src, int src_bytes) {
-  asm volatile("cp.async.ca.shared.global [%0], [%1], 4, %2;" ::"r"(smem_u32(dst)), "l"(src), "r"(src_bytes) : "memory");
-}
-__device__ __forceinline__ void cp_async_commit() { asm volatile("cp.async.commit_group;" ::: "memory"); }
-template <int N>
-__device__ __forceinline__ void cp_async_wait() { asm volatile("cp.async.wait_group %0;" ::"n"(N) : "memory"); }
 
 template <int COUT>
 __global__ void __launch_bounds__(256, 2) stem_mma_async_kernel(const StemParams p) {
diff --git a/yolov6_b200/csrc/yv6_common.cuh b/yolov6_b200/csrc/yv6_common.cuh
--- a/yolov6_b200/csrc/yv6_common.cuh
+++ b/yolov6_b200/csrc/yv6_common.cuh
@@ -119,6 +119,16 @@
       : "memory");
 }
 
+__device__ __forceinline__ void cp_async16(void* dst, const void* src, int src_bytes) {
+  asm volatile("cp.async.cg.shared.global [%0], [%1], 16, %2;" ::"r"(smem_u32(dst)), "l"(src), "r"(src_bytes) : "memory");
+}
+__device__ __forceinline__ void cp_async4(void* dst, const void* src, int src_bytes) {
+  asm volatile("cp.async.ca.shared.global [%0], [%1], 4, %2;" ::"r"(smem_u32(dst)), "l"(src), "r"(src_bytes) : "memory");
+}
+__device__ __forceinline__ void cp_async_commit() { asm volatile("cp.async.commit_group;" ::: "memory"); }
+template <int N>
+__device__ __forceinline__ void cp_async_wait() { asm volatile("cp.async.wait_group %0;" ::"n"(N) : "memory"); }
+
 __device__ __forceinline__ void tc_fence_before() {
   asm volatile("tcgen05.fence::before_thread_sync;" ::: "memory");
 }
diff --git a/yolov6_b200/csrc/yv6_conv_igemm.cu b/yolov6_b200/csrc/yv6_conv_igemm.cu
--- a/yolov6_b200/csrc/yv6_conv_igemm.cu
+++ b/yolov6_b200/csrc/yv6_conv_igemm.cu
@@ -37,6 +37,11 @@
   int32_t res_aligned;
   int32_t fast_act;
   unsigned long long* trace;
+  const void* img;
+  const float* stem_w;
+  const float* stem_b;
+  int32_t img_H, img_W, img_u8, stem_act, stem_Ho;
+  float in_scale;
 };
 #define YV6_TRACE(slot) do { if (p.trace != nullptr && blockIdx.x == 0) p.trace[slot] = (unsigned long long)clock64(); } while (0)
 
@@ -169,6 +174,11 @@
 
 constexpr int kBiasSmemFloats = 1024;
 
+constexpr int kStemWarps = 8;
+constexpr int kStemCBufs = 2;
+constexpr int kPatchRows = 67, kPatchPitch = 40;
+constexpr int kPatchBytes = 3 * kPatchRows * kPatchPitch * 4;
+
 __device__ __forceinline__ float ex2_ftz(float x) {
   float y;
   asm("ex2.approx.ftz.f32 %0, %1;" : "=f"(y) : "f"(x));
@@ -317,18 +327,163 @@
   }
 }
 
+__device__ __forceinline__ void stem_bar_sync() {
+  asm volatile("bar.sync 8, %0;" ::"n"(32 * kStemWarps) : "memory");
+}
+
+template <bool U8>
+__device__ __forceinline__ void stem_box_producer(const ConvKParams& p, int tid, uint8_t* sA, uint8_t* sPatch, uint64_t* a_full,
+                                                  uint64_t* a_empty, int unit0, int ustep) {
+  constexpr int PR = kPatchRows, PW = kPatchPitch, ESZ = U8 ? 1 : 4, NT = 4, COUT = 32;
+  constexpr int BOXW = 18, NPIX = HaloGeom<true>::H * BOXW, MTILES = (NPIX + 15) / 16;
+  constexpr int CHUNKS = PW / 4, ITEMS = 3 * PR * CHUNKS;
+  const int warp = tid >> 5, lane = tid & 31, g = lane >> 2, t = lane & 3;
+
+  uint32_t bfrag[NT][2][2];
+#pragma unroll
+  for (int nt = 0; nt < NT; ++nt)
+#pragma unroll
+    for (int ks = 0; ks < 2; ++ks)
+#pragma unroll
+      for (int h2 = 0; h2 < 2; ++h2) {
+        const int k = ks * 16 + h2 * 8 + 2 * t, nn = nt * 8 + g;
+        const float w0 = (k < 27) ? __ldg(p.stem_w + k * COUT + nn) : 0.f;
+        const float w1 = (k + 1 < 27) ? __ldg(p.stem_w + (k + 1) * COUT + nn) : 0.f;
+        bfrag[nt][ks][h2] = pack_bf16x2(w0, w1);
+      }
+  float bias[NT][2];
+#pragma unroll
+  for (int nt = 0; nt < NT; ++nt) {
+    bias[nt][0] = p.stem_b ? __ldg(p.stem_b + nt * 8 + 2 * t) : 0.f;
+    bias[nt][1] = p.stem_b ? __ldg(p.stem_b + nt * 8 + 2 * t + 1) : 0.f;
+  }
+  int koff[2][2][2];
+#pragma unroll
+  for (int ks = 0; ks < 2; ++ks)
+#pragma unroll
+    for (int h2 = 0; h2 < 2; ++h2)
+#pragma unroll
+      for (int e = 0; e < 2; ++e) {
+        const int k = ks * 16 + h2 * 8 + 2 * t + e;
+        const int tap = k / 3, c = k - 3 * tap, r = tap / 3, sx = tap - 3 * r;
+        koff[ks][h2][e] = (k < 27) ? (c * PR + r) * PW + sx : -1;
+      }
+
+  auto issue = [&](int tile, int slot) {
+    if (tile < p.num_tiles) {
+      const TileCoord tc = decode_tile(p, tile);
+      const int hi0 = 4 * tc.h0 - 3, wc0 = 4 * tc.w0 - 8;
+      uint8_t* dst0 = sPatch + slot * kPatchBytes;
+      for (int item = tid; item < ITEMS; item += 32 * kStemWarps) {
+        const int rc = item / CHUNKS, q = item - rc * CHUNKS;
+        const int c = rc / PR, hi = hi0 + (rc - c * PR), col = wc0 + 4 * q;
+        const bool ok = hi >= 0 && hi < p.img_H && col >= 0 && col < p.img_W;
+        const int64_t off = ok ? (((int64_t)tc.i0 * 3 + c) * p.img_H + hi) * p.img_W + col : 0;
+        const uint8_t* src = static_cast<const uint8_t*>(p.img) + off * ESZ;
+        uint8_t* dst = dst0 + (rc * PW + 4 * q) * ESZ;
+        if (U8) cp_async4(dst, src, ok ? 4 : 0);
+        else cp_async16(dst, src, ok ? 16 : 0);
+      }
+    }
+    cp_async_commit();
+  };
+  auto patch_bf16x2 = [&](const uint8_t* P, int i0, int i1) {
+    float v0 = 0.f, v1 = 0.f;
+    if (U8) {
+      if (i0 >= 0) v0 = (float)P[i0] * p.in_scale;
+      if (i1 >= 0) v1 = (float)P[i1] * p.in_scale;
+    } else {
+      const float* F = reinterpret_cast<const float*>(P);
+      if (i0 >= 0) v0 = F[i0];
+      if (i1 >= 0) v1 = F[i1];
+    }
+    return pack_bf16x2(v0, v1);
+  };
+
+  issue(unit0, 0);
+  int slot = 0, sa = 0;
+  uint32_t pha = 0;
+  for (int tile = unit0; tile < p.num_tiles; tile += ustep) {
+    cp_async_wait<0>();
+    stem_bar_sync();
+    issue(tile + ustep, slot ^ 1);
+    const TileCoord tc = decode_tile(p, tile);
+    const int gy0 = 2 * tc.h0 - 1, gv0 = tc.w0 - 1;
+    const uint8_t* P = sPatch + slot * kPatchBytes;
+    mbar_wait(&a_empty[sa], pha ^ 1);
+    const uint32_t abase = smem_u32(sA) + (uint32_t)(sa * HaloGeom<true>::kStageBytes);
+    for (int mt = warp; mt < MTILES; mt += kStemWarps) {
+      int base[2];
+#pragma unroll
+      for (int e = 0; e < 2; ++e) {
+        const int pix = min(16 * mt + g + 8 * e, NPIX - 1);
+        const int a = pix / BOXW, b = pix - a * BOXW;
+        base[e] = 2 * a * PW + 2 * b + 3;
+      }
+      float acc[NT][4];
+#pragma unroll
+      for (int nt = 0; nt < NT; ++nt)
+#pragma unroll
+        for (int j = 0; j < 4; ++j) acc[nt][j] = 0.f;
+#pragma unroll
+      for (int ks = 0; ks < 2; ++ks) {
+        uint32_t af[4];
+#pragma unroll
+        for (int h2 = 0; h2 < 2; ++h2) {
+          const int o0 = koff[ks][h2][0], o1 = koff[ks][h2][1];
+          af[2 * h2 + 0] = patch_bf16x2(P, o0 >= 0 ? base[0] + o0 : -1, o1 >= 0 ? base[0] + o1 : -1);
+          af[2 * h2 + 1] = patch_bf16x2(P, o0 >= 0 ? base[1] + o0 : -1, o1 >= 0 ? base[1] + o1 : -1);
+        }
+#pragma unroll
+        for (int nt = 0; nt < NT; ++nt) {
+          asm volatile(
+              "mma.sync.aligned.m16n8k16.row.col.f32.bf16.bf16.f32 {%0,%1,%2,%3}, {%4,%5,%6,%7}, {%8,%9}, {%0,%1,%2,%3};"
+              : "+f"(acc[nt][0]), "+f"(acc[nt][1]), "+f"(acc[nt][2]), "+f"(acc[nt][3])
+              : "r"(af[0]), "r"(af[1]), "r"(af[2]), "r"(af[3]), "r"(bfrag[nt][ks][0]), "r"(bfrag[nt][ks][1]));
+        }
+      }
+#pragma unroll
+      for (int e = 0; e < 2; ++e) {
+        const int pix = 16 * mt + g + 8 * e;
+        if (pix >= NPIX) continue;
+        const int a = pix / BOXW, b = pix - a * BOXW;
+        const int R = a * HaloGeom<true>::W + (b >> 1);
+        const bool inside = (unsigned)(gy0 + a) < (unsigned)p.stem_Ho && (unsigned)(gv0 + (b >> 1)) < (unsigned)p.Wo;
+        const uint32_t row = abase + (uint32_t)R * 128u + 4u * (uint32_t)t;
+#pragma unroll
+        for (int nt = 0; nt < NT; ++nt) {
+          const float v0 = act_apply(acc[nt][2 * e] + bias[nt][0], p.stem_act);
+          const float v1 = act_apply(acc[nt][2 * e + 1] + bias[nt][1], p.stem_act);
+          const uint32_t w = inside ? pack_bf16x2(v0, v1) : 0u;
+          const uint32_t unit = (uint32_t)(((b & 1) * 4 + nt) ^ (R & 7));
+          asm volatile("st.shared.b32 [%0], %1;" ::"r"(row + (unit << 4)), "r"(w) : "memory");
+        }
+      }
+    }
+    fence_proxy_async_smem();
+    __syncwarp();
+    if (lane == 0) mbar_arrive(&a_full[sa]);
+    if (++sa == p.a_stages) { sa = 0; pha ^= 1; }
+    slot ^= 1;
+  }
+  cp_async_wait<0>();
+}
+
 template <int G, int MODE, bool CP>
-__global__ void __launch_bounds__(64 + 128 * G, 1)
+__global__ void __launch_bounds__(64 + 128 * G + (MODE == 5 ? 32 * kStemWarps : 0), 1)
 conv_igemm_kernel(const __grid_constant__ CUtensorMap tmA, const __grid_constant__ CUtensorMap tmB,
                   const __grid_constant__ CUtensorMap tmC, const ConvKParams p) {
+  constexpr bool STEM = (MODE == 5);
+  constexpr int CBUFS = STEM ? kStemCBufs : kCBufCount;
   extern __shared__ uint8_t smem_raw[];
   const uint32_t raw_addr = smem_u32(smem_raw);
   uint8_t* smem = smem_raw + ((1024u - (raw_addr & 1023u)) & 1023u);
   uint8_t* sA = smem;
   uint8_t* sB = smem + (size_t)p.a_region_bytes;
   uint8_t* sC = sB + (size_t)p.b_region_bytes;
-  float* sBiasBuf = reinterpret_cast<float*>(sC + kCBufCount * kCBufBytes);
-  uint64_t* bars = reinterpret_cast<uint64_t*>(sC + kCBufCount * kCBufBytes + kBiasSmemFloats * sizeof(float));
+  float* sBiasBuf = reinterpret_cast<float*>(sC + CBUFS * kCBufBytes);
+  uint64_t* bars = reinterpret_cast<uint64_t*>(sC + CBUFS * kCBufBytes + kBiasSmemFloats * sizeof(float));
+  uint8_t* sPatch = reinterpret_cast<uint8_t*>(bars) + 1024;
   uint64_t* full = bars;
   uint64_t* empty = bars + kMaxStages;
   uint64_t* tfull = bars + 2 * kMaxStages;
@@ -342,7 +497,7 @@
   const int warp = threadIdx.x >> 5;
   const int lane = threadIdx.x & 31;
   constexpr bool HALO = (MODE != 0);
-  constexpr bool BRES = (MODE == 2 || MODE == 4);
+  constexpr bool BRES = (MODE == 2 || MODE == 4 || MODE == 5);
   using HG = HaloGeom<(MODE >= 3)>;
   const int rank = CP ? (int)cluster_ctarank() : 0;
   const int unit0 = CP ? (int)(blockIdx.x >> 1) : (int)blockIdx.x;
@@ -361,7 +516,8 @@
     for (int i = lane; i < kBarSlots; i += 32) {
       if (i == kTmemSlot || i == kTmemSlot + 1) continue;
       const bool is_tempty = (i >= kTemptyFirst && i < kTemptyFirst + kMaxGroups);
-      mbar_init(&bars[i], is_tempty ? (CP ? 8u : 128u) : 1u);
+      const bool is_stem_afull = STEM && (i >= kTmemSlot + 2 && i < kTmemSlot + 2 + kMaxAStages);
+      mbar_init(&bars[i], is_tempty ? (CP ? 8u : 128u) : is_stem_afull ? (uint32_t)kStemWarps : 1u);
     }
     fence_mbar_init();
   }
@@ -391,6 +547,7 @@
         for (int pi = 0; pi < p.npairs; ++pi) {
           const int pa = kPairA[6 - p.npairs + pi], pb = kPairB[6 - p.npairs + pi];
           for (int cb = 0; cb < p.cin_blocks; ++cb) {
+            if constexpr (!STEM) {
             mbar_wait(&a_empty[sa], pha ^ 1);
             if (pi == 0 && cb == 0 && lane == 0) {
               if (tile == unit0 + 4 * ustep) YV6_TRACE(12);
@@ -403,6 +560,7 @@
             }
             __syncwarp();
             if (++sa == p.a_stages) { sa = 0; pha ^= 1; }
+            }
             for (int tap = 0; tap < HG::TAPS; ++tap) {
               if (HG::SH == 2 && (tap % HG::KW) == 0 && cb < p.skip_cb) continue;
               if constexpr (BRES) {
@@ -427,6 +585,7 @@
           }
         }
         first = false;
+        if (STEM) break;
       }
     } else {
     int stage = 0;
@@ -574,6 +733,12 @@
       if (tile == unit0 && lane == 0) YV6_TRACE(4);
       if (++acc == G) { acc = 0; acc_phase ^= 1; }
     }
+  } else if (STEM && warp >= 2 + 4 * G) {
+    if constexpr (STEM) {
+      const int tid = (int)threadIdx.x - (64 + 128 * G);
+      if (p.img_u8) stem_box_producer<true>(p, tid, sA, sPatch, a_full, a_empty, unit0, ustep);
+      else stem_box_producer<false>(p, tid, sA, sPatch, a_full, a_empty, unit0, ustep);
+    }
   } else if (warp >= 2) {
     const int group = (warp - 2) >> 2;
     const int q = warp & 3;
@@ -582,7 +747,7 @@
     const int tq = row / p.BW;
     const int bh = tq % p.BH;
     const int bi = tq / p.BH;
-    constexpr int NBUF = kCBufCount / G;
+    constexpr int NBUF = CBUFS / G;
     uint8_t* gC = sC + group * NBUF * kCBufBytes;
     const bool f32 = (p.y_dtype == YV6_DT_F32);
     const float* sbias = nullptr;
@@ -1033,6 +1198,7 @@
     for (int g = 0; g < 2; ++g)
       for (int m = 0; m < 5; ++m)
         YV6_CHECK_CUDA(cudaFuncSetAttribute(kConvKernels[c][g][m], cudaFuncAttributeMaxDynamicSharedMemorySize, (int)h->max_smem_optin));
+  YV6_CHECK_CUDA(cudaFuncSetAttribute(conv_igemm_kernel<2, 5, false>, cudaFuncAttributeMaxDynamicSharedMemorySize, (int)h->max_smem_optin));
   cudaLaunchConfig_t cfg;
   memset(&cfg, 0, sizeof(cfg));
   cfg.gridDim = dim3((unsigned)(2 * h->num_sms));
@@ -1106,18 +1272,13 @@
   return YV6_OK;
 }
 
-extern "C" int yv6_conv_fwd(yv6_handle* h, const yv6_conv_desc* d, void* stream) {
-  yv6_device_guard _dev(h);
-  YV6_REQUIRE(h != nullptr, "conv_fwd: null handle");
-  { const int rc0 = conv_configure(h); if (rc0 != YV6_OK) return rc0; }
-  ConvPlan plan;
-  int rc = plan_conv(h, d, &plan);
-  if (rc != YV6_OK) return rc;
+static int conv_launch(yv6_handle* h, const yv6_conv_desc* d, const ConvPlan& plan, ConvKernelFn fn, bool with_a, int extra_threads,
+                       void* stream) {
   const ConvKParams& k = plan.k;
   YV6_REQUIRE(h->encode_tiled != nullptr, "conv_fwd: cuTensorMapEncodeTiled unavailable (no CUDA driver?)");
 
   CUtensorMap tmA, tmB, tmC;
-  {
+  if (with_a) {
     const uint64_t planes = (d->nsplit == 3) ? 3 : 1;
     cuuint64_t dims[5] = {(cuuint64_t)d->Cin, (cuuint64_t)d->W, (cuuint64_t)d->H, (cuuint64_t)d->N, planes};
     const uint64_t pix = (uint64_t)d->x_c_total * 2;
@@ -1185,15 +1346,14 @@
       return YV6_ERR_CUDA;
     }
   } else {
-    tmC = tmA;
-  }
-
-  const int mode = k.halo ? (k.halo == 2 ? 3 : 1) + (k.b_resident ? 1 : 0) : 0;
-  ConvKernelFn fn = kConvKernels[k.cpair][k.groups == 4 ? 1 : 0][mode];
+    tmC = tmB;
+  }
+  if (!with_a) tmA = tmB;
+
   cudaLaunchConfig_t cfg;
   memset(&cfg, 0, sizeof(cfg));
   cfg.gridDim = dim3((unsigned)plan.grid);
-  cfg.blockDim = dim3((unsigned)(64 + 128 * k.groups));
+  cfg.blockDim = dim3((unsigned)(64 + 128 * k.groups + extra_threads));
   cfg.dynamicSmemBytes = plan.smem_bytes;
   cfg.stream = (cudaStream_t)stream;
   cudaLaunchAttribute attr[1];
@@ -1209,3 +1369,59 @@
   YV6_CHECK_CUDA(cudaGetLastError());
   return YV6_OK;
 }
+
+extern "C" int yv6_conv_fwd(yv6_handle* h, const yv6_conv_desc* d, void* stream) {
+  yv6_device_guard _dev(h);
+  YV6_REQUIRE(h != nullptr, "conv_fwd: null handle");
+  { const int rc0 = conv_configure(h); if (rc0 != YV6_OK) return rc0; }
+  ConvPlan plan;
+  int rc = plan_conv(h, d, &plan);
+  if (rc != YV6_OK) return rc;
+  const ConvKParams& k = plan.k;
+  const int mode = k.halo ? (k.halo == 2 ? 3 : 1) + (k.b_resident ? 1 : 0) : 0;
+  return conv_launch(h, d, plan, kConvKernels[k.cpair][k.groups == 4 ? 1 : 0][mode], true, 0, stream);
+}
+
+extern "C" int yv6_stem_conv_fwd(yv6_handle* h, const yv6_stem_desc* s, const yv6_conv_desc* cd, void* stream) {
+  yv6_device_guard _dev(h);
+  YV6_REQUIRE(h != nullptr && s != nullptr && cd != nullptr, "stem_conv: null argument");
+  YV6_REQUIRE(s->x && s->w, "stem_conv: null stem tensor pointer");
+  YV6_REQUIRE(s->nsplit == 1 && !s->fp32_math && s->Cout == 32, "stem_conv: only the bf16 tensor-core stem with 32 channels is fused");
+  YV6_REQUIRE(s->x_dtype == YV6_DT_F32 || s->x_dtype == YV6_DT_U8, "stem_conv: image must be fp32 or uint8");
+  const int esz = (s->x_dtype == YV6_DT_F32) ? 4 : 1;
+  YV6_REQUIRE(s->W % 4 == 0 && (reinterpret_cast<uintptr_t>(s->x) & (4 * esz - 1)) == 0,
+              "stem_conv: image rows must be whole %d-byte groups (W=%d)", 4 * esz, s->W);
+  const int sHo = (s->H + 2 - 3) / 2 + 1, sWo = (s->W + 2 - 3) / 2 + 1;
+  YV6_REQUIRE(cd->pair_view == 1 && cd->N == s->N && cd->H == sHo && 2 * cd->W == sWo && cd->Cin == 2 * s->Cout &&
+                  cd->x_c_total == cd->Cin && cd->nsplit == 1,
+              "stem_conv: the conv is not the column-pair view of the stem's output");
+  { const int rc0 = conv_configure(h); if (rc0 != YV6_OK) return rc0; }
+  yv6_conv_desc c = *cd;
+  c.x = c.w;
+  ConvPlan plan;
+  int rc = plan_conv(h, &c, &plan);
+  if (rc != YV6_OK) return rc;
+  ConvKParams& k = plan.k;
+  YV6_REQUIRE(k.halo == 2 && k.b_resident && !k.cpair && k.tma_store == 2 && k.out_planes == 1,
+              "stem_conv: the conv does not run on the pair-view halo mainloop with resident weights (halo %d, resident %d, pair %d)",
+              k.halo, k.b_resident, k.cpair);
+  k.groups = 2;
+  k.tmem_cols = 32;
+  while (k.tmem_cols < k.groups * k.BN) k.tmem_cols *= 2;
+  k.a_stages = 2;
+  k.a_region_bytes = k.a_stages * HaloGeom<true>::kStageBytes;
+  plan.smem_bytes = (size_t)k.a_region_bytes + k.b_region_bytes + kStemCBufs * kCBufBytes + kBiasSmemFloats * sizeof(float) + 1024 +
+                    2 * kPatchBytes + 1024;
+  YV6_REQUIRE(plan.smem_bytes <= (size_t)h->max_smem_optin, "stem_conv: needs %zu bytes of shared memory, device offers %d",
+              plan.smem_bytes, h->max_smem_optin);
+  k.img = s->x;
+  k.stem_w = s->w;
+  k.stem_b = s->bias;
+  k.img_H = s->H;
+  k.img_W = s->W;
+  k.img_u8 = (s->x_dtype == YV6_DT_U8);
+  k.stem_act = s->act;
+  k.stem_Ho = sHo;
+  k.in_scale = s->in_scale;
+  return conv_launch(h, &c, plan, conv_igemm_kernel<2, 5, false>, false, 32 * kStemWarps, stream);
+}
diff --git a/yolov6_b200/engine.py b/yolov6_b200/engine.py
--- a/yolov6_b200/engine.py
+++ b/yolov6_b200/engine.py
@@ -19,6 +19,8 @@
 
 
 class InferEngine:
+    fuse_stem = True
+
     def __init__(self, graph, state_dict, device, precision="bf16"):
         if device.type != "cuda":
             raise RuntimeError("yolov6_b200 runs its networks on sm_100a CUDA kernels only (no CPU fallback); "
@@ -150,6 +152,11 @@
         def span(t):
             return (id(view(t)[0]), coff(t), coff(t) + t.c)
 
+        stem, nxt = g.ops[0], g.ops[1]
+        stem_fusable = (self.fuse_stem and P == 1 and stem.kind == "stem" and stem.cout == 32 and nxt.kind == "conv" and
+                        nxt.k == 3 and nxt.s == 2 and nxt.res is None and nxt.src == stem.dst and W % 4 == 0 and
+                        not any(t is not None and t.buf == stem.dst.buf for o in g.ops[2:] for t in (o.src, o.res)))
+        plan["stem_fused"] = False
         for i, op in enumerate(g.ops):
             ent = self.weights.get(i)
             if op.kind == "stem":
@@ -238,6 +245,12 @@
                             d.pair_view = 0
                     if "neck_start" not in plan and op.name.startswith("neck."):
                         plan["neck_start"] = len(plan["calls"])
+                    if stem_fusable and i == 1 and d.pair_view and out10[8] == 2 and out10[9] % 100 == 1:
+                        d.x = None
+                        plan["calls"][-1] = ("stem_conv", (plan["stem"], d))
+                        plan["deps"][-1] = dict(reads=[], writes=[span(op.dst)])
+                        plan["stem_fused"] = True
+                        continue
                     plan["calls"].append(("conv", d))
                     reads = [span(op.src)] + ([span(op.res)] if op.res is not None else [])
                     if op.kind == "pred":
@@ -251,6 +264,8 @@
                 buf, h, w, ct = view(op.dst)
                 plan["calls"].append(("pool", (buf.data_ptr(), N, h, w, op.cin, ct, P, buf.stride(0) if P == 3 else 0)))
                 plan["deps"].append(dict(reads=[(id(buf), 0, op.cin)], writes=[(id(buf), op.cin, 4 * op.cin)]))
+        if plan["stem_fused"]:
+            plan["bufs"][stem.dst.buf] = torch.empty(0, dtype=torch.bfloat16, device=dev)
         self._schedule(plan)
         self._plans[key] = plan
         return plan
@@ -339,12 +354,10 @@
                 for j in waits[i]:
                     streams[t].wait_event(events[j])
                 sp = sps[t]
-            if kind == "conv":
-                chk(lib.yv6_conv_fwd(h, C.byref(d), sp))
-            elif kind == "stem":
-                chk(lib.yv6_stem_fwd(h, C.byref(d), sp))
+            if kind == "pool":
+                chk(lib.yv6_sppf_pool(h, C.c_void_p(d[0]), d[1], d[2], d[3], d[4], d[5], d[6], d[7], sp))
             else:
-                chk(lib.yv6_sppf_pool(h, C.c_void_p(d[0]), d[1], d[2], d[3], d[4], d[5], d[6], d[7], sp))
+                self._launch(kind, d, sp)
             if multi and i in events:
                 events[i].record(streams[lane[i]])
         if multi:
@@ -361,6 +374,15 @@
                                 len(g.strides), plan["lvl_h"], plan["lvl_w"], plan["lvl_s"], sp))
         return plan["pred"]
 
+    def _launch(self, kind, d, sp):
+        lib, h = self.lib, self.handle
+        if kind == "conv":
+            _lib.check(lib.yv6_conv_fwd(h, C.byref(d), sp))
+        elif kind == "stem":
+            _lib.check(lib.yv6_stem_fwd(h, C.byref(d), sp))
+        else:
+            _lib.check(lib.yv6_stem_conv_fwd(h, C.byref(d[0]), C.byref(d[1]), sp))
+
     def head_outputs(self, N, H, W, in_dtype=torch.float32):
         plan = self._plan(N, H, W, in_dtype)
         return plan["cls"], plan["reg"]
@@ -381,14 +403,14 @@
         self.forward(x, stream)
         torch.cuda.synchronize()
         sp = _lib.stream_ptr(stream)
-        convs = [d for kind, d in plan["calls"] if kind == "conv"]
+        convs = [(kind, d) for kind, d in plan["calls"] if kind in ("conv", "stem_conv")]
         flops = sum(ci["flops"] for ci in plan["conv_info"])
         total_ms = 0.0
         for _ in range(steps):
             e0, e1 = torch.cuda.Event(enable_timing=True), torch.cuda.Event(enable_timing=True)
             e0.record()
-            for d in convs:
-                _lib.check(self.lib.yv6_conv_fwd(self.handle, C.byref(d), sp))
+            for kind, d in convs:
+                self._launch(kind, d, sp)
             e1.record()
             torch.cuda.synchronize()
             total_ms += e0.elapsed_time(e1)
@@ -412,15 +434,16 @@
         sp = _lib.stream_ptr(stream)
         flush = torch.empty(256 << 20, dtype=torch.uint8, device=self.device)
         rows = []
-        convs = [d for kind, d in plan["calls"] if kind == "conv"]
-        for ci, d in zip(plan["conv_info"], convs):
+        convs = [(kind, d) for kind, d in plan["calls"] if kind in ("conv", "stem_conv")]
+        for ci, (kind, call) in zip(plan["conv_info"], convs):
             name = ci["name"]
+            d = call[1] if kind == "stem_conv" else call
             ts = []
             for _ in range(iters):
                 flush.zero_()
                 e0, e1 = torch.cuda.Event(enable_timing=True), torch.cuda.Event(enable_timing=True)
                 e0.record()
-                _lib.check(self.lib.yv6_conv_fwd(self.handle, C.byref(d), sp))
+                self._launch(kind, call, sp)
                 e1.record()
                 torch.cuda.synchronize()
                 ts.append(e0.elapsed_time(e1))
@@ -430,6 +453,9 @@
             fl = ci["flops"]
             by = 2.0 * d.N * (ci["h"] * ci["w"] * ci["cin"] + ho * wo * ci["cout"])
             out = (C.c_int32 * 10)()
+            if kind == "stem_conv":
+                d = ConvDesc.from_buffer_copy(d)
+                d.x = d.w
             _lib.check(self.lib.yv6_conv_plan(self.handle, C.byref(d), out))
             rows.append(dict(name=name, cin=ci["cin"], cout=ci["cout"], k=ci["k"], s=ci["s"], hw=f"{ho}x{wo}", ms=ms,
                              tflops=fl / ms / 1e9, gbs=by / ms / 1e6, plan=list(out)))
```

New measurement: 15650, median of 6. -3.6%, worse.
